# yxyxcyx/Real-Time-Recommendation-System-with-Feature-Store

Hardware: AMD Instinct MI355X
Metric: user-item pairs scored/sec (train) + top-K queries/sec, emb_dim=128 (higher is better)
Workload: dtype f32; 1 GPU; C2: MovieLens-1M two-tower train step, emb 128, batch 1024, 16 negatives, hidden [256,128], dropout 0.2, tau 0.05, Adam+clip; global_batch=1024, emb_dim=128, num_negatives=16, parallelism=dp1

## Files before the change

### include/rtrec_hip.h

```cpp
#ifndef RTREC_HIP_H
#define RTREC_HIP_H

#include <stddef.h>
#include <stdint.h>

#ifdef __cplusplus
extern "C" {
#endif

typedef enum {
    RT_OK = 0,
    RT_ERR_INVALID = -1,
    RT_ERR_UNSUPPORTED = -2,
    RT_ERR_WORKSPACE = -3,
    RT_ERR_HIP = -4
} rt_status;

typedef enum { RT_F32 = 0, RT_F16 = 1, RT_BF16 = 2 } rt_dtype;

typedef enum {
    RT_ACT_RELU = 0,
    RT_ACT_GELU = 1,
    RT_ACT_LEAKY_RELU = 2,
    RT_ACT_TANH = 3,
    RT_ACT_SIGMOID = 4,
    RT_ACT_NONE = 5
} rt_act;

int rt_abi_version(void);
const char* rt_status_string(int status);
const char* rt_last_error(void);

int rt_gather_rows(const void* table, int64_t row_begin, int64_t n_rows, int64_t row_bytes,
                   const int64_t* ids, int64_t n_ids, void* out, int32_t* oob_count, void* stream);

int rt_scatter_add_rows_f32(float* grad_table, int64_t n_rows, int dim, const int64_t* ids,
                            int64_t n_ids, const float* grad_out, int64_t padding_idx, void* stream);

int rt_scatter_rows(const void* src, int64_t n, int64_t row_bytes, const int64_t* positions,
                    void* dst, int64_t dst_rows, int32_t* oob_count, void* stream);
size_t rt_rows_compact_workspace_bytes(int64_t n_rows);
int rt_rows_compact(const void* src, int64_t n_rows, int64_t row_bytes,
                    const uint32_t* keep_bits, int64_t keep_words,
                    void* dst, int64_t dst_rows, int64_t* n_kept,
                    void* workspace, size_t workspace_bytes, void* stream);

int rt_l2_renorm_f32(float* x, int64_t n, int d, void* stream);

size_t rt_flatip_topk_workspace_bytes(int64_t nq, int64_t nx, int d, int dtype, int k);
int rt_flatip_topk(const void* queries, int64_t nq, const void* items, int64_t nx, int d, int dtype,
                   int k, const uint32_t* exclude_bits, int64_t exclude_words, int64_t id_offset,
                   float* out_scores, int64_t* out_ids, void* workspace, size_t workspace_bytes,
                   void* stream);

#define RT_ONLINE_MAX_NQ 8
#define RT_ONLINE_MAX_K 128
size_t rt_flatip_topk_online_workspace_bytes(int64_t nq, int64_t nx, int d, int dtype, int k);
int rt_flatip_topk_online_plan(int64_t nq, int64_t nx, int d, int dtype, int k, int64_t* out);
int rt_flatip_topk_online(const void* queries, int64_t nq, const void* items, int64_t nx, int d, int dtype,
                          int k, const uint32_t* exclude_bits, int64_t exclude_words, int64_t id_offset,
                          float* out_scores, int64_t* out_ids, void* workspace, size_t workspace_bytes,
                          void* stream);

typedef struct {
    const int64_t* offsets;
    const int32_t* items;
    int64_t        n_rows;
    const int64_t* rows;
} RtExclusionLists;

#define RT_ONLINE_MAX_EXCL_SOURCES 2
int rt_flatip_topk_online_lists(const void* queries, int64_t nq, const void* items, int64_t nx, int d, int dtype,
                                int k, const RtExclusionLists* lists, int n_lists, int64_t id_offset,
                                float* out_scores, int64_t* out_ids, void* workspace, size_t workspace_bytes,
                                void* stream);

#define RT_IVF_MAX_K 128
#define RT_IVF_MAX_NPROBE 128
int rt_ivf_topk_tuning(int min_chunk_tiles);
int rt_ivf_topk_plan(int64_t nq, int nprobe, int64_t max_list_rows, int64_t* out);
size_t rt_ivf_topk_workspace_bytes(int64_t nq, int nprobe, int64_t max_list_rows, int k);
int rt_ivf_topk(const void* queries, int64_t nq, const void* rows, int64_t nx, int d, int dtype,
                const int64_t* list_offsets, int64_t nlist, const int32_t* row_pos, const int64_t* probes,
                int nprobe, int64_t max_list_rows, int k, const uint32_t* exclude_bits, int64_t exclude_words,
                float* out_scores, int64_t* out_ids, void* workspace, size_t workspace_bytes, void* stream);
int rt_segment_mean_f32(const void* rows, int64_t n, int d, int dtype, const int64_t* offsets, int64_t n_seg,
                        const float* prev, int normalize, float* out, void* stream);

size_t rt_flatip_topk_shard_workspace_bytes(int64_t nq, int64_t nx, int d, int dtype, int k);
int rt_flatip_topk_shard_plan(int64_t nq, int64_t nx, int d, int dtype, int k, int stride, int64_t* stage_counts);
int rt_flatip_topk_shard_sample(const void* queries, int64_t nq, const void* items, int64_t nx, int d, int dtype,
                                int k, int stride, float* top32, int64_t* stage_counts, void* workspace,
                                size_t workspace_bytes, void* stream);
int rt_topk_sample_rank(int k, int64_t sampled_stages, int64_t stages, int* rank);
int rt_topk_sample_threshold(const float* lists, int n_lists, int64_t nq, int rank, float* thr, void* stream);
int rt_flatip_topk_shard_search(const void* queries, int64_t nq, const void* items, int64_t nx, int d, int dtype,
                                int k, const float* thr, int64_t id_offset, float* out_scores, int64_t* out_ids,
                                void* workspace, size_t workspace_bytes, void* stream);

int rt_flatip_topk_tuning(int v4_mode, int v4_stride, int v4_rank);

int rt_l2_augment_f32(const float* x, int64_t n, int d, float* out, int ld_out, int role, void* stream);
int rt_l2_finish_f32(const float* q_aug, int ld_q, const float* x_aug, int ld_x, int d, int64_t nq, int k_sel,
                     const int64_t* sel_ids, const float* sel_scores, int k, float* scores, int64_t* ids,
                     int32_t* unverified, int64_t id_offset, void* stream);

int rt_topk_merge(const float* scores, const int64_t* ids, int64_t nq, int n_lists, int k_in,
                  int k_out, float* out_scores, int64_t* out_ids, void* stream);

int rt_sample_negatives(const int64_t* pos_offsets, const int32_t* pos_items, int64_t n_users,
                        const int64_t* users, int64_t n, int64_t num_items, int num_neg, uint64_t seed,
                        const uint64_t* seed_offset, int64_t* out, void* stream);

int rt_feeder_batch(const int64_t* order, const int64_t* inter_u, const int64_t* inter_m, const int64_t* state,
                    int64_t batch, int64_t* users, int64_t* pos, void* stream);
int rt_feeder_commit(const double* loss, double* losses, int64_t n_losses, int64_t* state, void* stream);

#ifndef RT_STAT_SLOTS
#define RT_STAT_SLOTS 8
#endif
#if RT_STAT_SLOTS > 15
#error "RT_STAT_SLOTS > 15: the host arenas (rtrec_amd/models/fused.py STAT_SLOTS) hold 16 slot rows, one of them for ticket counters"
#endif

typedef struct {
    const float* src;
    int64_t src_rows;
    int ld_src;
    const int64_t* ids;
    int64_t m;
    int k;
    int n;
    const float* w;
    const float* bias;
    int prev_mode;
    int prev_act;
    const double* prev_stats;
    const float* bn_gamma;
    const float* bn_beta;
    float* running_mean;
    float* running_var;
    float* save_mean;
    float* save_invstd;
    float bn_eps;
    float bn_momentum;
    float drop_p;
    uint64_t drop_seed;
    const uint64_t* seed_offset;
    float* z_out;
    int act;
    double* stats_out;
    float* l2_out;
    float* norms_out;
    int64_t* num_batches_tracked;
    int64_t seg_split;
    double* zero_buf;
    int64_t zero_words;
    float* wt_out;
    float* a_out;
    float* fin_save_mean;
    float* fin_save_invstd;
    float* fin_running_mean;
    float* fin_running_var;
    int64_t* fin_num_batches_tracked;
    float fin_eps;
    float fin_momentum;
    int prev_final;
    const uint16_t* w_planes;
    uint16_t* wt_planes_out;
    const float* next_w;
    uint16_t* next_w_planes;
    int next_n;
    int next_k;
} rt_linear_fwd_args;

int rt_linear_fwd_f32(const rt_linear_fwd_args* args, void* stream);

typedef struct {
    int64_t m; int k; int n;
    const float* w;
    float* dw;
    float* dbias;
    float* dz_ws;
    int grad_mode;
    const float* dout;
    const float* l2_out;
    const float* norms;
    const float* g;
    const float* z;
    int act;
    const double* g_stats;
    const float* save_mean;
    const float* save_invstd;
    const float* bn_gamma;
    float* dgamma;
    float* dbeta;
    const float* src; int64_t src_rows; int ld_src; const int64_t* ids;
    int prev_mode; int prev_act;
    const float* prev_mean; const float* prev_invstd;
    const float* prev_gamma; const float* prev_beta;
    float prev_drop_p; uint64_t prev_drop_seed; const uint64_t* seed_offset;
    float* g_prev;
    double* g_prev_stats;
    float* dsrc;
    int64_t seg_split;
    double* dbias_slots;
    const float* wt;
    int fuse_dz;
    const float* a_in;
    float* dw_part;
    const float* fold_src;
    float* fold_dst;
    int64_t fold_words;
    int fold_splits;
    int fold_in;
    const uint16_t* wt_planes;
} rt_linear_bwd_args;

int rt_linear_bwd_f32(const rt_linear_bwd_args* args, void* stream);
int rt_linear_bwd_dz_fused(const rt_linear_bwd_args* args, int n_args);
int rt_linear_bwd_dw_splits(const rt_linear_bwd_args* args, int n_args, int64_t* splits);
int rt_linear_bwd_dz_f32(const rt_linear_bwd_args* args, void* stream);
int rt_linear_bwd_dw_f32(const rt_linear_bwd_args* args, void* stream);
int rt_linear_fwd_f32_multi(const rt_linear_fwd_args* args, int n_args, void* stream);
int rt_linear_bwd_dz_f32_multi(const rt_linear_bwd_args* args, int n_args, void* stream);
int rt_linear_bwd_dw_f32_multi(const rt_linear_bwd_args* args, int n_args, void* stream);
int rt_linear_bwd_dw_f32_joint(const rt_linear_bwd_args* args, int n_args, void* stream);
int rt_linear_bwd_dw_joint_splits(const rt_linear_bwd_args* args, int n_args, int64_t* splits);

size_t rt_twotower_loss_workspace_bytes(int64_t b, int d);
int rt_twotower_loss_fwd_bwd(const void* u, const void* p, const void* q, int dtype, int64_t b,
                             int d, int n_neg, float inv_tau, const float* user_bias,
                             const float* item_bias, float w_explicit, float w_in_batch,
                             double* loss_out, float* du, float* dp, float* dq, float* d_user_bias,
                             float* d_item_bias, void* workspace, size_t workspace_bytes, void* stream);

int rt_twotower_loss_fwd(const void* u, const void* p, const void* q, int dtype, int64_t b, int d,
                         int n_neg, float inv_tau, const float* user_bias, const float* item_bias,
                         float w_explicit, float w_in_batch, double* loss_out, void* workspace,
                         size_t workspace_bytes, void* stream);

size_t rt_inbatch_loss_workspace_bytes(int64_t b, int64_t n_items, int d);
int rt_inbatch_loss_fwd_bwd(const void* u, const void* p, int dtype, int64_t b, int64_t n_items, int d,
                            int64_t label_offset, float inv_tau, double* loss_out, float* du, float* dp,
                            void* workspace, size_t workspace_bytes, void* stream);

int rt_similarity_f32(const float* u, const float* v, int64_t b, int d, float inv_tau,
                      const float* user_bias, const float* item_bias, float* out, void* stream);

#define RT_GRAD_FOLD_MAX 8
typedef struct {
    const float* part;
    int64_t dst_off;
    int64_t words;
    int splits;
    int tensor;
} rt_grad_fold;
int rt_grad_sqnorm(const float* grads, const int64_t* offsets, int n_tensors, double* sumsq_out,
                   int32_t* step_counter, int64_t* seed_counter, void* stream);
int rt_grad_sqnorm_fold(float* grads, const int64_t* offsets, int n_tensors, double* sumsq_out,
                        int32_t* step_counter, int64_t* seed_counter, const rt_grad_fold* folds,
                        int n_folds, void* stream);
int rt_clip_adam_step(float* params, float* grads, float* exp_avg, float* exp_avg_sq,
                      int64_t n, const double* sumsq, int n_tensors, float max_norm, float lr,
                      const float* lr_dev, float beta1, float beta2, float eps, float weight_decay,
                      int step, const int32_t* step_dev, double* zero_buf, int64_t zero_words,
                      void* stream);

#define RT_TOWER_MAX_LAYERS 8
#define RT_TOWER_MAX_ROWS   8
#define RT_TOWER_MAX_WIDTH  512
typedef struct {
    const float* w;
    const float* bias;
    int k, n;
    int act;
    const float* bn_gamma;
    const float* bn_beta;
    const float* bn_mean;
    const float* bn_var;
    float bn_eps;
} rt_tower_layer;
typedef struct {
    const float* src; int64_t src_rows; int ld_src;
    const int64_t* ids;
    int m;
    int n_layers;
    rt_tower_layer layers[RT_TOWER_MAX_LAYERS];
    int normalize;
    float* out;
    float* norms_out;
} rt_tower_infer_args;
int rt_tower_infer_f32(const rt_tower_infer_args* args, void* stream);

#define RT_METRICS_MAX_K 16

int rt_exclusion_bitmap(const int64_t* offsets, const int32_t* items, int64_t n_csr_rows, const int64_t* rows,
                        int64_t n_rows, int64_t n_items, uint32_t* bits, int64_t words, void* stream);
int rt_rank_metrics(const int64_t* preds, int64_t n_rows, int list_len, const int64_t* gt_offsets,
                    const int32_t* gt_items, const int64_t* gt_rows, int64_t n_gt_rows,
                    const int64_t* ex_offsets, const int32_t* ex_items, const int64_t* ex_rows,
                    int64_t n_ex_rows, const int32_t* k_values, int n_k, int64_t num_items,
                    double* per_row, int32_t* valid, uint32_t* coverage_bits, void* stream);
int rt_rank_metrics_reduce(const double* per_row, const int32_t* valid, int64_t n_rows, int n_cols,
                           const uint32_t* coverage_bits, int64_t num_items, double* out, void* stream);

int rt_list_metrics(const int64_t* preds, int64_t n_rows, int list_len, const void* emb, int emb_dtype,
                    int64_t n_emb, int d, int64_t ld_emb, const double* info, int64_t n_info, double default_info,
                    const int32_t* k_values, int n_k, double* div, int32_t* div_valid, double* nov_sum,
                    int32_t* nov_cnt, int32_t* oob_count, void* stream);
int rt_list_metrics_reduce(const double* div, const int32_t* div_valid, const double* nov_sum,
                           const int32_t* nov_cnt, int64_t n_rows, int n_k, double* out, void* stream);

#ifdef __cplusplus
}
#endif

#endif
```

### real-time-recommendation-system-with-feature-store_amd/csrc/loss.hip

```cpp
#include <float.h>

#include "rt_common.h"
#include "split3.h"

namespace rt {
size_t ib16_workspace_bytes(int64_t b, int64_t nx, int d);
int ib16_run(const void* u, const void* p, int dtype, int64_t b, int64_t nx, int d, int64_t off, float inv_tau,
             double* loss_out, float* du, float* dp, void* ws, size_t ws_bytes, hipStream_t st);
namespace loss {

typedef float f32x16 __attribute__((ext_vector_type(16)));
constexpr int RB = 32;
constexpr int kMaxD = 256;
constexpr int kMaxNeg = 64;
constexpr int NG = 16;


__device__ __forceinline__ int tile_row(int r, int h) { return (r & 3) + 8 * (r >> 2) + 4 * h; }

struct Args {
    const void* u; const void* p; const void* q;
    int64_t b; int d; int n_neg; float inv_tau;
    const float* ub; const float* ib;
    float we, wb;
    double* loss;
    float* du; float* dp; float* dq; float* dub; float* dib;
    float2* part;
    float* diag;
    float* expl;
    float* dposv;
    int64_t nx;
    int64_t off;
    int n_split;
    int ib_blocks;
    bool grad;
};

constexpr int SPAN = 256;
constexpr int LDP = 4;

template <typename T>
__device__ __forceinline__ float4 load4(const T* __restrict__ p) {
    if constexpr (sizeof(T) == 4) {
        return *reinterpret_cast<const float4*>(p);
    } else {
        const uint2 r = *reinterpret_cast<const uint2*>(p);
        const T* e = reinterpret_cast<const T*>(&r);
        return make_float4(to_f32(e[0]), to_f32(e[1]), to_f32(e[2]), to_f32(e[3]));
    }
}

template <int DP, typename T>
__device__ __forceinline__ void load_rows(const T* __restrict__ M, int64_t r0, int64_t n, int D,
                                          float4 (&v)[DP / 8]) {
    const int lane = threadIdx.x & 63;
#pragma unroll
    for (int u = 0; u < DP / 8; ++u) {
        const int e = lane + 64 * u;
        const int row = e / (DP / 4), c = (e % (DP / 4)) * 4;
        const int64_t gr = r0 + row;
        v[u] = make_float4(0.f, 0.f, 0.f, 0.f);
        if (gr < n && c < D) v[u] = load4<T>(M + gr * D + c);
    }
}
template <int DP>
__device__ __forceinline__ void store_rows(float* __restrict__ S, const float4 (&v)[DP / 8]) {
    const int lane = threadIdx.x & 63;
#pragma unroll
    for (int u = 0; u < DP / 8; ++u) {
        const int e = lane + 64 * u;
        const int row = e / (DP / 4), c = (e % (DP / 4)) * 4;
        *reinterpret_cast<float4*>(S + row * (DP + LDP) + c) = v[u];
    }
}
using fsplit::Pieces;
using fsplit::split8;
using fsplit::mfma3;
template <int DP, typename T>
__device__ __forceinline__ void load_fixed3(const T* __restrict__ F, int64_t f0, int64_t n, int D,
                                            Pieces (&pf)[DP / 16]) {
    const int lane = threadIdx.x & 63, c = lane & 31, h = lane >> 5;
    const int64_t r = f0 + c;
#pragma unroll
    for (int kb = 0; kb < DP / 16; ++kb) {
        const int k = 16 * kb + 8 * h;
        float4 u = make_float4(0.f, 0.f, 0.f, 0.f), v = u;
        if (r < n && k < D) {
            u = load4<T>(F + r * D + k);
            v = load4<T>(F + r * D + k + 4);
        }
        const float x[8] = {u.x, u.y, u.z, u.w, v.x, v.y, v.z, v.w};
        pf[kb] = split8(x);
    }
}
template <int DP>
__device__ __forceinline__ f32x16 s_tile3(const float* __restrict__ Ss, const Pieces (&pf)[DP / 16]) {
    const int lane = threadIdx.x & 63, c = lane & 31, h = lane >> 5;
    const float* ap = Ss + c * (DP + LDP) + 8 * h;
    f32x16 acc = {};
#pragma unroll
    for (int kb = 0; kb < DP / 16; ++kb) {
        const float4 u = *reinterpret_cast<const float4*>(ap + 16 * kb);
        const float4 v = *reinterpret_cast<const float4*>(ap + 16 * kb + 4);
        const float x[8] = {u.x, u.y, u.z, u.w, v.x, v.y, v.z, v.w};
        acc = mfma3(split8(x), pf[kb], acc);
    }
    return acc;
}
template <int DP>
constexpr size_t inb_lds_bytes(int waves) { return static_cast<size_t>(waves) * 32 * (DP + LDP) * sizeof(float); }
template <int DP>
constexpr int bwd_waves() {
#ifdef RT_LOSS_BWD_WAVES
    static_assert(RT_LOSS_BWD_WAVES == 4 || RT_LOSS_BWD_WAVES == 8, "the two forms that are built and tested");
    return DP <= 128 ? RT_LOSS_BWD_WAVES : 4;
#else
    return DP <= 128 ? 8 : 4;
#endif
}

template <int DP, typename T>
__global__ __launch_bounds__(256) void loss_fwd_kernel(Args a) {
    const T* __restrict__ U = static_cast<const T*>(a.u);
    const T* __restrict__ P = static_cast<const T*>(a.p);
    const T* __restrict__ Qn = static_cast<const T*>(a.q);
    extern __shared__ __attribute__((aligned(16))) float sm_f[];
    __shared__ float negs[4][kMaxNeg];
    __shared__ float red_m[4][RB], red_l[4][RB];
    const int tid = threadIdx.x, lane = tid & 63, w = tid >> 6, c = lane & 31, h = lane >> 5;
    const int it = blockIdx.x, js = blockIdx.y;
    const int64_t i0 = static_cast<int64_t>(it) * RB;
    const int D = a.d;
    const float bias = (a.ub ? a.ub[0] : 0.f) + (a.ib ? a.ib[0] : 0.f);
    const float inv_b = 1.f / static_cast<float>(a.b);

    if (js < a.ib_blocks) {
        float* Ss = sm_f + w * 32 * (DP + LDP);
        Pieces pf[DP / 16];
        load_fixed3<DP, T>(U, i0, a.b, D, pf);
        const int64_t t0 = static_cast<int64_t>(js) * SPAN + 32 * w, t1 = t0 + 128;
        float4 buf[DP / 8];
        load_rows<DP, T>(P, t0, a.nx, D, buf);
        float om = -INFINITY, ol = 0.f;
#pragma unroll 1
        for (int q = 0; q < 2; ++q) {
            const int64_t tt = q == 0 ? t0 : t1;
            if (tt >= a.nx) break;
            store_rows<DP>(Ss, buf);
            wave_lds_sync();
            if (q == 0 && t1 < a.nx) load_rows<DP, T>(P, t1, a.nx, D, buf);
            const f32x16 acc = s_tile3<DP>(Ss, pf);
#pragma unroll
            for (int r = 0; r < 16; ++r) {
                if (tt + tile_row(r, h) < a.nx) {
                    const float sv = acc[r] * a.inv_tau;
                    if (sv > om) { ol = ol * expf(om - sv) + 1.f; om = sv; }
                    else ol += expf(sv - om);
                }
            }
            wave_lds_sync();
        }
        const float m2 = __shfl_xor(om, 32, 64), l2 = __shfl_xor(ol, 32, 64);
        const float mm = fmaxf(om, m2);
        ol = (mm == -INFINITY) ? 0.f : ol * expf(om - mm) + l2 * expf(m2 - mm);
        if (h == 0) { red_m[w][c] = mm; red_l[w][c] = ol; }
        __syncthreads();
        if (w == 0 && h == 0 && i0 + c < a.b) {
            float m3 = -INFINITY;
            for (int x = 0; x < 4; ++x) m3 = fmaxf(m3, red_m[x][c]);
            float ll = 0.f;
            if (m3 != -INFINITY)
                for (int x = 0; x < 4; ++x) ll += red_l[x][c] * expf(red_m[x][c] - m3);
            a.part[static_cast<int64_t>(js) * a.b + i0 + c] = make_float2(m3, ll);
        }
        return;
    }

    const int64_t i = i0 + 4 * (js - a.ib_blocks) + w;
    if (i >= a.b) return;
    const T* ur = U + i * D;
    const T* pr = P + (a.off + i) * D;
    constexpr int V = kMaxD / 64;
    float uv[V], pv[V];
    float part = 0.f;
#pragma unroll
    for (int t = 0; t < V; ++t) {
        const int dd = lane + 64 * t;
        uv[t] = dd < D ? to_f32(ur[dd]) : 0.f;
        pv[t] = dd < D ? to_f32(pr[dd]) : 0.f;
        part += uv[t] * pv[t];
    }
    float qv[NG][V];
    auto load_q = [&](int g0) {
#pragma unroll
        for (int jj = 0; jj < NG; ++jj) {
            const int j = g0 + jj;
            const T* qr = Qn + (i * a.n_neg + (j < a.n_neg ? j : 0)) * D;
#pragma unroll
            for (int t = 0; t < V; ++t) {
                const int dd = lane + 64 * t;
                qv[jj][t] = (j < a.n_neg && dd < D) ? to_f32(qr[dd]) : 0.f;
            }
        }
    };
    if (a.n_neg > 0) load_q(0);
    const float dup = wave_sum(part) * a.inv_tau;
    if (lane == 0) a.diag[i] = dup;
    if (a.n_neg <= 0) {
        if (a.grad) {
#pragma unroll
            for (int t = 0; t < V; ++t) {
                const int dd = lane + 64 * t;
                if (dd < D) { a.du[i * D + dd] = 0.f; a.dp[i * D + dd] = 0.f; }
            }
        }
        return;
    }
    const float pos = dup + bias;
    float mx = pos;
    for (int g0 = 0; g0 < a.n_neg; g0 += NG) {
        if (g0 > 0) load_q(g0);
        float part_j[NG];
#pragma unroll
        for (int jj = 0; jj < NG; ++jj) {
            part_j[jj] = 0.f;
#pragma unroll
            for (int t = 0; t < V; ++t) part_j[jj] += uv[t] * qv[jj][t];
        }
#pragma unroll
        for (int o = 32; o > 0; o >>= 1)
#pragma unroll
            for (int jj = 0; jj < NG; ++jj) part_j[jj] += __shfl_xor(part_j[jj], o, 64);
#pragma unroll
        for (int jj = 0; jj < NG; ++jj) {
            if (g0 + jj < a.n_neg) {
                const float nv = part_j[jj] * a.inv_tau;
                if (lane == 0) negs[w][g0 + jj] = nv;
                mx = fmaxf(mx, nv);
            }
        }
    }
    wave_lds_sync();
    float se = expf(pos - mx);
    for (int j = 0; j < a.n_neg; ++j) se += expf(negs[w][j] - mx);
    const float lse = mx + logf(se);
    const float dpos = a.we * inv_b * (expf(pos - lse) - 1.f);
    if (lane == 0) {
        a.expl[i] = lse - pos;
        a.dposv[i] = dpos;
    }
    if (!a.grad) return;
    float duv[V];
#pragma unroll
    for (int t = 0; t < V; ++t) duv[t] = dpos * pv[t];
    for (int g0 = 0; g0 < a.n_neg; g0 += NG) {
        if (a.n_neg > NG) load_q(g0);
#pragma unroll
        for (int jj = 0; jj < NG; ++jj) {
            const int j = g0 + jj;
            if (j >= a.n_neg) break;
            const float dn = a.we * inv_b * expf(negs[w][j] - lse);
            float* dqr = a.dq + (i * a.n_neg + j) * D;
#pragma unroll
            for (int t = 0; t < V; ++t) {
                const int dd = lane + 64 * t;
                if (dd < D) {
                    duv[t] += dn * qv[jj][t];
                    dqr[dd] = dn * uv[t] * a.inv_tau;
                }
            }
        }
    }
#pragma unroll
    for (int t = 0; t < V; ++t) {
        const int dd = lane + 64 * t;
        if (dd < D) {
            a.du[i * D + dd] = duv[t] * a.inv_tau;
            a.dp[i * D + dd] = dpos * uv[t] * a.inv_tau;
        }
    }
}

__device__ __forceinline__ float combine_lse(const float2* part, int n_split, int64_t b, int64_t i) {
    float mm = -INFINITY;
    for (int s = 0; s < n_split; ++s) mm = fmaxf(mm, part[static_cast<int64_t>(s) * b + i].x);
    float ll = 0.f;
    for (int s = 0; s < n_split; ++s) {
        const float2 v = part[static_cast<int64_t>(s) * b + i];
        if (v.x != -INFINITY) ll += v.y * expf(v.x - mm);
    }
    return mm + logf(ll);
}

template <int DP, typename T, int NW>
__global__ __launch_bounds__(64 * NW) void loss_bwd_kernel(Args a, float wb_eff, bool add_loss) {
    constexpr int DT = DP / 32;
    constexpr int NT = SPAN / (32 * NW);
    static_assert(NT * 32 * NW == SPAN && NT >= 1, "the waves' tiles cover the span");
    extern __shared__ __attribute__((aligned(16))) float sm_b[];
    __shared__ float lse_s[SPAN];
    const int tid = threadIdx.x, lane = tid & 63, w = tid >> 6, c = lane & 31, h = lane >> 5;
    const int D = a.d;
    const bool row_pass = blockIdx.z == 0;
    const int64_t f0 = static_cast<int64_t>(blockIdx.x) * RB;
    const int64_t s0 = static_cast<int64_t>(blockIdx.y) * SPAN;
    const int64_t n_fixed = row_pass ? a.b : a.nx, n_str = row_pass ? a.nx : a.b;
    if (f0 >= n_fixed || s0 >= n_str) {
        if (!(row_pass && blockIdx.y == 0 && f0 < a.b)) return;
    }
    const T* Fm = static_cast<const T*>(row_pass ? a.u : a.p);
    const T* Sm = static_cast<const T*>(row_pass ? a.p : a.u);
    const float scale = wb_eff / static_cast<float>(a.b);
    float lse_fixed = 0.f;
    const bool ib = wb_eff != 0.f;
    if (row_pass) {
        const int64_t i = f0 + c;
        if (ib && i < a.b) lse_fixed = combine_lse(a.part, a.n_split, a.b, i);
        if (add_loss && blockIdx.y == 0 && w == 0) {
            double li = 0.0, le = 0.0;
            float dpb = 0.f;
            if (h == 0 && i < a.b) {
                if (ib) li = static_cast<double>(lse_fixed - a.diag[i]) / static_cast<double>(a.b);
                if (a.n_neg > 0) {
                    le = static_cast<double>(a.expl[i]) / static_cast<double>(a.b);
                    dpb = a.dposv[i];
                }
            }
            li = wave_sum(li);
            le = wave_sum(le);
            dpb = wave_sum(dpb);
            if (lane == 0) {
                if (ib) atomicAdd(&a.loss[2], li);
                if (a.n_neg > 0) atomicAdd(&a.loss[1], le);
                atomicAdd(&a.loss[0], static_cast<double>(wb_eff) * li + static_cast<double>(a.we) * le);
                if (a.grad && a.n_neg > 0) {
                    if (a.dub) atomicAdd(a.dub, dpb);
                    if (a.dib) atomicAdd(a.dib, dpb);
                }
            }
        }
    } else {
        for (int x = tid; x < SPAN; x += 64 * NW) {
            const int64_t i = s0 + x;
            lse_s[x] = i < a.b ? combine_lse(a.part, a.n_split, a.b, i) : 0.f;
        }
    }
    __syncthreads();
    if (!a.grad || !ib || f0 >= n_fixed || s0 >= n_str) return;

    float* Ss = sm_b + w * 32 * (DP + LDP);
    Pieces pf[DP / 16];
    load_fixed3<DP, T>(Fm, f0, n_fixed, D, pf);
    const int64_t t0 = s0 + 32 * w;
    float4 buf[DP / 8];
    load_rows<DP, T>(Sm, t0, n_str, D, buf);
    f32x16 acc[DT];
#pragma unroll
    for (int x = 0; x < DT; ++x) acc[x] = f32x16{};
#pragma unroll 1
    for (int q = 0; q < NT; ++q) {
        const int64_t tt = t0 + 32 * NW * q;
        if (tt >= n_str) break;
        store_rows<DP>(Ss, buf);
        wave_lds_sync();
        if (q + 1 < NT && tt + 32 * NW < n_str) load_rows<DP, T>(Sm, tt + 32 * NW, n_str, D, buf);
        const f32x16 st = s_tile3<DP>(Ss, pf);
        float ds[16];
        const int64_t fcol = f0 + c;
#pragma unroll
        for (int r = 0; r < 16; ++r) {
            const int rr = tile_row(r, h);
            const int64_t srow = tt + rr;
            float v = 0.f;
            if (srow < n_str && fcol < n_fixed) {
                const float lse = row_pass ? lse_fixed : lse_s[32 * (w + NW * q) + rr];
                const bool label = row_pass ? (srow == a.off + fcol) : (fcol == a.off + srow);
                v = scale * (expf(st[r] * a.inv_tau - lse) - (label ? 1.f : 0.f));
            }
            ds[r] = v;
        }
        Pieces pds[2];
#pragma unroll
        for (int b = 0; b < 2; ++b) {
            const float x[8] = {ds[8 * b], ds[8 * b + 1], ds[8 * b + 2], ds[8 * b + 3],
                                ds[8 * b + 4], ds[8 * b + 5], ds[8 * b + 6], ds[8 * b + 7]};
            pds[b] = split8(x);
        }
#pragma unroll
        for (int dt = 0; dt < DT; ++dt) {
#pragma unroll
            for (int b = 0; b < 2; ++b) {
                float y[8];
#pragma unroll
                for (int j = 0; j < 8; ++j) y[j] = Ss[tile_row(8 * b + j, h) * (DP + LDP) + dt * 32 + c];
                acc[dt] = mfma3(pds[b], split8(y), acc[dt]);
            }
        }
        wave_lds_sync();
    }
    __syncthreads();
    float* red = sm_b;
#pragma unroll
    for (int dt = 0; dt < DT; ++dt)
#pragma unroll
        for (int r = 0; r < 16; ++r) red[(w * DT * 16 + dt * 16 + r) * 64 + lane] = acc[dt][r];
    __syncthreads();
    float* out = row_pass ? a.du : a.dp;
    for (int p = tid; p < DT * 16 * 64; p += 64 * NW) {
        const int v = p >> 6, l = p & 63;
        float t = red[v * 64 + l];
#pragma unroll
        for (int x = 1; x < NW; ++x) t += red[(x * DT * 16 + v) * 64 + l];
        const int dt = v >> 4, r = v & 15;
        const int64_t gi = f0 + tile_row(r, l >> 5);
        const int dd = dt * 32 + (l & 31);
        if (gi < n_fixed && dd < D) atomicAdd(&out[gi * D + dd], t * a.inv_tau);
    }
}

__global__ __launch_bounds__(256) void similarity_kernel(const float* u, const float* v, int64_t b, int d,
                                                         float inv_tau, const float* ub, const float* ib,
                                                         float* out) {
    const int lane = threadIdx.x & 63;
    const int64_t i = static_cast<int64_t>(blockIdx.x) * 4 + (threadIdx.x >> 6);
    if (i >= b) return;
    float s = 0.f;
    for (int dd = lane; dd < d; dd += 64) s += u[i * d + dd] * v[i * d + dd];
    s = wave_sum(s);
    if (lane == 0) {
        float r = s * inv_tau;
        if (ub) r = r + ub[0] + ib[0];
        out[i] = r;
    }
}

}
}

using namespace rt;

namespace {
template <auto Kernel>
void allow_lds(size_t bytes) {
    static size_t set = 0;
    if (bytes > set) {
        (void)hipFuncSetAttribute(reinterpret_cast<const void*>(Kernel), hipFuncAttributeMaxDynamicSharedMemorySize,
                                  static_cast<int>(bytes));
        set = bytes;
    }
}

template <int DP, typename T>
int launch_loss(const loss::Args& a, dim3 grid1, dim3 grid2, float wb_eff, hipStream_t st) {
    const size_t lds1 = loss::inb_lds_bytes<DP>(4);
    allow_lds<loss::loss_fwd_kernel<DP, T>>(lds1);
    hipLaunchKernelGGL((loss::loss_fwd_kernel<DP, T>), grid1, dim3(256), lds1, st, a);
    const int rc = check_launch("loss_fwd_kernel");
    if (rc) return rc;
    constexpr int NW = loss::bwd_waves<DP>();
    const size_t lds2 = loss::inb_lds_bytes<DP>(NW);
    allow_lds<loss::loss_bwd_kernel<DP, T, NW>>(lds2);
    hipLaunchKernelGGL((loss::loss_bwd_kernel<DP, T, NW>), grid2, dim3(64 * NW), lds2, st, a, wb_eff, true);
    return check_launch("loss_bwd_kernel");
}

template <typename T>
int launch_loss_d(const loss::Args& a, int dp32, dim3 grid1, dim3 grid2, float wb_eff, hipStream_t st) {
    switch (dp32) {
        case 32: return launch_loss<32, T>(a, grid1, grid2, wb_eff, st);
        case 64: return launch_loss<64, T>(a, grid1, grid2, wb_eff, st);
        case 96:
        case 128: return launch_loss<128, T>(a, grid1, grid2, wb_eff, st);
        default: return launch_loss<256, T>(a, grid1, grid2, wb_eff, st);
    }
}

size_t loss_ws_bytes(int64_t b, int64_t nx) {
    const int64_t n_split = (nx + loss::SPAN - 1) / loss::SPAN;
    return static_cast<size_t>(n_split) * b * sizeof(float2) + 3 * static_cast<size_t>(b) * sizeof(float);
}

int run_loss(const void* u, const void* p, const void* q, int dtype, int64_t b, int64_t nx, int64_t off, int d,
             int n_neg, float inv_tau, const float* ub, const float* ib, float we, float wb, double* loss_out,
             float* du, float* dp, float* dq, float* dub, float* dib, void* ws, size_t ws_bytes, void* stream,
             bool grad) {
    if (dtype != RT_F32 && dtype != RT_F16 && dtype != RT_BF16) return RT_ERR_INVALID;
    if (b <= 0 || d <= 0 || n_neg < 0 || !u || !p || !loss_out) return RT_ERR_INVALID;
    if (nx < b || off < 0 || off + b > nx) return RT_ERR_INVALID;
    if (d % 8 != 0 || d > loss::kMaxD || n_neg > loss::kMaxNeg) return RT_ERR_UNSUPPORTED;
    if (n_neg > 0 && !q) return RT_ERR_INVALID;
    if (grad && (!du || !dp || (n_neg > 0 && !dq))) return RT_ERR_INVALID;
    const int n_split = static_cast<int>((nx + loss::SPAN - 1) / loss::SPAN);
    if (!ws || ws_bytes < loss_ws_bytes(b, nx)) return RT_ERR_WORKSPACE;
    if ((reinterpret_cast<uintptr_t>(u) | reinterpret_cast<uintptr_t>(p)) & 15) return RT_ERR_INVALID;
    float2* part = reinterpret_cast<float2*>(ws);
    float* diag = reinterpret_cast<float*>(part + static_cast<size_t>(n_split) * b);
    const float wb_eff = n_neg > 0 ? wb : 1.f;
    const float we_eff = n_neg > 0 ? we : 0.f;
    const bool want_ib = wb_eff != 0.f;
    loss::Args a{u, p, q, b, d, n_neg, inv_tau, ub, ib, we_eff, wb_eff, loss_out, du, dp, dq, dub, dib, part, diag,
                 diag + b, diag + 2 * b, nx, off, n_split, want_ib ? n_split : 0, grad};
    hipStream_t st = as_stream(stream);
    if (grad && nx != b) {
        if (hipMemsetAsync(dp, 0, static_cast<size_t>(nx) * d * sizeof(float), st) != hipSuccess)
            return check_launch("hipMemsetAsync(dp)");
    }
    const int64_t big = nx > b ? nx : b;
    const int dp32 = (d + 31) / 32 * 32;
    const unsigned y2 = static_cast<unsigned>((big + loss::SPAN - 1) / loss::SPAN);
    const dim3 grid1(static_cast<unsigned>((b + loss::RB - 1) / loss::RB), a.ib_blocks + 8);
    const dim3 grid2(static_cast<unsigned>((big + loss::RB - 1) / loss::RB), want_ib ? y2 : 1,
                     (grad && want_ib) ? 2 : 1);
    switch (dtype) {
        case RT_F32: return launch_loss_d<float>(a, dp32, grid1, grid2, wb_eff, st);
        case RT_F16: return launch_loss_d<__half>(a, dp32, grid1, grid2, wb_eff, st);
        default: return launch_loss_d<__hip_bfloat16>(a, dp32, grid1, grid2, wb_eff, st);
    }
}
}

extern "C" size_t rt_twotower_loss_workspace_bytes(int64_t b, int d) {
    (void)d;
    if (b <= 0) return 256;
    return loss_ws_bytes(b, b) + 256;
}

extern "C" size_t rt_inbatch_loss_workspace_bytes(int64_t b, int64_t n_items, int d) {
    if (b <= 0 || n_items < b || d <= 0) return 256;
    const size_t f32 = loss_ws_bytes(b, n_items), h16 = ib16_workspace_bytes(b, n_items, d);
    return (f32 > h16 ? f32 : h16) + 256;
}

extern "C" int rt_inbatch_loss_fwd_bwd(const void* u, const void* p, int dtype, int64_t b, int64_t n_items, int d,
                                       int64_t label_offset, float inv_tau, double* loss_out, float* du, float* dp,
                                       void* workspace, size_t workspace_bytes, void* stream) {
    if (dtype == RT_F16 || dtype == RT_BF16) {
        if (b <= 0 || d <= 0 || !u || !p || !loss_out) return RT_ERR_INVALID;
        if (n_items < b || label_offset < 0 || label_offset + b > n_items) return RT_ERR_INVALID;
        if (d % 8 != 0 || d > loss::kMaxD) return RT_ERR_UNSUPPORTED;
        if ((du == nullptr) != (dp == nullptr)) return RT_ERR_INVALID;
        if ((reinterpret_cast<uintptr_t>(u) | reinterpret_cast<uintptr_t>(p)) & 15) return RT_ERR_INVALID;
        return ib16_run(u, p, dtype, b, n_items, d, label_offset, inv_tau, loss_out, du, dp, workspace,
                        workspace_bytes, as_stream(stream));
    }
    return run_loss(u, p, nullptr, dtype, b, n_items, label_offset, d, 0, inv_tau, nullptr, nullptr, 0.f, 1.f,
                    loss_out, du, dp, nullptr, nullptr, nullptr, workspace, workspace_bytes, stream, du != nullptr);
}


extern "C" int rt_twotower_loss_fwd_bwd(const void* u, const void* p, const void* q, int dtype, int64_t b, int d,
                                        int n_neg, float inv_tau, const float* user_bias, const float* item_bias,
                                        float w_explicit, float w_in_batch, double* loss_out, float* du, float* dp,
                                        float* dq, float* d_user_bias, float* d_item_bias, void* workspace,
                                        size_t workspace_bytes, void* stream) {
    return run_loss(u, p, q, dtype, b, b, 0, d, n_neg, inv_tau, user_bias, item_bias, w_explicit, w_in_batch,
                    loss_out, du, dp, dq, d_user_bias, d_item_bias, workspace, workspace_bytes, stream, true);
}

extern "C" int rt_twotower_loss_fwd(const void* u, const void* p, const void* q, int dtype, int64_t b, int d,
                                    int n_neg, float inv_tau, const float* user_bias, const float* item_bias,
                                    float w_explicit, float w_in_batch, double* loss_out, void* workspace,
                                    size_t workspace_bytes, void* stream) {
    return run_loss(u, p, q, dtype, b, b, 0, d, n_neg, inv_tau, user_bias, item_bias, w_explicit, w_in_batch,
                    loss_out, nullptr, nullptr, nullptr, nullptr, nullptr, workspace, workspace_bytes, stream, false);
}

extern "C" int rt_similarity_f32(const float* u, const float* v, int64_t b, int d, float inv_tau,
                                 const float* user_bias, const float* item_bias, float* out, void* stream) {
    if (b < 0 || d <= 0 || !u || !v || !out) return RT_ERR_INVALID;
    if ((user_bias == nullptr) != (item_bias == nullptr)) return RT_ERR_INVALID;
    if (b == 0) return RT_OK;
    hipLaunchKernelGGL(loss::similarity_kernel, dim3(static_cast<unsigned>((b + 3) / 4)), dim3(256), 0,
                       as_stream(stream), u, v, b, d, inv_tau, user_bias, item_bias, out);
    return check_launch("similarity_kernel");
}
```

### real-time-recommendation-system-with-feature-store_amd/csrc/mlp.hip

```cpp
#include "rt_common.h"
#include "split3.h"

namespace rt {
namespace mlp {

typedef float f32x16 __attribute__((ext_vector_type(16)));



constexpr float kNormEps = 1e-12f;

struct FwdLaunch {
    rt_linear_fwd_args a0, a1;
    unsigned split;
};
struct BwdLaunch {
    rt_linear_bwd_args a0, a1;
    unsigned split;
    int64_t rps0, rps1;
    unsigned tn0, tk0, tn1, tk1;
    bool vec0, vec1;
    int ngroups;
    unsigned ksplit = 1;
};

constexpr int kFoldG = 8;
__device__ __forceinline__ void fold_side(const BwdLaunch& L, int which) {
    const int64_t nt = static_cast<int64_t>(gridDim.x) * blockDim.x;
    const int64_t gt = static_cast<int64_t>(blockIdx.x) * blockDim.x + threadIdx.x;
    for (int g = 0; g < L.ngroups; ++g) {
        const rt_linear_bwd_args& f = g ? L.a1 : L.a0;
        if (!f.fold_src || f.fold_in != which || f.fold_splits <= 0) continue;
        const int64_t n4 = f.fold_words / 4;
        const int ng = (f.fold_splits + kFoldG - 1) / kFoldG;
        for (int64_t it = gt; it < n4 * ng; it += nt) {
            const int64_t e = it % n4;
            const int s0 = static_cast<int>(it / n4) * kFoldG;
            float4 v[kFoldG];
#pragma unroll
            for (int j = 0; j < kFoldG; ++j)
                v[j] = s0 + j < f.fold_splits
                           ? reinterpret_cast<const float4*>(f.fold_src + static_cast<int64_t>(s0 + j) * f.fold_words)[e]
                           : make_float4(0.f, 0.f, 0.f, 0.f);
            float4 t = v[0];
#pragma unroll
            for (int j = 1; j < kFoldG; ++j) { t.x += v[j].x; t.y += v[j].y; t.z += v[j].z; t.w += v[j].w; }
            float* d = f.fold_dst + 4 * e;
            if (ng == 1) {
                const float4 o = *reinterpret_cast<const float4*>(d);
                *reinterpret_cast<float4*>(d) = make_float4(o.x + t.x, o.y + t.y, o.z + t.z, o.w + t.w);
            } else {
                atomicAdd(d, t.x); atomicAdd(d + 1, t.y); atomicAdd(d + 2, t.z); atomicAdd(d + 3, t.w);
            }
        }
    }
}


#ifdef RT_PHASE_PROBE
__device__ unsigned long long* g_probe_buf = nullptr;
__device__ unsigned int g_probe_ctr[64];
__device__ unsigned int g_probe_cap = 0;
struct PhaseProbe {
    uint64_t rt0 = 0, t0 = 0, m[4] = {0, 0, 0, 0};
    __device__ __forceinline__ void start() {
        if (threadIdx.x == 0) {
            rt0 = __builtin_amdgcn_s_memrealtime();
            t0 = __builtin_amdgcn_s_memtime();
        }
    }
    __device__ __forceinline__ void mark(int i) {
        if (threadIdx.x == 0) m[i] = __builtin_amdgcn_s_memtime() - t0;
    }
    __device__ __forceinline__ void end(unsigned tag) {
        if (threadIdx.x == 0) {
            asm volatile("s_waitcnt vmcnt(0)" ::: "memory");
            m[3] = __builtin_amdgcn_s_memtime() - t0;
            const uint64_t rt1 = __builtin_amdgcn_s_memrealtime();
            const unsigned xcc = __builtin_amdgcn_s_getreg((20) | (0 << 6) | ((4 - 1) << 11));
            const unsigned sh = blockIdx.x & 63u;
            const unsigned slot = atomicAdd(&g_probe_ctr[sh], 1u);
            if (slot < g_probe_cap && g_probe_buf) {
                unsigned long long* o = g_probe_buf + (static_cast<uint64_t>(slot) * 64 + sh) * 8;
                o[0] = (static_cast<uint64_t>(tag) << 32) | blockIdx.x;
                o[1] = rt0; o[2] = m[0]; o[3] = m[1]; o[4] = m[2]; o[5] = m[3]; o[6] = rt1; o[7] = xcc;
            }
        }
    }
};
#define RT_PP_DECL PhaseProbe pp_; pp_.start();
#define RT_PP_MARK(i) pp_.mark(i);
#define RT_PP_END(tag) pp_.end(tag);
#else
#define RT_PP_DECL
#define RT_PP_MARK(i)
#define RT_PP_END(tag)
#endif

#if !defined(RT_NO_WT_STORES)
#define RT_WT_STORES 1
#endif
__device__ __forceinline__ void st_act(float* p, float v) {
#ifdef RT_WT_STORES
    __hip_atomic_store(p, v, __ATOMIC_RELAXED, __HIP_MEMORY_SCOPE_AGENT);
#else
    *p = v;
#endif
}
__device__ __forceinline__ void st_act4(float* p, float4 v) {
#ifdef RT_WT_STORES
    typedef float f4v __attribute__((ext_vector_type(4)));
    const f4v x = {v.x, v.y, v.z, v.w};
    asm volatile("global_store_dwordx4 %0, %1, off sc1" ::"v"(p), "v"(x) : "memory");
#else
    *reinterpret_cast<float4*>(p) = v;
#endif
}

__device__ __forceinline__ f32x16 mfma(float a, float b, f32x16 c) {
    return __builtin_amdgcn_mfma_f32_32x32x2f32(a, b, c, 0, 0, 0);
}

using fsplit::Pieces;
using fsplit::s16x8;
using fsplit::split8;
using fsplit::mfma3;
using fsplit::split3;

struct Pro {
    int mode;
    int act;
    float drop_p, drop_scale;
    uint64_t seed;
    const float* scale;
    const float* shift;
};

__device__ __forceinline__ float pro_apply(const Pro& p, int64_t r, int c, float v) {
    if (p.mode == 0) return v;
    v = act_eval(p.act, v);
    if (p.mode != 3) v = __builtin_fmaf(v, p.scale[c], p.shift[c]);
    if (p.drop_p > 0.f) v = dropout_keep(p.seed, r, c, p.drop_p) ? v * p.drop_scale : 0.f;
    return v;
}

__device__ __forceinline__ void slot_sums(const double* __restrict__ base, int w, int c, double& s1, double& s2) {
    double v1[RT_STAT_SLOTS], v2[RT_STAT_SLOTS];
#pragma unroll
    for (int sl = 0; sl < RT_STAT_SLOTS; ++sl) {
        v1[sl] = base[static_cast<int64_t>(sl) * 2 * w + c];
        v2[sl] = base[static_cast<int64_t>(sl) * 2 * w + w + c];
    }
    s1 = 0.0;
    s2 = 0.0;
#pragma unroll
    for (int sl = 0; sl < RT_STAT_SLOTS; ++sl) {
        s1 += v1[sl];
        s2 += v2[sl];
    }
}

__device__ __forceinline__ void bn_affine(float gamma, float beta, float mean, float invstd, float& scale,
                                          float& shift) {
    scale = gamma * invstd;
    shift = __builtin_fmaf(-mean, scale, beta);
}

__device__ __forceinline__ void ticket_release() {
#ifdef RT_TICKET_WBL2
    __builtin_amdgcn_fence(__ATOMIC_RELEASE, "agent");
#endif
    asm volatile("s_waitcnt vmcnt(0)" ::: "memory");
}

__device__ __forceinline__ void bn_finalize_last(const rt_linear_fwd_args& a, unsigned nblk) {
    __shared__ int last_s;
    const int tid = threadIdx.x, n = a.n;
    const bool two = a.seg_split > 0;
    const int nseg = two ? 2 : 1;
    asm volatile("s_waitcnt vmcnt(0)" ::: "memory");
    __syncthreads();
    if (tid == 0) {
        ticket_release();
        unsigned long long* cnt =
            reinterpret_cast<unsigned long long*>(a.stats_out + static_cast<int64_t>(nseg) * RT_STAT_SLOTS * 2 * n);
        last_s = atomicAdd(cnt, 1ull) == static_cast<unsigned long long>(nblk) - 1ull ? 1 : 0;
    }
    __syncthreads();
    if (!last_s) return;
    for (int c = tid; c < n; c += blockDim.x) {
        for (int sg = 0; sg < nseg; ++sg) {
            const int64_t ms = two ? (sg == 0 ? a.seg_split : a.m - a.seg_split) : a.m;
            double* ps = a.stats_out + static_cast<int64_t>(sg) * RT_STAT_SLOTS * 2 * n;
            double v1[RT_STAT_SLOTS], v2[RT_STAT_SLOTS];
#pragma unroll
            for (int sl = 0; sl < RT_STAT_SLOTS; ++sl) {
                v1[sl] = atomicAdd(&ps[static_cast<int64_t>(sl) * 2 * n + c], 0.0);
                v2[sl] = atomicAdd(&ps[static_cast<int64_t>(sl) * 2 * n + n + c], 0.0);
            }
            double s1 = 0.0, s2 = 0.0;
#pragma unroll
            for (int sl = 0; sl < RT_STAT_SLOTS; ++sl) {
                s1 += v1[sl];
                s2 += v2[sl];
            }
            const double md = s1 / static_cast<double>(ms);
            double vd = s2 / static_cast<double>(ms) - md * md;
            vd = vd > 0.0 ? vd : 0.0;
            const float mean = static_cast<float>(md);
            const float invstd = static_cast<float>(1.0 / sqrt(vd + static_cast<double>(a.fin_eps)));
            const float var_f = static_cast<float>(ms > 1 ? vd * static_cast<double>(ms) / static_cast<double>(ms - 1) : vd);
            a.fin_save_mean[sg * n + c] = mean;
            if (a.fin_save_invstd) a.fin_save_invstd[sg * n + c] = invstd;
            if (a.fin_running_mean) {
                const float mo = a.fin_momentum;
                a.fin_running_mean[c] = (1.f - mo) * a.fin_running_mean[c] + mo * mean;
                a.fin_running_var[c] = (1.f - mo) * a.fin_running_var[c] + mo * var_f;
            }
        }
    }
    if (tid == 0 && a.fin_num_batches_tracked) *a.fin_num_batches_tracked += nseg;
}

constexpr int FM = 32;

__host__ __device__ __forceinline__ int pad8(int k) { return (k + 31) / 32 * 32; }
__host__ __device__ __forceinline__ bool dz_norm_fast(int n) {
    const int l4 = n / 4;
    return (n % 4) == 0 && l4 <= 64 && (l4 & (l4 - 1)) == 0 && pad8(n) == n;
}
__host__ __device__ __forceinline__ bool dz_bn_fast(int n, int act, int grad_mode) {
    return (n % 4) == 0 && (256 % (pad8(n) / 4)) == 0 && act_is_piecewise_linear(act) && grad_mode != 3;
}
__host__ __device__ __forceinline__ bool dz_da_fast(const rt_linear_bwd_args& a) {
    return !a.dsrc && a.g_prev && act_is_piecewise_linear(a.prev_act);
}

template <int TPW, bool KVEC, bool WPL>
__global__ __launch_bounds__(256) __attribute__((amdgpu_waves_per_eu(TPW == 1 ? 3 : 2))) void linear_fwd_kernel(FwdLaunch L) {
    static_assert(!WPL || (TPW == 1 && KVEC), "split-weight planes: one-tile waves, k % 4 == 0");
    const bool g1 = blockIdx.x >= L.split;
    const rt_linear_fwd_args& a = g1 ? L.a1 : L.a0;
    const unsigned bid = blockIdx.x - (g1 ? L.split : 0u);
    constexpr int NT = 4 * TPW;
    extern __shared__ __attribute__((aligned(16))) float sm[];
    const int k = a.k, n = a.n;
    const int kp = pad8(k), aplane = FM * kp, aw = 3 * aplane / 2;
    const int nch = kp / 8, am = ((nch & -nch) < 16 ? (nch & -nch) : 16) - 1;
    float* scale = sm;
    float* shift = scale + kp;
    float* As = shift + kp;
    uint16_t* const Ap = reinterpret_cast<uint16_t*>(As);
    float* rowpart = As + aw;
    int64_t* srow = reinterpret_cast<int64_t*>(rowpart + NT * FM);

    const int tid = threadIdx.x, lane = tid & 63, w = tid >> 6, h = lane >> 5, c32 = lane & 31;
    const int64_t row0 = static_cast<int64_t>(bid) * FM;
    const int64_t m = a.m;
    auto put_a = [&](int r, int c, float4 o) {
        if (a.a_out && c < k && row0 + r < m) st_act4(a.a_out + (row0 + r) * k + c, o);
        uint32_t h0, m0, l0, h1, m1, l1;
        split3(o.x, o.y, h0, m0, l0);
        split3(o.z, o.w, h1, m1, l1);
        uint16_t* q = Ap + r * kp + ((((c >> 3) ^ (r & am)) << 3) | (c & 7));
        *reinterpret_cast<uint2*>(q) = make_uint2(h0, h1);
        *reinterpret_cast<uint2*>(q + aplane) = make_uint2(m0, m1);
        *reinterpret_cast<uint2*>(q + 2 * aplane) = make_uint2(l0, l1);
    };
    RT_PP_DECL
    if (blockIdx.x == 0 && a.zero_buf)
        for (int64_t e = tid; e < a.zero_words; e += 256) a.zero_buf[e] = 0.0;

    const int vpr = kp / 4;
    const bool vec = (a.ld_src % 4) == 0 && (reinterpret_cast<uintptr_t>(a.src) & 15) == 0;
    const bool fast = vec && (a.k % 4) == 0 && (256 % vpr) == 0 &&
                      (a.prev_mode == 0 || act_is_piecewise_linear(a.prev_act));
    const bool early = fast && !a.ids && 8 * (256 / vpr) >= FM;
    if (a.wt_out) {
        const int tk = (k + 31) / 32, tiles = tk * ((n + 31) / 32);
        const int nblk = static_cast<int>(g1 ? gridDim.x - L.split : L.split);
        for (int wt = static_cast<int>(bid); wt < tiles; wt += nblk) {
            const int n0 = (wt / tk) * 32, k0 = (wt % tk) * 32;
            const int r = tid >> 3, c = (tid & 7) * 4;
            if (n0 + r < n) {
#pragma unroll
                for (int j = 0; j < 4; ++j)
                    if (k0 + c + j < k) a.wt_out[static_cast<int64_t>(k0 + c + j) * n + n0 + r] = a.w[static_cast<int64_t>(n0 + r) * k + k0 + c + j];
            }
        }
    }
    if (a.wt_planes_out || a.next_w_planes) {
        const int nblk = static_cast<int>(g1 ? gridDim.x - L.split : L.split);
        if (a.wt_planes_out) {
            const int64_t plane = static_cast<int64_t>(n) * k;
            const int nq = (n + 3) / 4;
            for (int64_t e = static_cast<int64_t>(bid) * 256 + tid; e < static_cast<int64_t>(k) * nq;
                 e += static_cast<int64_t>(nblk) * 256) {
                const int kk = static_cast<int>(e / nq), n0 = static_cast<int>(e % nq) * 4;
                float x[4];
#pragma unroll
                for (int j = 0; j < 4; ++j) x[j] = n0 + j < n ? a.w[static_cast<int64_t>(n0 + j) * k + kk] : 0.f;
                uint32_t h0, m0, l0, h1, m1, l1;
                split3(x[0], x[1], h0, m0, l0);
                split3(x[2], x[3], h1, m1, l1);
                uint16_t* q = a.wt_planes_out + static_cast<int64_t>(kk) * n + n0;
                if (n0 + 4 <= n && (n % 4) == 0) {
                    *reinterpret_cast<uint2*>(q) = make_uint2(h0, h1);
                    *reinterpret_cast<uint2*>(q + plane) = make_uint2(m0, m1);
                    *reinterpret_cast<uint2*>(q + 2 * plane) = make_uint2(l0, l1);
                } else {
                    const uint32_t hv[2] = {h0, h1}, mv[2] = {m0, m1}, lv[2] = {l0, l1};
                    for (int j = 0; j < 4 && n0 + j < n; ++j) {
                        const int sh = 16 * (j & 1);
                        q[j] = static_cast<uint16_t>(hv[j >> 1] >> sh);
                        q[j + plane] = static_cast<uint16_t>(mv[j >> 1] >> sh);
                        q[j + 2 * plane] = static_cast<uint16_t>(lv[j >> 1] >> sh);
                    }
                }
            }
        }
        if (a.next_w_planes) {
            const int64_t tot8 = static_cast<int64_t>(a.next_n) * a.next_k / 8;
            const float4* src4 = reinterpret_cast<const float4*>(a.next_w);
            s16x8* dst = reinterpret_cast<s16x8*>(a.next_w_planes);
            for (int64_t e = static_cast<int64_t>(bid) * 256 + tid; e < tot8; e += static_cast<int64_t>(nblk) * 256) {
                const float4 u = src4[2 * e], v = src4[2 * e + 1];
                const float x[8] = {u.x, u.y, u.z, u.w, v.x, v.y, v.z, v.w};
                const Pieces pc = split8(x);
                dst[e] = pc.hi;
                dst[e + tot8] = pc.mid;
                dst[e + 2 * tot8] = pc.lo;
            }
        }
    }
    const float* wrow[TPW];
    bool tile_on[TPW], row_ok[TPW];
#pragma unroll
    for (int i = 0; i < TPW; ++i) {
        tile_on[i] = (w + 4 * i) * 32 < n;
        const int nn = (w + 4 * i) * 32 + c32;
        row_ok[i] = nn < n;
        wrow[i] = a.w + static_cast<int64_t>(row_ok[i] ? nn : 0) * k;
    }
    float4 wv[TPW][4], wn[TPW][4];
    auto load_w = [&](int s, float4 (&dst)[TPW][4]) {
#pragma unroll
        for (int i = 0; i < TPW; ++i)
#pragma unroll
            for (int j = 0; j < 4; ++j) {
                const int kk = s + 16 * (j >> 1) + 8 * h + 4 * (j & 1);
                float4 v = make_float4(0.f, 0.f, 0.f, 0.f);
                if (tile_on[i] && row_ok[i]) {
                    const float* wr = wrow[i] + kk;
                    if constexpr (KVEC) {
                        if (kk < k) v = *reinterpret_cast<const float4*>(wr);
                    } else {
                        if (kk < k) v.x = wr[0];
                        if (kk + 1 < k) v.y = wr[1];
                        if (kk + 2 < k) v.z = wr[2];
                        if (kk + 3 < k) v.w = wr[3];
                    }
                }
                dst[i][j] = v;
            }
    };
    uint4 pv[2][3], pn[2][3];
    const int64_t wplane = static_cast<int64_t>(n) * k;
    auto load_p = [&](int s, uint4 (&dst)[2][3]) {
#pragma unroll
        for (int b = 0; b < 2; ++b) {
            const int kk = s + 16 * b + 8 * h;
            const bool ok = tile_on[0] && row_ok[0] && kk < k;
            const uint16_t* q = a.w_planes + (static_cast<int64_t>(row_ok[0] ? w * 32 + c32 : 0) * k + (ok ? kk : 0));
#pragma unroll
            for (int p = 0; p < 3; ++p)
                dst[b][p] = ok ? *reinterpret_cast<const uint4*>(q + p * wplane) : make_uint4(0u, 0u, 0u, 0u);
        }
    };
    if constexpr (WPL) load_p(0, pn);
    else if constexpr (TPW == 1) load_w(0, wn);
    float4 pre[8];
    if (early) {
        const int c = (tid % vpr) * 4, rstep = 256 / vpr, r0 = tid / vpr;
#pragma unroll
        for (int u = 0; u < 8; ++u) {
            const int r = r0 + u * rstep;
            const int64_t gr = row0 + r;
            pre[u] = make_float4(0.f, 0.f, 0.f, 0.f);
            if (r < FM && c < k && gr < m && gr < a.src_rows)
                pre[u] = *reinterpret_cast<const float4*>(a.src + gr * a.ld_src + c);
        }
    }

    const bool two = a.seg_split > 0;
    const int my_seg = (two && row0 >= a.seg_split) ? 1 : 0;
    if (a.prev_mode == 1 && a.prev_final) {
        for (int c = tid; c < k; c += 256)
            bn_affine(a.bn_gamma[c], a.bn_beta[c], a.save_mean[my_seg * k + c], a.save_invstd[my_seg * k + c], scale[c],
                      shift[c]);
    } else if (a.prev_mode == 1 || a.prev_mode == 2) {
        const int nseg = two ? 2 : 1;
        for (int c = tid; c < k; c += 256) {
            for (int sg = 0; sg < nseg; ++sg) {
                if (bid != 0 && sg != my_seg) continue;
                const int64_t ms = two ? (sg == 0 ? a.seg_split : m - a.seg_split) : m;
                float mean, invstd, var_f = 0.f;
                if (a.prev_mode == 1) {
                    const double* ps = a.prev_stats + static_cast<int64_t>(sg) * RT_STAT_SLOTS * 2 * k;
                    double s1, s2;
                    slot_sums(ps, k, c, s1, s2);
                    const double md = s1 / static_cast<double>(ms);
                    double vd = s2 / static_cast<double>(ms) - md * md;
                    vd = vd > 0.0 ? vd : 0.0;
                    mean = static_cast<float>(md);
                    invstd = static_cast<float>(1.0 / sqrt(vd + static_cast<double>(a.bn_eps)));
                    var_f = static_cast<float>(ms > 1 ? vd * static_cast<double>(ms) / static_cast<double>(ms - 1) : vd);
                } else {
                    mean = a.running_mean[c];
                    invstd = static_cast<float>(1.0 / sqrt(static_cast<double>(a.running_var[c]) + a.bn_eps));
                }
                if (sg == my_seg) bn_affine(a.bn_gamma[c], a.bn_beta[c], mean, invstd, scale[c], shift[c]);
                if (bid == 0) {
                    if (c == 0 && a.prev_mode == 1 && a.num_batches_tracked) *a.num_batches_tracked += 1;
                    if (a.save_mean) a.save_mean[sg * k + c] = mean;
                    if (a.save_invstd) a.save_invstd[sg * k + c] = invstd;
                    if (a.prev_mode == 1 && a.running_mean) {
                        const float mo = a.bn_momentum;
                        a.running_mean[c] = (1.f - mo) * a.running_mean[c] + mo * mean;
                        a.running_var[c] = (1.f - mo) * a.running_var[c] + mo * var_f;
                    }
                }
            }
        }
    }
    RT_PP_MARK(0)
    if (tid < FM) {
        const int64_t gr = row0 + tid;
        int64_t sr = -1;
        if (gr < m) {
            sr = a.ids ? a.ids[gr] : gr;
            if (sr < 0 || sr >= a.src_rows) sr = -1;
        }
        srow[tid] = sr;
    }
    __syncthreads();
    const uint64_t seed = a.drop_seed + (a.seed_offset ? *a.seed_offset : 0ull);
    const Pro pro{a.prev_mode, a.prev_act, a.drop_p, a.drop_p > 0.f ? 1.f / (1.f - a.drop_p) : 1.f, seed,
                  scale, shift};
    {
        const int total = FM * vpr;
        if (fast) {
            const int c = (tid % vpr) * 4, rstep = 256 / vpr;
            const bool bn = pro.mode == 1 || pro.mode == 2;
            const float4 sc4 = bn ? *reinterpret_cast<const float4*>(scale + c) : make_float4(1.f, 1.f, 1.f, 1.f);
            const float4 sh4 = bn ? *reinterpret_cast<const float4*>(shift + c) : make_float4(0.f, 0.f, 0.f, 0.f);
            const float sl = act_slope(pro.act);
            const bool drop = pro.drop_p > 0.f;
            for (int r0 = tid / vpr; r0 < FM; r0 += 8 * rstep) {
                float4 v[8];
#pragma unroll
                for (int u = 0; u < 8; ++u) {
                    const int r = r0 + u * rstep;
                    v[u] = make_float4(0.f, 0.f, 0.f, 0.f);
                    if (early) {
                        v[u] = pre[u];
                    } else if (r < FM && c < k) {
                        const int64_t sr = srow[r];
                        if (sr >= 0) v[u] = *reinterpret_cast<const float4*>(a.src + sr * a.ld_src + c);
                    }
                }
#pragma unroll
                for (int u = 0; u < 8; ++u) {
                    const int r = r0 + u * rstep;
                    if (r >= FM) break;
                    const int64_t gr = row0 + r;
                    const bool ok = srow[r] >= 0 && c < k;
                    auto tf = [&](float x, int cc, float scv, float shv) {
                        if (pro.mode == 0) return x;
                        x = act_pwl(sl, x);
                        if (bn) x = __builtin_fmaf(x, scv, shv);
                        if (drop) x = dropout_keep(pro.seed, gr, cc, pro.drop_p) ? x * pro.drop_scale : 0.f;
                        return x;
                    };
                    float4 o;
                    o.x = ok ? tf(v[u].x, c, sc4.x, sh4.x) : 0.f;
                    o.y = ok ? tf(v[u].y, c + 1, sc4.y, sh4.y) : 0.f;
                    o.z = ok ? tf(v[u].z, c + 2, sc4.z, sh4.z) : 0.f;
                    o.w = ok ? tf(v[u].w, c + 3, sc4.w, sh4.w) : 0.f;
                    put_a(r, c, o);
                }
            }
        } else
        for (int base = tid; base < total; base += 256 * 4) {
            float4 v[4];
#pragma unroll
            for (int u = 0; u < 4; ++u) {
                const int e = base + u * 256;
                v[u] = make_float4(0.f, 0.f, 0.f, 0.f);
                if (e < total) {
                    const int r = e / vpr, c = (e - r * vpr) * 4;
                    const int64_t sr = srow[r];
                    if (sr >= 0 && c < k) {
                        const float* sp = a.src + sr * a.ld_src + c;
                        if (vec && c + 4 <= k) v[u] = *reinterpret_cast<const float4*>(sp);
                        else {
                            v[u].x = sp[0];
                            if (c + 1 < k) v[u].y = sp[1];
                            if (c + 2 < k) v[u].z = sp[2];
                            if (c + 3 < k) v[u].w = sp[3];
                        }
                    }
                }
            }
#pragma unroll
            for (int u = 0; u < 4; ++u) {
                const int e = base + u * 256;
                if (e < total) {
                    const int r = e / vpr, c = (e - r * vpr) * 4;
                    const bool ok = srow[r] >= 0;
                    const int64_t gr = row0 + r;
                    float4 o;
                    o.x = (ok && c < k) ? pro_apply(pro, gr, c, v[u].x) : 0.f;
                    o.y = (ok && c + 1 < k) ? pro_apply(pro, gr, c + 1, v[u].y) : 0.f;
                    o.z = (ok && c + 2 < k) ? pro_apply(pro, gr, c + 2, v[u].z) : 0.f;
                    o.w = (ok && c + 3 < k) ? pro_apply(pro, gr, c + 3, v[u].w) : 0.f;
                    put_a(r, c, o);
                }
            }
        }
    }
    __syncthreads();
    RT_PP_MARK(1)

    f32x16 acc[TPW];
#pragma unroll
    for (int i = 0; i < TPW; ++i) acc[i] = f32x16{};
    const uint16_t* ap = Ap + c32 * kp;
    const int asw = c32 & am;
    if constexpr (TPW != 1) load_w(0, wn);
    if constexpr (WPL) {
        for (int s = 0; s < kp; s += 32) {
#pragma unroll
            for (int b = 0; b < 2; ++b)
#pragma unroll
                for (int p = 0; p < 3; ++p) pv[b][p] = pn[b][p];
            if (s + 32 < kp) load_p(s + 32, pn);
#pragma unroll
            for (int b = 0; b < 2; ++b) {
                const int ao = (((s + 16 * b) >> 3) + h) ^ asw;
                Pieces pa;
                pa.hi = *reinterpret_cast<const s16x8*>(ap + 8 * ao);
                pa.mid = *reinterpret_cast<const s16x8*>(ap + aplane + 8 * ao);
                pa.lo = *reinterpret_cast<const s16x8*>(ap + 2 * aplane + 8 * ao);
                if (tile_on[0]) {
                    const Pieces pb{__builtin_bit_cast(s16x8, pv[b][0]), __builtin_bit_cast(s16x8, pv[b][1]),
                                    __builtin_bit_cast(s16x8, pv[b][2])};
                    acc[0] = mfma3(pa, pb, acc[0]);
                }
            }
        }
    } else
    for (int s = 0; s < kp; s += 32) {
#pragma unroll
        for (int i = 0; i < TPW; ++i)
#pragma unroll
            for (int j = 0; j < 4; ++j) wv[i][j] = wn[i][j];
        if (s + 32 < kp) load_w(s + 32, wn);
#pragma unroll
        for (int b = 0; b < 2; ++b) {
            const int ao = (((s + 16 * b) >> 3) + h) ^ asw;
            Pieces pa;
            pa.hi = *reinterpret_cast<const s16x8*>(ap + 8 * ao);
            pa.mid = *reinterpret_cast<const s16x8*>(ap + aplane + 8 * ao);
            pa.lo = *reinterpret_cast<const s16x8*>(ap + 2 * aplane + 8 * ao);
#pragma unroll
            for (int i = 0; i < TPW; ++i) {
                if (!tile_on[i]) continue;
                const float4 u = wv[i][2 * b], v = wv[i][2 * b + 1];
                const float x[8] = {u.x, u.y, u.z, u.w, v.x, v.y, v.z, v.w};
                acc[i] = mfma3(pa, split8(x), acc[i]);
            }
        }
    }

    RT_PP_MARK(2)
    const bool l2 = a.l2_out != nullptr;
    if (l2 && !a.z_out && !a.stats_out && n * (FM + 1) <= aw) {
        __syncthreads();
        float* zsq = As;
#pragma unroll
        for (int i = 0; i < TPW; ++i) {
            const int col = (w + 4 * i) * 32 + c32;
            if ((w + 4 * i) * 32 >= n) continue;
            const bool col_ok = col < n;
            const float b = (col_ok && a.bias) ? a.bias[col] : 0.f;
#pragma unroll
            for (int r = 0; r < 16; ++r) {
                const int lr = (r & 3) + 8 * (r >> 2) + 4 * h;
                const float z = acc[i][r] + b;
                acc[i][r] = z;
                if (col_ok) zsq[col * (FM + 1) + lr] = (row0 + lr < m) ? z * z : 0.f;
            }
        }
        __syncthreads();
        {
            const int row = tid >> 3, part = tid & 7;
            float ss = 0.f;
            for (int c = part; c < n; c += 8) ss += zsq[c * (FM + 1) + row];
            ss += __shfl_xor(ss, 1, 64);
            ss += __shfl_xor(ss, 2, 64);
            ss += __shfl_xor(ss, 4, 64);
            if (part == 0) {
                const float nrm = sqrtf(ss);
                rowpart[row] = 1.f / fmaxf(nrm, kNormEps);
                if (row0 + row < m && a.norms_out) a.norms_out[row0 + row] = nrm;
            }
        }
        __syncthreads();
#pragma unroll
        for (int i = 0; i < TPW; ++i) {
            const int col = (w + 4 * i) * 32 + c32;
            if ((w + 4 * i) * 32 >= n) continue;
#pragma unroll
            for (int r = 0; r < 16; ++r) {
                const int lr = (r & 3) + 8 * (r >> 2) + 4 * h;
                const int64_t gr = row0 + lr;
                if (gr < m && col < n) st_act(a.l2_out + gr * n + col, acc[i][r] * rowpart[lr]);
            }
        }
        RT_PP_END(1)
        return;
    }
    double* const stats = a.stats_out ? a.stats_out + (static_cast<int64_t>(my_seg) * RT_STAT_SLOTS +
                                                       bid % RT_STAT_SLOTS) * 2 * n : nullptr;
#pragma unroll
    for (int i = 0; i < TPW; ++i) {
        const int ct = w + 4 * i;
        const int col = ct * 32 + c32;
        const bool col_ok = col < n;
        const float b = (col_ok && a.bias) ? a.bias[col] : 0.f;
        float s1 = 0.f, s2 = 0.f;
        if (row0 + FM <= m && a.z_out && !l2 && act_is_piecewise_linear(a.act)) {
            if (ct * 32 >= n) continue;
            float* zp = a.z_out + (row0 + 4 * h) * n + col;
            const float sl = act_slope(a.act);
#pragma unroll
            for (int r = 0; r < 16; ++r) {
                const float z = acc[i][r] + b;
                if (col_ok) st_act(zp + ((r & 3) + 8 * (r >> 2)) * n, z);
                const float av = act_pwl(sl, z);
                s1 += av;
                s2 += av * av;
            }
            if (!col_ok) s1 = s2 = 0.f;
        } else
#pragma unroll
        for (int r = 0; r < 16; ++r) {
            const int lr = (r & 3) + 8 * (r >> 2) + 4 * h;
            const int64_t gr = row0 + lr;
            const float z = acc[i][r] + b;
            acc[i][r] = z;
            const bool ok = col_ok && gr < m;
            if (ok && a.z_out) st_act(a.z_out + gr * n + col, z);
            if (ok && stats) {
                const float av = act_eval(a.act, z);
                s1 += av;
                s2 += av * av;
            }
            if (l2) {
                float q = ok ? z * z : 0.f;
#pragma unroll
                for (int o = 1; o < 32; o <<= 1) q += __shfl_xor(q, o, 64);
                if (c32 == 0) rowpart[ct * FM + lr] = q;
            }
        }
        if (stats) {
            s1 += __shfl_xor(s1, 32, 64);
            s2 += __shfl_xor(s2, 32, 64);
            if (h == 0 && col_ok) {
                atomicAdd(&stats[col], static_cast<double>(s1));
                atomicAdd(&stats[n + col], static_cast<double>(s2));
            }
        }
    }
    if (stats && a.fin_save_mean) bn_finalize_last(a, g1 ? gridDim.x - L.split : L.split);
    if (l2) {
        __syncthreads();
        const int nt_used = (n + 31) / 32;
#pragma unroll
        for (int i = 0; i < TPW; ++i) {
            const int col = (w + 4 * i) * 32 + c32;
#pragma unroll
            for (int r = 0; r < 16; ++r) {
                const int lr = (r & 3) + 8 * (r >> 2) + 4 * h;
                const int64_t gr = row0 + lr;
                if (gr < m && col < n) {
                    float ss = 0.f;
                    for (int t = 0; t < nt_used; ++t) ss += rowpart[t * FM + lr];
                    const float nrm = sqrtf(ss);
                    a.l2_out[gr * n + col] = acc[i][r] / fmaxf(nrm, kNormEps);
                    if (col == 0 && a.norms_out) a.norms_out[gr] = nrm;
                }
            }
        }
    }
    RT_PP_END(1)
}

template <int TPWK, bool WPL, bool KS, int FE>
__global__ __launch_bounds__(256) __attribute__((amdgpu_waves_per_eu(3))) void linear_bwd_dz_kernel(BwdLaunch L) {
#ifdef RT_FOLD_FIRST
    fold_side(L, 0);
#endif
    const unsigned kpart = KS ? blockIdx.x % L.ksplit : 0u, bx = KS ? blockIdx.x / L.ksplit : blockIdx.x;
    const bool prim = kpart == 0;
    const int tb = static_cast<int>(kpart) * 4 * TPWK;
    const bool g1 = bx >= L.split;
    const rt_linear_bwd_args& a = g1 ? L.a1 : L.a0;
    const unsigned bid = bx - (g1 ? L.split : 0u);
    extern __shared__ __attribute__((aligned(16))) float sm[];
    const int n = a.n, k = a.k;
    const int64_t m = a.m;
    const int np = pad8(n), ldz = np + 4;
    float* Dz = sm;
    const int tid = threadIdx.x, lane = tid & 63, w = tid >> 6, h = lane >> 5, c32 = lane & 31;
    const int64_t row0 = static_cast<int64_t>(bid) * FM;
    const bool two = a.seg_split > 0;
    const int my_seg = (two && row0 >= a.seg_split) ? 1 : 0;
    const int64_t seg_m = two ? (my_seg == 0 ? a.seg_split : m - a.seg_split) : m;
    RT_PP_DECL

    float wv[TPWK][8], wn[TPWK][8];
    const float* __restrict__ Wt = a.w;
#ifdef RT_NO_WT_ROWS
    const float* __restrict__ WtT = nullptr;
#else
    const float* __restrict__ WtT = (a.wt && (n % 8) == 0) ? a.wt : nullptr;
#endif
    auto load_w = [&](int s, float (&dst)[TPWK][8]) {
#pragma unroll
        for (int i = 0; i < TPWK; ++i) {
            const int kk = (tb + w + 4 * i) * 32 + c32;
            const bool on = (tb + w + 4 * i) * 32 < k && kk < k;
            if (FE != 0 || WtT) {
                const int nn = s + 8 * h;
                float4 v0 = make_float4(0.f, 0.f, 0.f, 0.f), v1 = v0;
                if (on && nn < n) {
                    const float* p = WtT + static_cast<int64_t>(kk) * n + nn;
                    v0 = *reinterpret_cast<const float4*>(p);
                    v1 = *reinterpret_cast<const float4*>(p + 4);
                }
                dst[i][0] = v0.x; dst[i][1] = v0.y; dst[i][2] = v0.z; dst[i][3] = v0.w;
                dst[i][4] = v1.x; dst[i][5] = v1.y; dst[i][6] = v1.z; dst[i][7] = v1.w;
            } else {
#pragma unroll
                for (int j = 0; j < 8; ++j) {
                    const int nn = s + 8 * h + j;
                    dst[i][j] = (on && nn < n) ? Wt[static_cast<int64_t>(nn) * k + kk] : 0.f;
                }
            }
        }
    };
    uint4 pv[TPWK][3], pn[TPWK][3];
    const uint16_t* __restrict__ WtP = a.wt_planes;
    const int64_t tplane = static_cast<int64_t>(k) * n;
    auto load_p = [&](int s, uint4 (&dst)[TPWK][3]) {
#pragma unroll
        for (int i = 0; i < TPWK; ++i) {
            const int kk = (tb + w + 4 * i) * 32 + c32;
            const int nn = s + 8 * h;
            const bool ok = (tb + w + 4 * i) * 32 < k && kk < k && nn < n;
            const uint16_t* q = WtP + (ok ? static_cast<int64_t>(kk) * n + nn : 0);
#pragma unroll
            for (int p = 0; p < 3; ++p)
                dst[i][p] = ok ? *reinterpret_cast<const uint4*>(q + p * tplane) : make_uint4(0u, 0u, 0u, 0u);
        }
    };
    if constexpr (TPWK == 1) {
        if (a.g_prev || a.dsrc) {
            if constexpr (WPL) load_p(0, pn);
            else load_w(0, wn);
        }
    }

    const int l4 = n / 4;
    if (FE == 1 || (FE == 0 && a.grad_mode == 0 && dz_norm_fast(n))) {
        const int rpp = 64 / l4, sub = lane / l4, li = lane % l4, c = 4 * li;
        float4 lv[8], dv[8];
        float nr[8];
#pragma unroll
        for (int p = 0; p < 8; ++p) {
            const int r = w * 8 + p * rpp + sub;
            const int64_t gr = row0 + r;
            lv[p] = make_float4(0.f, 0.f, 0.f, 0.f);
            dv[p] = lv[p];
            nr[p] = 1.f;
            if (p * rpp < 8 && gr < m) {
                lv[p] = *reinterpret_cast<const float4*>(a.l2_out + gr * n + c);
                dv[p] = *reinterpret_cast<const float4*>(a.dout + gr * n + c);
                nr[p] = a.norms[gr];
            }
        }
#pragma unroll
        for (int p = 0; p < 8; ++p) {
            if (p * rpp >= 8) break;
            const int r = w * 8 + p * rpp + sub;
            const int64_t gr = row0 + r;
            float dot = lv[p].x * dv[p].x + lv[p].y * dv[p].y + lv[p].z * dv[p].z + lv[p].w * dv[p].w;
            for (int o = 1; o < l4; o <<= 1) dot += __shfl_xor(dot, o, 64);
            const bool big = nr[p] > kNormEps;
            const float inv = 1.f / (big ? nr[p] : kNormEps);
            float4 d = make_float4(0.f, 0.f, 0.f, 0.f);
            if (gr < m) {
                d.x = big ? (dv[p].x - lv[p].x * dot) * inv : dv[p].x * inv;
                d.y = big ? (dv[p].y - lv[p].y * dot) * inv : dv[p].y * inv;
                d.z = big ? (dv[p].z - lv[p].z * dot) * inv : dv[p].z * inv;
                d.w = big ? (dv[p].w - lv[p].w * dot) * inv : dv[p].w * inv;
                if (prim) st_act4(a.dz_ws + gr * n + c, d);
            }
            *reinterpret_cast<float4*>(Dz + r * ldz + c) = d;
        }
    } else if (FE == 0 && a.grad_mode == 0) {
        for (int rr = w * 8; rr < w * 8 + 8; ++rr) {
            const int64_t gr = row0 + rr;
            if (gr < m) {
                float dot = 0.f;
                for (int c = lane; c < n; c += 64) dot += a.l2_out[gr * n + c] * a.dout[gr * n + c];
                dot = wave_sum(dot);
                const float nrm = a.norms[gr];
                const bool big = nrm > kNormEps;
                const float inv = 1.f / (big ? nrm : kNormEps);
                for (int c = lane; c < np; c += 64) {
                    float dz = 0.f;
                    if (c < n) {
                        const float dv = a.dout[gr * n + c];
                        dz = big ? (dv - a.l2_out[gr * n + c] * dot) * inv : dv * inv;
                        if (prim) a.dz_ws[gr * n + c] = dz;
                    }
                    Dz[rr * ldz + c] = dz;
                }
            } else {
                for (int c = lane; c < np; c += 64) Dz[rr * ldz + c] = 0.f;
            }
        }
    } else if constexpr (FE != 1) {
        float* cA = Dz + FM * ldz;
        float* cB = cA + np;
        float* cC = cB + np;
        float* cM = cC + np;
        float* cI = cM + np;
        const float inv_m = 1.f / static_cast<float>(seg_m);
        const double* gst = a.g_stats ? a.g_stats + static_cast<int64_t>(my_seg) * RT_STAT_SLOTS * 2 * n : nullptr;
        const int vpr = np / 4;
        const bool vec = (n % 4) == 0;
        const bool fast = FE != 0 || dz_bn_fast(n, a.act, a.grad_mode);
        const bool early = fast && 8 * (256 / vpr) >= FM;
        float4 pg[8];
        if (early) {
            const int c = (tid % vpr) * 4, rstep = 256 / vpr, r0 = tid / vpr;
#pragma unroll
            for (int u = 0; u < 8; ++u) {
                const int r = r0 + u * rstep;
                const int64_t gr = row0 + r;
                pg[u] = make_float4(0.f, 0.f, 0.f, 0.f);
                if (r < FM && gr < m && c < n) pg[u] = *reinterpret_cast<const float4*>(a.g + gr * n + c);
            }
        }
        for (int c = tid; c < np; c += 256) {
            float A = 1.f, Bc = 0.f, C = 0.f, M = 0.f, I = 1.f;
            if (c < n && (a.grad_mode == 1 || a.grad_mode == 2)) {
                I = a.save_invstd[my_seg * n + c];
                M = a.save_mean[my_seg * n + c];
                A = a.bn_gamma[c] * I;
                if (a.grad_mode == 1) {
                    double gs1, gs2;
                    slot_sums(gst, n, c, gs1, gs2);
                    Bc = static_cast<float>(gs1) * inv_m;
                    C = static_cast<float>(gs2) * inv_m;
                }
            }
            cA[c] = A; cB[c] = Bc; cC[c] = C; cM[c] = M; cI[c] = I;
        }
        __syncthreads();
        const int total = FM * vpr;
        if (fast) {
            const int c = (tid % vpr) * 4, rstep = 256 / vpr;
            const float4 fA = *reinterpret_cast<const float4*>(cA + c), fB = *reinterpret_cast<const float4*>(cB + c);
            const float4 fC = *reinterpret_cast<const float4*>(cC + c), fM = *reinterpret_cast<const float4*>(cM + c);
            const float4 fI = *reinterpret_cast<const float4*>(cI + c);
            const float sl = act_slope(a.act);
            for (int r0 = tid / vpr; r0 < FM; r0 += 8 * rstep) {
                float4 gv[8], zv[8];
#pragma unroll
                for (int u = 0; u < 8; ++u) {
                    const int r = r0 + u * rstep;
                    const int64_t gr = row0 + r;
                    gv[u] = make_float4(0.f, 0.f, 0.f, 0.f);
                    zv[u] = gv[u];
                    if (early) {
                        gv[u] = pg[u];
                        if (r < FM && gr < m && c < n) zv[u] = *reinterpret_cast<const float4*>(a.z + gr * n + c);
                    } else if (r < FM && gr < m && c < n) {
                        gv[u] = *reinterpret_cast<const float4*>(a.g + gr * n + c);
                        zv[u] = *reinterpret_cast<const float4*>(a.z + gr * n + c);
                    }
                }
#pragma unroll
                for (int u = 0; u < 8; ++u) {
                    const int r = r0 + u * rstep;
                    if (r >= FM) break;
                    const int64_t gr = row0 + r;
                    auto one = [&](float g, float z, float A, float B, float C, float M, float I) {
                        const float xh = (act_pwl(sl, z) - M) * I;
                        return A * (g - B - xh * C) * (z > 0.f ? 1.f : sl);
                    };
                    float4 d;
                    d.x = one(gv[u].x, zv[u].x, fA.x, fB.x, fC.x, fM.x, fI.x);
                    d.y = one(gv[u].y, zv[u].y, fA.y, fB.y, fC.y, fM.y, fI.y);
                    d.z = one(gv[u].z, zv[u].z, fA.z, fB.z, fC.z, fM.z, fI.z);
                    d.w = one(gv[u].w, zv[u].w, fA.w, fB.w, fC.w, fM.w, fI.w);
                    if (gr >= m || c >= n) d = make_float4(0.f, 0.f, 0.f, 0.f);
                    *reinterpret_cast<float4*>(Dz + r * ldz + c) = d;
                    if (prim && gr < m && c < n) st_act4(a.dz_ws + gr * n + c, d);
                }
            }
        } else if constexpr (FE == 0) {
        for (int base = tid; base < total; base += 256 * 4) {
            float4 gv[4], zv[4];
#pragma unroll
            for (int u = 0; u < 4; ++u) {
                const int e = base + u * 256;
                gv[u] = make_float4(0.f, 0.f, 0.f, 0.f);
                zv[u] = gv[u];
                if (e < total) {
                    const int r = e / vpr, c = (e - r * vpr) * 4;
                    const int64_t gr = row0 + r;
                    if (gr < m && c < n) {
                        const int64_t off = gr * n + c;
                        if (vec) {
                            gv[u] = *reinterpret_cast<const float4*>(a.g + off);
                            zv[u] = *reinterpret_cast<const float4*>(a.z + off);
                        } else {
                            gv[u].x = a.g[off]; zv[u].x = a.z[off];
                            if (c + 1 < n) { gv[u].y = a.g[off + 1]; zv[u].y = a.z[off + 1]; }
                            if (c + 2 < n) { gv[u].z = a.g[off + 2]; zv[u].z = a.z[off + 2]; }
                            if (c + 3 < n) { gv[u].w = a.g[off + 3]; zv[u].w = a.z[off + 3]; }
                        }
                    }
                }
            }
#pragma unroll
            for (int u = 0; u < 4; ++u) {
                const int e = base + u * 256;
                if (e >= total) continue;
                const int r = e / vpr, c = (e - r * vpr) * 4;
                const int64_t gr = row0 + r;
                float dzv[4];
                const float gs[4] = {gv[u].x, gv[u].y, gv[u].z, gv[u].w};
                const float zs[4] = {zv[u].x, zv[u].y, zv[u].z, zv[u].w};
#pragma unroll
                for (int j = 0; j < 4; ++j) {
                    const int cc = c + j;
                    float dz = 0.f;
                    if (gr < m && cc < n) {
                        const float xh = (act_eval(a.act, zs[j]) - cM[cc]) * cI[cc];
                        const float dr = (a.grad_mode == 3) ? gs[j] : cA[cc] * (gs[j] - cB[cc] - xh * cC[cc]);
                        dz = dr * act_grad_eval(a.act, zs[j]);
                    }
                    dzv[j] = dz;
                }
                *reinterpret_cast<float4*>(Dz + r * ldz + c) = make_float4(dzv[0], dzv[1], dzv[2], dzv[3]);
                if (prim && gr < m && c < n) {
                    const int64_t off = gr * n + c;
                    if (vec) *reinterpret_cast<float4*>(a.dz_ws + off) = make_float4(dzv[0], dzv[1], dzv[2], dzv[3]);
                    else
                        for (int j = 0; j < 4 && c + j < n; ++j) a.dz_ws[off + j] = dzv[j];
                }
            }
        }
        }
    }
    RT_PP_MARK(0)
    if (prim && a.dbias && a.dbias_slots) {
        __syncthreads();
        double* sl = a.dbias_slots + static_cast<int64_t>(bid % RT_STAT_SLOTS) * n;
        for (int c = tid; c < n; c += 256) {
            float cs = 0.f;
#pragma unroll 8
            for (int r = 0; r < FM; ++r) cs += Dz[r * ldz + c];
            atomicAdd(&sl[c], static_cast<double>(cs));
        }
    }
    if (prim && bid == 0 && (a.grad_mode == 1 || a.grad_mode == 2) && a.dgamma) {
        for (int c = tid; c < n; c += 256) {
            for (int sg = 0; sg < (two ? 2 : 1); ++sg) {
                const double* gs = a.g_stats + static_cast<int64_t>(sg) * RT_STAT_SLOTS * 2 * n;
                double gs1, gs2;
                slot_sums(gs, n, c, gs1, gs2);
                atomicAdd(&a.dgamma[c], static_cast<float>(gs2));
                atomicAdd(&a.dbeta[c], static_cast<float>(gs1));
            }
        }
    }
    if (!a.g_prev && !a.dsrc) {
#ifndef RT_FOLD_FIRST
        fold_side(L, 0);
#endif
        RT_PP_END(2)
        return;
    }
    __syncthreads();
    RT_PP_MARK(1)

    const int ldb = np + 8;
    uint16_t* const planes = reinterpret_cast<uint16_t*>(Dz + FM * ldz + 5 * np);
    const int plane = FM * ldb;
    for (int e = tid; e < FM * (np / 4); e += 256) {
        const int r = e / (np / 4), c = (e - r * (np / 4)) * 4;
        const float4 v = *reinterpret_cast<const float4*>(Dz + r * ldz + c);
        uint32_t h0, m0, l0, h1, m1, l1;
        split3(v.x, v.y, h0, m0, l0);
        split3(v.z, v.w, h1, m1, l1);
        uint16_t* q = planes + r * ldb + c;
        *reinterpret_cast<uint2*>(q) = make_uint2(h0, h1);
        *reinterpret_cast<uint2*>(q + plane) = make_uint2(m0, m1);
        *reinterpret_cast<uint2*>(q + 2 * plane) = make_uint2(l0, l1);
    }
    __syncthreads();
    f32x16 acc[TPWK];
#pragma unroll
    for (int i = 0; i < TPWK; ++i) acc[i] = f32x16{};
    const uint16_t* ap = planes + c32 * ldb + 8 * h;
    const bool want_stats = a.g_prev && a.g_prev_stats && (a.prev_mode == 1 || a.prev_mode == 2);
    const bool fast = FE != 0 || (row0 + FM <= m && dz_da_fast(a));
    float zpre[TPWK][16], pmean[TPWK], pinv[TPWK];
#pragma unroll
    for (int i = 0; i < TPWK; ++i) {
        const int kk = (tb + w + 4 * i) * 32 + c32;
        const bool ld = fast && want_stats && kk < k;
        pmean[i] = ld ? a.prev_mean[my_seg * k + kk] : 0.f;
        pinv[i] = ld ? a.prev_invstd[my_seg * k + kk] : 0.f;
        const float* zp = a.src + (row0 + 4 * h) * a.ld_src + kk;
        if (ld) {
#pragma unroll
            for (int r = 0; r < 16; ++r) zpre[i][r] = zp[((r & 3) + 8 * (r >> 2)) * a.ld_src];
        } else {
#pragma unroll
            for (int r = 0; r < 16; ++r) zpre[i][r] = 0.f;
        }
    }
    if constexpr (WPL) {
        if constexpr (TPWK != 1) load_p(0, pn);
        for (int s = 0; s < np; s += 16) {
#pragma unroll
            for (int i = 0; i < TPWK; ++i)
#pragma unroll
                for (int p = 0; p < 3; ++p) pv[i][p] = pn[i][p];
            if (s + 16 < np) load_p(s + 16, pn);
            Pieces pa;
            pa.hi = *reinterpret_cast<const s16x8*>(ap + s);
            pa.mid = *reinterpret_cast<const s16x8*>(ap + plane + s);
            pa.lo = *reinterpret_cast<const s16x8*>(ap + 2 * plane + s);
#pragma unroll
            for (int i = 0; i < TPWK; ++i) {
                if ((tb + w + 4 * i) * 32 >= k) continue;
                const Pieces pb{__builtin_bit_cast(s16x8, pv[i][0]), __builtin_bit_cast(s16x8, pv[i][1]),
                                __builtin_bit_cast(s16x8, pv[i][2])};
                acc[i] = mfma3(pa, pb, acc[i]);
            }
        }
    } else {
    if constexpr (TPWK != 1) load_w(0, wn);
    for (int s = 0; s < np; s += 16) {
#pragma unroll
        for (int i = 0; i < TPWK; ++i)
#pragma unroll
            for (int j = 0; j < 8; ++j) wv[i][j] = wn[i][j];
        if (s + 16 < np) load_w(s + 16, wn);
        Pieces pa;
        pa.hi = *reinterpret_cast<const s16x8*>(ap + s);
        pa.mid = *reinterpret_cast<const s16x8*>(ap + plane + s);
        pa.lo = *reinterpret_cast<const s16x8*>(ap + 2 * plane + s);
#pragma unroll
        for (int i = 0; i < TPWK; ++i) {
            if ((tb + w + 4 * i) * 32 >= k) continue;
            acc[i] = mfma3(pa, split8(wv[i]), acc[i]);
        }
    }
    }
    RT_PP_MARK(2)
    const float pscale = a.prev_drop_p > 0.f ? 1.f / (1.f - a.prev_drop_p) : 1.f;
    const uint64_t pseed = a.prev_drop_seed + (a.seed_offset ? *a.seed_offset : 0ull);
    double* const gps = want_stats ? a.g_prev_stats + (static_cast<int64_t>(my_seg) * RT_STAT_SLOTS +
                                                        bid % RT_STAT_SLOTS) * 2 * k : nullptr;
    const float psl = act_slope(a.prev_act);
#pragma unroll
    for (int i = 0; i < TPWK; ++i) {
        const int kk = (tb + w + 4 * i) * 32 + c32;
        const bool col_ok = kk < k;
        float s1 = 0.f, s2 = 0.f;
        if ((tb + w + 4 * i) * 32 >= k) continue;
        if (fast) {
            const int64_t rb = row0 + 4 * h;
            float* gp = a.g_prev + rb * k + kk;
            const float* zv = zpre[i];
            const float pm = pmean[i], pi = pinv[i];
            const bool drop = a.prev_drop_p > 0.f;
#pragma unroll
            for (int r = 0; r < 16; ++r) {
                const int lr = (r & 3) + 8 * (r >> 2);
                float gv = acc[i][r];
                if (drop) gv = dropout_keep(pseed, rb + lr, kk, a.prev_drop_p) ? gv * pscale : 0.f;
                if (col_ok) st_act(gp + lr * k, gv);
                const float xh = (act_pwl(psl, zv[r]) - pm) * pi;
                s1 += gv;
                s2 += gv * xh;
            }
            if (!want_stats || !col_ok) s1 = s2 = 0.f;
        } else if constexpr (FE == 0) {
#pragma unroll
        for (int r = 0; r < 16; ++r) {
            const int64_t gr = row0 + (r & 3) + 8 * (r >> 2) + 4 * h;
            if (gr < m && col_ok) {
                const float da = acc[i][r];
                if (a.dsrc) a.dsrc[gr * k + kk] = da;
                if (a.g_prev) {
                    float gv = da;
                    if (a.prev_drop_p > 0.f)
                        gv = dropout_keep(pseed, gr, kk, a.prev_drop_p) ? da * pscale : 0.f;
                    a.g_prev[gr * k + kk] = gv;
                    if (want_stats) {
                        const float xh = (act_eval(a.prev_act, a.src[gr * a.ld_src + kk]) -
                                          a.prev_mean[my_seg * k + kk]) * a.prev_invstd[my_seg * k + kk];
                        s1 += gv;
                        s2 += gv * xh;
                    }
                }
            }
        }
        }
        if (want_stats) {
            s1 += __shfl_xor(s1, 32, 64);
            s2 += __shfl_xor(s2, 32, 64);
            if (h == 0 && col_ok) {
                atomicAdd(&gps[kk], static_cast<double>(s1));
                atomicAdd(&gps[k + kk], static_cast<double>(s2));
            }
        }
    }
#ifndef RT_FOLD_FIRST
    fold_side(L, 0);
#endif
    RT_PP_END(2)
}

constexpr int DW_R = 32;
constexpr int DW_G = 2;
constexpr int DW_NT = 256 * DW_G;
constexpr int DW_MAXR = 2048;

__host__ __device__ constexpr int dw_ld(int x) { return x + ((x / 32) % 2 == 0 ? 32 : 0); }

template <int PRO>
__device__ __forceinline__ float pro_col(const Pro& p, float slope, int64_t r, int c, float sc, float sh, float v) {
    if constexpr (PRO == 0) {
        return v;
    } else {
        if constexpr (PRO == 3) v = act_eval(p.act, v);
        else v = act_pwl(slope, v);
        v = __builtin_fmaf(v, sc, sh);
        if constexpr (PRO == 2) v = dropout_keep(p.seed, r, c, p.drop_p) ? v * p.drop_scale : 0.f;
        if constexpr (PRO == 3) {
            if (p.drop_p > 0.f) v = dropout_keep(p.seed, r, c, p.drop_p) ? v * p.drop_scale : 0.f;
        }
        return v;
    }
}

__host__ __device__ constexpr int dw_lds_floats(int BN, int BK, int PRO, bool DZF) {
    return 2 * DW_R * dw_ld(BN) + 2 * DW_R * dw_ld(BK) + (PRO != 0 ? 4 * BK : 0) + (DZF ? 10 * BN : 0) + 4;
}

template <int BN, int BK, int PRO, bool VEC, bool DZF>
__device__ __forceinline__ void dw_tile(const rt_linear_bwd_args& a_set, const int64_t rows_per_split,
                                        const unsigned tn, const unsigned tk, const unsigned bid, float* smem) {
    constexpr int NTN = BN / 32, WK = 4 / NTN, T = (BK / 32) / WK;
    static_assert(NTN * 32 == BN && 4 % NTN == 0 && T >= 1 && T * WK * 32 == BK, "dW tile");
    constexpr int LDN = dw_ld(BN), LDK = dw_ld(BK);
    constexpr int VN = BN / 4, VK = BK / 4;
    constexpr int LN = (DW_R * VN + DW_NT - 1) / DW_NT, LK = (DW_R * VK + DW_NT - 1) / DW_NT;
    static_assert(DW_NT % VN == 0 && DW_NT % VK == 0, "fixed staging columns per thread");
    static_assert(2 * DW_R * LDN >= 4 * T * 16 * 64, "row-group reduction fits in the dz buffers");
    static_assert(2 * DW_R * LDK >= (DW_NT / 64) * VN * 4, "dbias partials fit in the A buffers");
    float* const Ld = smem;
    float* const La = Ld + 2 * DW_R * LDN;
    float* const aff_s = La + 2 * DW_R * LDK;
    float* const dzc_s = aff_s + (PRO != 0 ? 4 * BK : 0);
    int* const last_s = reinterpret_cast<int*>(dzc_s + (DZF ? 10 * BN : 0));
    int* const srow = last_s + 4;
    static_assert(dw_lds_floats(BN, BK, PRO, DZF) * sizeof(float) % 16 == 0, "16-B carve offsets");

    const rt_linear_bwd_args a = a_set;
    const unsigned bx = bid % tn, by = (bid / tn) % tk, bz = bid / (tn * tk);
    const int n = a.n, k = a.k;
    const int64_t m = a.m;
    const int tid = threadIdx.x, lane = tid & 63, wg = tid >> 6, w = wg & 3, grp = wg >> 2, h = lane >> 5,
              c = lane & 31;
    const int n0 = static_cast<int>(bx) * BN, k0 = static_cast<int>(by) * BK;
    const int64_t r_begin = static_cast<int64_t>(bz) * rows_per_split;
    const int64_t r_end = (r_begin + rows_per_split) < m ? (r_begin + rows_per_split) : m;
    if (r_begin >= m) return;
    RT_PP_DECL
    const bool gather = PRO == 0 && a.ids != nullptr && !a.a_in;
    const float* const asrc = a.a_in ? a.a_in : a.src;
    const int64_t ald = a.a_in ? static_cast<int64_t>(k) : static_cast<int64_t>(a.ld_src);
    const bool two = a.seg_split > 0;

    const int cn = (tid % VN) * 4, ck = (tid % VK) * 4;
    const int gn = n0 + cn, gk = k0 + ck;
    float4 sc0 = make_float4(1.f, 1.f, 1.f, 1.f), sc1 = sc0;
    float4 sh0 = make_float4(0.f, 0.f, 0.f, 0.f), sh1 = sh0;
    if (PRO != 0 && (a.prev_mode == 1 || a.prev_mode == 2) && !a.a_in) {
        if (tid < 2 * BK) {
            const int sg = tid / BK, cl = tid % BK, cc = k0 + cl;
            const int so = two ? sg * k : 0;
            float scv = 1.f, shv = 0.f;
            if (cc < k) bn_affine(a.prev_gamma[cc], a.prev_beta[cc], a.prev_mean[so + cc], a.prev_invstd[so + cc], scv, shv);
            aff_s[(sg * 2 + 0) * BK + cl] = scv;
            aff_s[(sg * 2 + 1) * BK + cl] = shv;
        }
        __syncthreads();
        sc0 = *reinterpret_cast<const float4*>(&aff_s[0 * BK + ck]);
        sh0 = *reinterpret_cast<const float4*>(&aff_s[1 * BK + ck]);
        sc1 = *reinterpret_cast<const float4*>(&aff_s[2 * BK + ck]);
        sh1 = *reinterpret_cast<const float4*>(&aff_s[3 * BK + ck]);
    }
    const uint64_t pseed = a.prev_drop_seed + (a.seed_offset ? *a.seed_offset : 0ull);
    const Pro pro{a.prev_mode, a.prev_act, a.prev_drop_p, a.prev_drop_p > 0.f ? 1.f / (1.f - a.prev_drop_p) : 1.f,
                  pseed, nullptr, nullptr};
    const float slope = act_slope(a.prev_act);
    if constexpr (DZF) {
        if (tid < 2 * BN) {
            const int sg = tid / BN, cl = tid % BN, c = n0 + cl;
            const int my = two ? sg : 0;
            const int64_t seg_m = two ? (my == 0 ? a.seg_split : m - a.seg_split) : m;
            float A = 1.f, Bc = 0.f, C = 0.f, M = 0.f, I = 1.f;
            if (c < n && (a.grad_mode == 1 || a.grad_mode == 2)) {
                I = a.save_invstd[my * n + c];
                M = a.save_mean[my * n + c];
                A = a.bn_gamma[c] * I;
                if (a.grad_mode == 1) {
                    double gs1, gs2;
                    slot_sums(a.g_stats + static_cast<int64_t>(my) * RT_STAT_SLOTS * 2 * n, n, c, gs1, gs2);
                    const float inv_m = 1.f / static_cast<float>(seg_m);
                    Bc = static_cast<float>(gs1) * inv_m;
                    C = static_cast<float>(gs2) * inv_m;
                }
            }
            float* const dc = dzc_s + sg * 5 * BN + cl;
            dc[0] = A; dc[BN] = Bc; dc[2 * BN] = C;
            dc[3 * BN] = M; dc[4 * BN] = I;
        }
        if (bid == 0 && (a.grad_mode == 1 || a.grad_mode == 2) && a.dgamma) {
            for (int c = tid; c < n; c += DW_NT) {
                for (int sg = 0; sg < (two ? 2 : 1); ++sg) {
                    double gs1, gs2;
                    slot_sums(a.g_stats + static_cast<int64_t>(sg) * RT_STAT_SLOTS * 2 * n, n, c, gs1, gs2);
                    atomicAdd(&a.dgamma[c], static_cast<float>(gs2));
                    atomicAdd(&a.dbeta[c], static_cast<float>(gs1));
                }
            }
        }
        __syncthreads();
    }
    if (!DZF && a.dbias && a.dbias_slots && bid == 0) {
        for (int cc = tid; cc < n; cc += DW_NT) {
            double v = 0.0;
#pragma unroll
            for (int sl = 0; sl < RT_STAT_SLOTS; ++sl) v += a.dbias_slots[static_cast<int64_t>(sl) * n + cc];
            atomicAdd(&a.dbias[cc], static_cast<float>(v));
        }
    }
    const bool do_bias = a.dbias != nullptr && (DZF || a.dbias_slots == nullptr) && by == 0;
    const bool slot_bias = DZF && do_bias && a.dbias_slots != nullptr;

    if (gather) {
        for (int64_t t = tid; t < r_end - r_begin; t += DW_NT) {
            const int64_t id = a.ids[r_begin + t];
            srow[t] = (id < 0 || id >= a.src_rows) ? -1 : static_cast<int>(id);
        }
        __syncthreads();
    }

    float4 rd[LN], rz[DZF ? LN : 1], ra[LK];
    float4 bsum = make_float4(0.f, 0.f, 0.f, 0.f);
    const float dsl = act_slope(a.act);
    auto load = [&](int64_t base) {
#pragma unroll
        for (int j = 0; j < LN; ++j) {
            const int e = tid + DW_NT * j, row = e / VN;
            const int64_t r = base + row;
            float4 v = make_float4(0.f, 0.f, 0.f, 0.f);
            if constexpr (DZF) {
                float4 zv = v;
                if (e < DW_R * VN && r < r_end && gn < n) {
                    v = *reinterpret_cast<const float4*>(a.g + r * n + gn);
                    zv = *reinterpret_cast<const float4*>(a.z + r * n + gn);
                }
                rd[j] = v;
                rz[j] = zv;
                continue;
            }
            if (e < DW_R * VN && r < r_end) {
                const float* dz = a.dz_ws + r * n + gn;
                if constexpr (VEC) {
                    if (gn < n) v = *reinterpret_cast<const float4*>(dz);
                } else {
                    if (gn < n) v.x = dz[0];
                    if (gn + 1 < n) v.y = dz[1];
                    if (gn + 2 < n) v.z = dz[2];
                    if (gn + 3 < n) v.w = dz[3];
                }
            }
            rd[j] = v;
        }
#pragma unroll
        for (int j = 0; j < LK; ++j) {
            const int e = tid + DW_NT * j, row = e / VK;
            const int64_t r = base + row;
            float4 v = make_float4(0.f, 0.f, 0.f, 0.f);
            if (e < DW_R * VK && r < r_end) {
                const int64_t sr = gather ? srow[r - r_begin] : r;
                if (sr >= 0) {
                    const float* ap = asrc + sr * ald + gk;
                    if constexpr (VEC) {
                        if (gk < k) v = *reinterpret_cast<const float4*>(ap);
                    } else {
                        if (gk < k) v.x = ap[0];
                        if (gk + 1 < k) v.y = ap[1];
                        if (gk + 2 < k) v.z = ap[2];
                        if (gk + 3 < k) v.w = ap[3];
                    }
                }
            }
            ra[j] = v;
        }
    };
    auto store = [&](int buf, int64_t base) {
#pragma unroll
        for (int j = 0; j < LN; ++j) {
            const int e = tid + DW_NT * j, row = e / VN;
            if (e < DW_R * VN) {
                if constexpr (DZF) {
                    const int64_t r = base + row;
                    const int sg = (two && r >= a.seg_split) ? 1 : 0;
                    const bool ok = r < r_end;
                    float4 d;
                    auto one = [&](float g, float z, int i) {
                        const int cl = cn + i;
                        const float* const dc = dzc_s + sg * 5 * BN + cl;
                        const float A = dc[0], Bc = dc[BN], C = dc[2 * BN];
                        const float M = dc[3 * BN], I = dc[4 * BN];
                        const float xh = (act_pwl(dsl, z) - M) * I;
                        return (ok && gn + i < n) ? A * (g - Bc - xh * C) * (z > 0.f ? 1.f : dsl) : 0.f;
                    };
                    d.x = one(rd[j].x, rz[j].x, 0);
                    d.y = one(rd[j].y, rz[j].y, 1);
                    d.z = one(rd[j].z, rz[j].z, 2);
                    d.w = one(rd[j].w, rz[j].w, 3);
                    rd[j] = d;
                }
                *reinterpret_cast<float4*>(&Ld[buf * DW_R * LDN + row * LDN + cn]) = rd[j];
                bsum.x += rd[j].x; bsum.y += rd[j].y; bsum.z += rd[j].z; bsum.w += rd[j].w;
            }
        }
#pragma unroll
        for (int j = 0; j < LK; ++j) {
            const int e = tid + DW_NT * j, row = e / VK;
            if (e < DW_R * VK) {
                const int64_t r = base + row;
                const bool ok = r < r_end && (!gather || srow[r - r_begin] >= 0);
                const bool hi_seg = two && r >= a.seg_split;
                const float4 scs = hi_seg ? sc1 : sc0, shs = hi_seg ? sh1 : sh0;
                float4 v;
                v.x = (ok && gk < k) ? pro_col<PRO>(pro, slope, r, gk, scs.x, shs.x, ra[j].x) : 0.f;
                v.y = (ok && gk + 1 < k) ? pro_col<PRO>(pro, slope, r, gk + 1, scs.y, shs.y, ra[j].y) : 0.f;
                v.z = (ok && gk + 2 < k) ? pro_col<PRO>(pro, slope, r, gk + 2, scs.z, shs.z, ra[j].z) : 0.f;
                v.w = (ok && gk + 3 < k) ? pro_col<PRO>(pro, slope, r, gk + 3, scs.w, shs.w, ra[j].w) : 0.f;
                *reinterpret_cast<float4*>(&La[buf * DW_R * LDK + row * LDK + ck]) = v;
            }
        }
    };

    f32x16 acc[T];
#pragma unroll
    for (int t = 0; t < T; ++t) acc[t] = f32x16{};
    const int ncol = (w % NTN) * 32 + c;
    const int kcol0 = (w / NTN) * T * 32 + c;
    int buf = 0;
    RT_PP_MARK(0)
    load(r_begin);
    store(0, r_begin);
    __syncthreads();
    RT_PP_MARK(1)
    for (int64_t base = r_begin; base < r_end; base += DW_R) {
        const bool more = base + DW_R < r_end;
        if (more) load(base + DW_R);
        const float* dl = &Ld[buf * DW_R * LDN + (2 * grp + h) * LDN + ncol];
        const float* al = &La[buf * DW_R * LDK + (2 * grp + h) * LDK + kcol0];
#pragma unroll
        for (int i = 0; i < DW_R / (2 * DW_G); ++i) {
            const float av = dl[2 * DW_G * i * LDN];
#pragma unroll
            for (int t = 0; t < T; ++t) acc[t] = mfma(av, al[2 * DW_G * i * LDK + 32 * t], acc[t]);
        }
        if (more) store(buf ^ 1, base + DW_R);
        __syncthreads();
        buf ^= 1;
    }

    RT_PP_MARK(2)
    float* red = Ld;
    float* bred = La;
    if (do_bias) {
#pragma unroll
        for (int o = VN; o < 64; o <<= 1) {
            bsum.x += __shfl_xor(bsum.x, o, 64);
            bsum.y += __shfl_xor(bsum.y, o, 64);
            bsum.z += __shfl_xor(bsum.z, o, 64);
            bsum.w += __shfl_xor(bsum.w, o, 64);
        }
        if (lane < VN) *reinterpret_cast<float4*>(&bred[(wg * VN + lane) * 4]) = bsum;
    }
#pragma unroll
    for (int t = 0; t < T; ++t)
#pragma unroll
        for (int r = 0; r < 16; ++r)
            if ((r >> 3) != grp) red[((w * T + t) * 16 + r) * 64 + lane] = acc[t][r];
    __syncthreads();
    if (do_bias && tid < VN) {
        float4 sb = make_float4(0.f, 0.f, 0.f, 0.f);
#pragma unroll
        for (int o = 0; o < DW_NT / 64; ++o) {
            const float4 v = *reinterpret_cast<const float4*>(&bred[(o * VN + tid) * 4]);
            sb.x += v.x; sb.y += v.y; sb.z += v.z; sb.w += v.w;
        }
        const int cb = n0 + tid * 4;
        if (slot_bias) {
            double* sl = a.dbias_slots + static_cast<int64_t>(bz % RT_STAT_SLOTS) * n;
            if (cb < n) atomicAdd(&sl[cb], static_cast<double>(sb.x));
            if (cb + 1 < n) atomicAdd(&sl[cb + 1], static_cast<double>(sb.y));
            if (cb + 2 < n) atomicAdd(&sl[cb + 2], static_cast<double>(sb.z));
            if (cb + 3 < n) atomicAdd(&sl[cb + 3], static_cast<double>(sb.w));
        } else {
            if (cb < n) atomicAdd(&a.dbias[cb], sb.x);
            if (cb + 1 < n) atomicAdd(&a.dbias[cb + 1], sb.y);
            if (cb + 2 < n) atomicAdd(&a.dbias[cb + 2], sb.z);
            if (cb + 3 < n) atomicAdd(&a.dbias[cb + 3], sb.w);
        }
    }
    auto add_row = [&](int t, int r, int kk) {
        const int nn = n0 + (w % NTN) * 32 + (r & 3) + 8 * (r >> 2) + 4 * h;
        const float v = acc[t][r] + red[((w * T + t) * 16 + r) * 64 + lane];
        if (nn < n) {
            if (a.dw_part) {
#ifdef RT_DW_PART_PLAIN
                a.dw_part[(static_cast<int64_t>(bz) * n + nn) * k + kk] = v;
#else
                st_act(a.dw_part + (static_cast<int64_t>(bz) * n + nn) * k + kk, v);
#endif
            }
            else atomicAdd(&a.dw[static_cast<int64_t>(nn) * k + kk], v);
        }
    };
#pragma unroll
    for (int t = 0; t < T; ++t) {
        const int kk = k0 + kcol0 + 32 * t;
        if (kk >= k) continue;
#pragma unroll
        for (int r = 0; r < 16; ++r)
            if ((r >> 3) == grp) add_row(t, r, kk);
    }
    if (slot_bias) {
        asm volatile("s_waitcnt vmcnt(0)" ::: "memory");
        __syncthreads();
        if (tid == 0) {
            ticket_release();
            unsigned long long* cnt = reinterpret_cast<unsigned long long*>(a.dbias_slots + static_cast<int64_t>(RT_STAT_SLOTS) * n);
            const unsigned long long nsplit = static_cast<unsigned long long>((m + rows_per_split - 1) / rows_per_split);
            *last_s = atomicAdd(&cnt[bx], 1ull) == nsplit - 1 ? 1 : 0;
        }
        __syncthreads();
        if (*last_s) {
            for (int cl = tid; cl < BN; cl += DW_NT) {
                const int c = n0 + cl;
                if (c >= n) continue;
                double v = 0.0;
#pragma unroll
                for (int sl = 0; sl < RT_STAT_SLOTS; ++sl) v += atomicAdd(&a.dbias_slots[static_cast<int64_t>(sl) * n + c], 0.0);
                atomicAdd(&a.dbias[c], static_cast<float>(v));
            }
        }
    }
    RT_PP_END(3)
}

extern __shared__ __attribute__((aligned(16))) float dw_smem[];

template <int BN, int BK, int PRO, bool VEC, bool DZF>
__global__ __launch_bounds__(DW_NT) void linear_bwd_dw_kernel(BwdLaunch L) {
#ifdef RT_FOLD_FIRST
    fold_side(L, 1);
#endif
    const bool g1 = blockIdx.x >= L.split;
    dw_tile<BN, BK, PRO, VEC, DZF>(g1 ? L.a1 : L.a0, g1 ? L.rps1 : L.rps0, g1 ? L.tn1 : L.tn0, g1 ? L.tk1 : L.tk0,
                                   blockIdx.x - (g1 ? L.split : 0u), dw_smem);
#ifndef RT_FOLD_FIRST
    fold_side(L, 1);
#endif
}

constexpr int DWJ_MAX = 6;
struct DwJointLaunch {
    rt_linear_bwd_args a[DWJ_MAX];
    int64_t rps[DWJ_MAX];
    unsigned tn[DWJ_MAX], tk[DWJ_MAX], end[DWJ_MAX];
    unsigned char body[DWJ_MAX];
    int nsets;
};
template <bool VS>
__global__ __launch_bounds__(DW_NT) void linear_bwd_dw_joint_kernel(DwJointLaunch L) {
    int s = 0;
    while (s + 1 < L.nsets && blockIdx.x >= L.end[s]) ++s;
    const unsigned bid = blockIdx.x - (s ? L.end[s - 1] : 0u);
    if (L.body[s] == 0) dw_tile<128, 32, 0, VS, true>(L.a[s], L.rps[s], L.tn[s], L.tk[s], bid, dw_smem);
    else dw_tile<64, 64, 0, true, false>(L.a[s], L.rps[s], L.tn[s], L.tk[s], bid, dw_smem);
}

}
}

using namespace rt;

template <auto Kernel>
static void allow_lds(size_t bytes) {
    static size_t set = 0;
    if (bytes > set) {
        (void)hipFuncSetAttribute(reinterpret_cast<const void*>(Kernel), hipFuncAttributeMaxDynamicSharedMemorySize,
                            static_cast<int>(bytes));
        set = bytes;
    }
}

static int validate_fwd(const rt_linear_fwd_args* args) {
    if (!args) return RT_ERR_INVALID;
    const rt_linear_fwd_args& a = *args;
    if (a.m < 0 || a.k <= 0 || a.n <= 0 || !a.src || !a.w || a.ld_src < a.k) return RT_ERR_INVALID;
    if (a.n > 512 || a.k > 8192) return RT_ERR_UNSUPPORTED;
    if (a.prev_mode < 0 || a.prev_mode > 3) return RT_ERR_INVALID;
    if (a.seg_split < 0 || (a.seg_split > 0 && (a.seg_split >= a.m || a.seg_split % mlp::FM != 0)))
        return RT_ERR_INVALID;
    if (a.prev_mode == 1 && (!a.prev_stats || !a.bn_gamma || !a.bn_beta)) return RT_ERR_INVALID;
    if (a.prev_mode == 2 && (!a.running_mean || !a.running_var || !a.bn_gamma || !a.bn_beta)) return RT_ERR_INVALID;
    if (a.a_out && ((a.k % 4) != 0 || (reinterpret_cast<uintptr_t>(a.a_out) & 15) != 0)) return RT_ERR_INVALID;
    if (a.fin_save_mean && (!a.stats_out || !a.fin_save_invstd || (!a.fin_running_mean != !a.fin_running_var)))
        return RT_ERR_INVALID;
    if (a.prev_final && (a.prev_mode != 1 || !a.save_mean || !a.save_invstd)) return RT_ERR_INVALID;
    if (a.w_planes && ((a.k % 8) != 0 || a.n > 128 || (reinterpret_cast<uintptr_t>(a.w_planes) & 15) ||
                       (reinterpret_cast<uintptr_t>(a.w) & 15)))
        return RT_ERR_INVALID;
    if (a.next_w_planes && (!a.next_w || a.next_n <= 0 || a.next_k <= 0 || (a.next_k % 8) != 0 ||
                            (reinterpret_cast<uintptr_t>(a.next_w) & 15) ||
                            (reinterpret_cast<uintptr_t>(a.next_w_planes) & 15)))
        return RT_ERR_INVALID;
    const int kp = mlp::pad8(a.k);
    const int tpw = a.n <= 128 ? 1 : a.n <= 256 ? 2 : 4;
    const size_t lds = (2 * kp + 3 * mlp::FM * kp / 2 + 4 * tpw * mlp::FM) * sizeof(float) + mlp::FM * sizeof(int64_t) + 16;
    if (lds > 160 * 1024) return RT_ERR_UNSUPPORTED;
    return RT_OK;
}

extern "C" int rt_linear_fwd_f32_multi(const rt_linear_fwd_args* args, int n_args, void* stream) {
    if (!args || n_args < 1 || n_args > 2) return RT_ERR_INVALID;
#ifdef RT_NO_AIN
    rt_linear_fwd_args noa[2];
    for (int g = 0; g < n_args; ++g) { noa[g] = args[g]; noa[g].a_out = nullptr; }
    args = noa;
#endif
    int tpw = 1, kp_max = 0;
    bool kvec = true, wpl = true;
    unsigned blocks[2] = {0u, 0u};
    for (int g = 0; g < n_args; ++g) {
        const int v = validate_fwd(&args[g]);
        if (v) return v;
        const rt_linear_fwd_args& a = args[g];
        wpl = wpl && a.w_planes != nullptr;
        const int t = a.n <= 128 ? 1 : a.n <= 256 ? 2 : 4;
        tpw = t > tpw ? t : tpw;
        kvec = kvec && (a.k % 4) == 0 && (reinterpret_cast<uintptr_t>(a.w) & 15) == 0;
        const int kp = mlp::pad8(a.k);
        kp_max = kp > kp_max ? kp : kp_max;
        blocks[g] = static_cast<unsigned>((a.m + mlp::FM - 1) / mlp::FM);
    }
    const size_t lds = (2 * kp_max + 3 * mlp::FM * kp_max / 2 + 4 * tpw * mlp::FM) * sizeof(float) +
                       mlp::FM * sizeof(int64_t) + 16;
    if (lds > 160 * 1024) return RT_ERR_UNSUPPORTED;
    mlp::FwdLaunch L{};
    L.a0 = args[0];
    L.a1 = n_args > 1 ? args[1] : args[0];
    L.split = blocks[0];
    const unsigned total = blocks[0] + (n_args > 1 ? blocks[1] : 0u);
    if (total == 0) return RT_OK;
    hipStream_t st = as_stream(stream);
    const dim3 grid(total);
#define RT_FWD(T, V, P)                                                                           \
    do {                                                                                          \
        allow_lds<mlp::linear_fwd_kernel<T, V, P>>(lds);                                          \
        hipLaunchKernelGGL((mlp::linear_fwd_kernel<T, V, P>), grid, dim3(256), lds, st, L);       \
    } while (0)
    if (kvec && tpw == 1 && wpl) {
        RT_FWD(1, true, true);
    } else if (kvec) {
        if (tpw == 1) RT_FWD(1, true, false); else if (tpw == 2) RT_FWD(2, true, false); else RT_FWD(4, true, false);
    } else {
        if (tpw == 1) RT_FWD(1, false, false); else if (tpw == 2) RT_FWD(2, false, false); else RT_FWD(4, false, false);
    }
#undef RT_FWD
    return check_launch("linear_fwd_kernel");
}

extern "C" int rt_linear_fwd_f32(const rt_linear_fwd_args* args, void* stream) {
    return rt_linear_fwd_f32_multi(args, 1, stream);
}

static bool dz_fusable(const rt_linear_bwd_args& a) {
#ifdef RT_NO_DZ_FUSE
    return false;
#endif
    return a.fuse_dz && !a.g_prev && !a.dsrc && a.grad_mode >= 1 && a.grad_mode <= 3 &&
           act_is_piecewise_linear(a.act) && (a.n % 4) == 0 && a.g && a.z &&
           (reinterpret_cast<uintptr_t>(a.g) & 15) == 0 && (reinterpret_cast<uintptr_t>(a.z) & 15) == 0;
}
static bool all_dz_fusable(const rt_linear_bwd_args* args, int n_args) {
    for (int g = 0; g < n_args; ++g)
        if (!dz_fusable(args[g])) return false;
    return true;
}

static int dz_fast_class(const rt_linear_bwd_args& a) {
#if defined(RT_DZ_NO_FE) || defined(RT_NO_WT_ROWS)
    return 0;
#endif
    if (!a.wt || (a.n % 8) != 0) return 0;
    if ((a.m % mlp::FM) != 0 || !mlp::dz_da_fast(a)) return 0;
    if (a.grad_mode == 0) return mlp::dz_norm_fast(a.n) ? 1 : 0;
    return ((a.grad_mode == 1 || a.grad_mode == 2) && mlp::dz_bn_fast(a.n, a.act, a.grad_mode)) ? 2 : 0;
}

static int validate_bwd(const rt_linear_bwd_args* args) {
    if (!args) return RT_ERR_INVALID;
    const rt_linear_bwd_args& a = *args;
    if (a.m < 0 || a.k <= 0 || a.n <= 0 || !a.w || !a.dw || !a.dz_ws || !a.src || a.ld_src < a.k)
        return RT_ERR_INVALID;
    const bool need_da = a.g_prev || a.dsrc;
    if (a.n > 2048 || (need_da && a.k > 512)) return RT_ERR_UNSUPPORTED;
    if (a.grad_mode == 0 && (!a.dout || !a.l2_out || !a.norms)) return RT_ERR_INVALID;
    if (a.grad_mode >= 1 && a.grad_mode <= 3 && (!a.g || !a.z)) return RT_ERR_INVALID;
    if ((a.grad_mode == 1 || a.grad_mode == 2) && (!a.g_stats || !a.save_mean || !a.save_invstd || !a.bn_gamma))
        return RT_ERR_INVALID;
    if (a.grad_mode < 0 || a.grad_mode > 3) return RT_ERR_INVALID;
    if (a.seg_split < 0 || (a.seg_split > 0 && (a.seg_split >= a.m || a.seg_split % mlp::FM != 0)))
        return RT_ERR_INVALID;
    if ((a.prev_mode == 1 || a.prev_mode == 2) &&
        (!a.prev_mean || !a.prev_invstd || !a.prev_gamma || !a.prev_beta))
        return RT_ERR_INVALID;
    if (a.fold_src && (!a.fold_dst || a.fold_words % 4 != 0 || a.fold_splits <= 0 || a.fold_in < 0 || a.fold_in > 1 ||
                       (reinterpret_cast<uintptr_t>(a.fold_src) & 15) || (reinterpret_cast<uintptr_t>(a.fold_dst) & 15)))
        return RT_ERR_INVALID;
    if (a.wt_planes && ((a.n % 8) != 0 || (reinterpret_cast<uintptr_t>(a.wt_planes) & 15))) return RT_ERR_INVALID;
    return RT_OK;
}

extern "C" int rt_linear_bwd_dz_f32_multi(const rt_linear_bwd_args* args, int n_args, void* stream) {
    if (!args || n_args < 1 || n_args > 2) return RT_ERR_INVALID;
    int tpwk = 1;
    size_t lds = 0;
    unsigned blocks[2] = {0u, 0u};
    bool wpl = true;
    int fe = -1;
    for (int g = 0; g < n_args; ++g) {
        const int v = validate_bwd(&args[g]);
        if (v) return v;
        const rt_linear_bwd_args& a = args[g];
        const bool need_da = a.g_prev || a.dsrc;
        const int fc = dz_fast_class(a);
        fe = (fe < 0 || fe == fc) ? fc : 0;
        wpl = wpl && (!need_da || a.wt_planes != nullptr);
        const int t = !need_da ? 1 : a.k <= 128 ? 1 : a.k <= 256 ? 2 : 4;
        tpwk = t > tpwk ? t : tpwk;
        const int np = mlp::pad8(a.n);
        const size_t l = (static_cast<size_t>(mlp::FM) * (np + 4) + 5 * static_cast<size_t>(np)) * sizeof(float) +
                         3 * static_cast<size_t>(mlp::FM) * (np + 8) * sizeof(uint16_t) + 16;
        lds = l > lds ? l : lds;
        blocks[g] = static_cast<unsigned>((a.m + mlp::FM - 1) / mlp::FM);
    }
    if (all_dz_fusable(args, n_args)) {
        for (int g = 0; g < n_args; ++g)
            if (args[g].fold_src && args[g].fold_in == 0) return RT_ERR_INVALID;
        return RT_OK;
    }
    mlp::BwdLaunch L{};
    L.a0 = args[0];
    L.a1 = n_args > 1 ? args[1] : args[0];
    L.ngroups = n_args;
    L.split = blocks[0];
    const unsigned total = blocks[0] + (n_args > 1 ? blocks[1] : 0u);
    if (total == 0) return RT_OK;
    bool any_da = false;
    for (int g = 0; g < n_args; ++g) any_da = any_da || args[g].g_prev || args[g].dsrc;
    static const int ks_env = [] { const char* e = getenv("RT_DZ_KSPLIT"); return e ? atoi(e) : 0; }();
    unsigned ks = (tpwk == 2 && any_da && total <= 256u) ? 2u : 1u;
    if (ks_env == 1 || (ks_env == 2 && tpwk == 2 && any_da)) ks = static_cast<unsigned>(ks_env);
    L.ksplit = ks;
    if (ks == 2) tpwk = 1;
    const dim3 grid(total * ks);
    hipStream_t st = as_stream(stream);
#define RT_DZ(T, P, K, F)                                                                        \
    do {                                                                                         \
        allow_lds<mlp::linear_bwd_dz_kernel<T, P, K, F>>(lds);                                   \
        hipLaunchKernelGGL((mlp::linear_bwd_dz_kernel<T, P, K, F>), grid, dim3(256), lds, st, L); \
    } while (0)
    if (ks > 1) {
        if (wpl) RT_DZ(1, true, true, 0); else RT_DZ(1, false, true, 0);
    } else {
        switch (tpwk) {
            case 1:
                if (wpl) RT_DZ(1, true, false, 0);
                else if (fe == 1) RT_DZ(1, false, false, 1);
                else RT_DZ(1, false, false, 0);
                break;
            case 2:
                if (wpl) RT_DZ(2, true, false, 0);
                else if (fe == 1) RT_DZ(2, false, false, 1);
                else if (fe == 2) RT_DZ(2, false, false, 2);
                else RT_DZ(2, false, false, 0);
                break;
            default: RT_DZ(4, false, false, 0); break;
        }
    }
#undef RT_DZ
    return check_launch("linear_bwd_dz_kernel");
}

extern "C" int rt_linear_bwd_dz_fused(const rt_linear_bwd_args* args, int n_args) {
    return (args && n_args >= 1 && n_args <= 2 && all_dz_fusable(args, n_args)) ? 1 : 0;
}

extern "C" int rt_linear_bwd_dz_f32(const rt_linear_bwd_args* args, void* stream) {
    return rt_linear_bwd_dz_f32_multi(args, 1, stream);
}

#ifndef RT_DW_BLOCKS
#define RT_DW_BLOCKS 384
#endif
#ifndef RT_DW_BLOCKS_SMALLK
#define RT_DW_BLOCKS_SMALLK 256
#endif
#ifndef RT_DW_CAP_SMALLK
#define RT_DW_CAP_SMALLK 128
#endif
static void dw_plan(const rt_linear_bwd_args* args, int n_args, bool small_k, unsigned* tn, unsigned* tk,
                    int64_t* splits, int64_t& rps, int64_t target_blocks = 0, int64_t split_cap = 0) {
    const int bn = small_k ? 128 : 64, bk = small_k ? 32 : 64;
    const int64_t cap = split_cap > 0 ? split_cap : small_k ? RT_DW_CAP_SMALLK : 64;
    int64_t work = 0, rmin = mlp::DW_R;
    for (int g = 0; g < n_args; ++g) {
        const rt_linear_bwd_args& a = args[g];
        tn[g] = static_cast<unsigned>((a.n + bn - 1) / bn);
        tk[g] = static_cast<unsigned>((a.k + bk - 1) / bk);
        work += a.m * tn[g] * tk[g];
        const int64_t r = (a.m + cap - 1) / cap;
        rmin = r > rmin ? r : rmin;
    }
    const int64_t target = target_blocks > 0 ? target_blocks : small_k ? RT_DW_BLOCKS_SMALLK : RT_DW_BLOCKS;
    rps = (work + target - 1) / target;
    rps = rps > rmin ? rps : rmin;
    rps = (rps + mlp::DW_R - 1) / mlp::DW_R * mlp::DW_R;
    for (int g = 0; g < n_args; ++g)
        if (args[g].ids && rps > mlp::DW_MAXR) rps = mlp::DW_MAXR;
    for (int g = 0; g < n_args; ++g) splits[g] = args[g].m > 0 ? (args[g].m + rps - 1) / rps : 0;
}

static int dw_prologue(const rt_linear_bwd_args& a) {
    if (a.prev_mode == 0 || a.a_in) return 0;
    return !act_is_piecewise_linear(a.prev_act) ? 3 : (a.prev_drop_p > 0.f ? 2 : 1);
}
static bool dw_mixed(const rt_linear_bwd_args* args, int n_args) {
    return n_args == 2 && (dw_prologue(args[0]) == 0) != (dw_prologue(args[1]) == 0);
}

static bool dw_vec(const rt_linear_bwd_args& a) {
    const float* asrc = a.a_in ? a.a_in : a.src;
    const int ald = a.a_in ? a.k : a.ld_src;
    return (a.n % 4) == 0 && (a.k % 4) == 0 && (ald % 4) == 0 && (reinterpret_cast<uintptr_t>(asrc) & 15) == 0 &&
           (reinterpret_cast<uintptr_t>(a.dz_ws) & 15) == 0;
}

static int dw_launch(const rt_linear_bwd_args* args, int n_args, bool dzf, hipStream_t st) {
    mlp::BwdLaunch L{};
    unsigned blocks[2] = {0u, 0u};
    int pro = -1;
    bool small_k = true;
    for (int g = 0; g < n_args; ++g) small_k = small_k && args[g].k <= 32;
    unsigned tns[2] = {1u, 1u}, tks[2] = {1u, 1u};
    int64_t nsplit[2] = {0, 0}, rps = mlp::DW_R;
    dw_plan(args, n_args, small_k, tns, tks, nsplit, rps);
    for (int g = 0; g < n_args; ++g) {
        const rt_linear_bwd_args& a = args[g];
        const int64_t nb = static_cast<int64_t>(tns[g]) * tks[g] * nsplit[g];
        if (nb > (1ll << 30)) return RT_ERR_UNSUPPORTED;
        blocks[g] = static_cast<unsigned>(nb);
        (g ? L.tn1 : L.tn0) = tns[g] ? tns[g] : 1u;
        (g ? L.tk1 : L.tk0) = tks[g] ? tks[g] : 1u;
        (g ? L.rps1 : L.rps0) = rps;
        const int p = dw_prologue(a);
        pro = p > pro ? p : pro;
        (g ? L.vec1 : L.vec0) = dw_vec(a);
    }
    L.a0 = args[0];
    L.a1 = n_args > 1 ? args[1] : args[0];
    L.ngroups = n_args;
    if (n_args == 1) { L.tn1 = L.tn0; L.tk1 = L.tk0; L.rps1 = L.rps0; L.vec1 = L.vec0; }
    L.split = blocks[0];
    const unsigned total = blocks[0] + (n_args > 1 ? blocks[1] : 0u);
    if (total == 0) return RT_OK;
    const dim3 grid(total);
    const bool vec = L.vec0 && L.vec1;
    size_t id_bytes = 0;
    for (int g = 0; g < n_args; ++g)
        if (args[g].ids && !args[g].a_in) id_bytes = static_cast<size_t>(rps) * sizeof(int);
#define RT_DW(BN, BK, P)                                                                                                 \
    do {                                                                                                                 \
        const size_t lds = mlp::dw_lds_floats(BN, BK, P, dzf) * sizeof(float) + id_bytes;                                \
        if (dzf) {                                                                                                       \
            if (vec) hipLaunchKernelGGL((mlp::linear_bwd_dw_kernel<BN, BK, P, true, true>), grid, dim3(mlp::DW_NT), lds, st, L);  \
            else hipLaunchKernelGGL((mlp::linear_bwd_dw_kernel<BN, BK, P, false, true>), grid, dim3(mlp::DW_NT), lds, st, L);     \
        } else {                                                                                                         \
            if (vec) hipLaunchKernelGGL((mlp::linear_bwd_dw_kernel<BN, BK, P, true, false>), grid, dim3(mlp::DW_NT), lds, st, L); \
            else hipLaunchKernelGGL((mlp::linear_bwd_dw_kernel<BN, BK, P, false, false>), grid, dim3(mlp::DW_NT), lds, st, L);    \
        }                                                                                                                \
    } while (0)
    if (small_k) {
        switch (pro) { case 0: RT_DW(128, 32, 0); break; case 1: RT_DW(128, 32, 1); break;
                       case 2: RT_DW(128, 32, 2); break; default: RT_DW(128, 32, 3); }
    } else {
        switch (pro) { case 0: RT_DW(64, 64, 0); break; case 1: RT_DW(64, 64, 1); break;
                       case 2: RT_DW(64, 64, 2); break; default: RT_DW(64, 64, 3); }
    }
#undef RT_DW
    return check_launch("linear_bwd_dw_kernel");
}

extern "C" int rt_linear_bwd_dw_f32_multi(const rt_linear_bwd_args* args, int n_args, void* stream) {
    if (!args || n_args < 1 || n_args > 2) return RT_ERR_INVALID;
#ifdef RT_NO_AIN
    rt_linear_bwd_args noa[2];
    for (int g = 0; g < n_args; ++g) { noa[g] = args[g]; noa[g].a_in = nullptr; }
    args = noa;
#endif
    for (int g = 0; g < n_args; ++g) {
        const int v = validate_bwd(&args[g]);
        if (v) return v;
        if (args[g].ids && args[g].prev_mode != 0) return RT_ERR_UNSUPPORTED;
    }
    hipStream_t st = as_stream(stream);
    const bool dzf = all_dz_fusable(args, n_args);
    if (dw_mixed(args, n_args)) {
        const int r0 = dw_launch(&args[0], 1, dzf, st);
        return r0 ? r0 : dw_launch(&args[1], 1, dzf, st);
    }
    return dw_launch(args, n_args, dzf, st);
}

extern "C" int rt_linear_bwd_dw_splits(const rt_linear_bwd_args* args, int n_args, int64_t* splits) {
    if (!args || !splits || n_args < 1 || n_args > 2) return RT_ERR_INVALID;
#ifdef RT_NO_DW_PART
    return RT_ERR_UNSUPPORTED;
#endif
    bool small_k = true;
    for (int g = 0; g < n_args; ++g) {
        const int v = validate_bwd(&args[g]);
        if (v) return v;
        small_k = small_k && args[g].k <= 32;
    }
    unsigned tns[2] = {1u, 1u}, tks[2] = {1u, 1u};
    int64_t nsplit[2] = {0, 0}, rps = mlp::DW_R;
    if (dw_mixed(args, n_args)) {
        for (int g = 0; g < 2; ++g) {
            dw_plan(&args[g], 1, args[g].k <= 32, tns, tks, nsplit, rps);
            splits[g] = nsplit[0];
        }
        return RT_OK;
    }
    dw_plan(args, n_args, small_k, tns, tks, nsplit, rps);
    for (int g = 0; g < n_args; ++g) splits[g] = nsplit[g];
    return RT_OK;
}

extern "C" int rt_linear_bwd_dw_f32(const rt_linear_bwd_args* args, void* stream) {
    return rt_linear_bwd_dw_f32_multi(args, 1, stream);
}

static int dwj_body(const rt_linear_bwd_args& a) {
    if (dw_prologue(a) != 0) return -1;
    if (a.k <= 32) return dz_fusable(a) ? 0 : -1;
    return (!dz_fusable(a) && dw_vec(a) && !(a.ids && !a.a_in)) ? 1 : -1;
}

#ifndef RT_DWJ_SLOTS
#define RT_DWJ_SLOTS 512
#endif
#ifndef RT_DWJ_BLOCKS_SMALLK
#define RT_DWJ_BLOCKS_SMALLK 128
#endif
#ifndef RT_DWJ_CAP_SMALLK
#define RT_DWJ_CAP_SMALLK 64
#endif
#ifndef RT_DWJ_MIN_BLOCKS
#define RT_DWJ_MIN_BLOCKS 128
#endif
struct DwJointPlan {
    int body[mlp::DWJ_MAX];
    unsigned tn[mlp::DWJ_MAX], tk[mlp::DWJ_MAX];
    int64_t splits[mlp::DWJ_MAX], rps[mlp::DWJ_MAX];
};
static void dwj_plan(const rt_linear_bwd_args* args, int n_args, DwJointPlan& P) {
    rt_linear_bwd_args small[mlp::DWJ_MAX];
    int small_of[mlp::DWJ_MAX], ns = 0;
    for (int g = 0; g < n_args; ++g) {
        P.body[g] = dwj_body(args[g]);
        P.tn[g] = P.tk[g] = 1u;
        P.splits[g] = 0;
        P.rps[g] = mlp::DW_R;
        if (P.body[g] == 0) { small_of[ns] = g; small[ns++] = args[g]; }
    }
    int64_t blocks_small = 0;
    if (ns) {
        unsigned tn[mlp::DWJ_MAX], tk[mlp::DWJ_MAX];
        int64_t sp[mlp::DWJ_MAX], rps = mlp::DW_R;
        dw_plan(small, ns, true, tn, tk, sp, rps, RT_DWJ_BLOCKS_SMALLK, RT_DWJ_CAP_SMALLK);
        for (int i = 0; i < ns; ++i) {
            const int g = small_of[i];
            P.tn[g] = tn[i]; P.tk[g] = tk[i]; P.splits[g] = sp[i]; P.rps[g] = rps;
            blocks_small += static_cast<int64_t>(tn[i]) * tk[i] * sp[i];
        }
    }
    int64_t work = 0, rmax = mlp::DW_R;
    for (int g = 0; g < n_args; ++g) {
        if (P.body[g] != 1) continue;
        P.tn[g] = static_cast<unsigned>((args[g].n + 63) / 64);
        P.tk[g] = static_cast<unsigned>((args[g].k + 63) / 64);
        work += args[g].m * P.tn[g] * P.tk[g];
        rmax = args[g].m > rmax ? args[g].m : rmax;
    }
    if (work > 0) {
        int64_t target = RT_DWJ_SLOTS - blocks_small;
        target = target > RT_DWJ_MIN_BLOCKS ? target : RT_DWJ_MIN_BLOCKS;
        int64_t rps = (work + target - 1) / target;
        rps = (rps + mlp::DW_R - 1) / mlp::DW_R * mlp::DW_R;
        rmax = (rmax + mlp::DW_R - 1) / mlp::DW_R * mlp::DW_R;
        for (;; rps += mlp::DW_R) {
            int64_t blocks = 0;
            for (int g = 0; g < n_args; ++g)
                if (P.body[g] == 1) blocks += ((args[g].m + rps - 1) / rps) * P.tn[g] * P.tk[g];
            if (blocks <= target || rps >= rmax) break;
        }
        for (int g = 0; g < n_args; ++g)
            if (P.body[g] == 1) { P.rps[g] = rps; P.splits[g] = args[g].m > 0 ? (args[g].m + rps - 1) / rps : 0; }
    }
    for (int g = 0; g < n_args; ++g) {
        if (P.body[g] >= 0) continue;
        int64_t sp = 0;
        dw_plan(&args[g], 1, args[g].k <= 32, &P.tn[g], &P.tk[g], &sp, P.rps[g]);
        P.splits[g] = sp;
    }
}

static int dwj_validate(const rt_linear_bwd_args* args, int n_args) {
    if (!args || n_args < 1 || n_args > mlp::DWJ_MAX) return RT_ERR_INVALID;
    for (int g = 0; g < n_args; ++g) {
        const int v = validate_bwd(&args[g]);
        if (v) return v;
        if (args[g].ids && args[g].prev_mode != 0) return RT_ERR_UNSUPPORTED;
        if (args[g].fold_src && args[g].fold_in == 1) return RT_ERR_INVALID;
    }
    return RT_OK;
}

#ifdef RT_NO_AIN
#define RT_DWJ_NO_AIN(args, n_args)                                                        \
    rt_linear_bwd_args noa[mlp::DWJ_MAX];                                                  \
    for (int g = 0; g < n_args; ++g) { noa[g] = args[g]; noa[g].a_in = nullptr; }          \
    args = noa;
#else
#define RT_DWJ_NO_AIN(args, n_args)
#endif

extern "C" int rt_linear_bwd_dw_joint_splits(const rt_linear_bwd_args* args, int n_args, int64_t* splits) {
    if (!splits) return RT_ERR_INVALID;
    const int v = dwj_validate(args, n_args);
    if (v) return v;
#ifdef RT_NO_DW_PART
    return RT_ERR_UNSUPPORTED;
#endif
    RT_DWJ_NO_AIN(args, n_args)
    DwJointPlan P;
    dwj_plan(args, n_args, P);
    for (int g = 0; g < n_args; ++g) splits[g] = P.splits[g];
    return RT_OK;
}

extern "C" int rt_linear_bwd_dw_f32_joint(const rt_linear_bwd_args* args, int n_args, void* stream) {
    const int v = dwj_validate(args, n_args);
    if (v) return v;
    RT_DWJ_NO_AIN(args, n_args)
    DwJointPlan P;
    dwj_plan(args, n_args, P);
    hipStream_t st = as_stream(stream);
    mlp::DwJointLaunch L{};
    bool vs = true;
    size_t lds = 0;
    int64_t total = 0;
    for (int body = 0; body < 2; ++body) {
        for (int g = 0; g < n_args; ++g) {
            if (P.body[g] != body) continue;
            const int64_t nb = static_cast<int64_t>(P.tn[g]) * P.tk[g] * P.splits[g];
            if (nb == 0) continue;
            total += nb;
            if (total > (1ll << 30)) return RT_ERR_UNSUPPORTED;
            const int s = L.nsets++;
            L.a[s] = args[g];
            L.rps[s] = P.rps[g];
            L.tn[s] = P.tn[g];
            L.tk[s] = P.tk[g];
            L.end[s] = static_cast<unsigned>(total);
            L.body[s] = static_cast<unsigned char>(body);
            size_t need = mlp::dw_lds_floats(body ? 64 : 128, body ? 64 : 32, 0, body == 0) * sizeof(float);
            if (body == 0) {
                vs = vs && dw_vec(args[g]);
                if (args[g].ids && !args[g].a_in) need += static_cast<size_t>(P.rps[g]) * sizeof(int);
            }
            lds = need > lds ? need : lds;
        }
    }
    if (total > 0) {
        const dim3 grid(static_cast<unsigned>(total));
        if (vs) hipLaunchKernelGGL(mlp::linear_bwd_dw_joint_kernel<true>, grid, dim3(mlp::DW_NT), lds, st, L);
        else hipLaunchKernelGGL(mlp::linear_bwd_dw_joint_kernel<false>, grid, dim3(mlp::DW_NT), lds, st, L);
        const int rc = check_launch("linear_bwd_dw_joint_kernel");
        if (rc) return rc;
    }
    for (int g = 0; g < n_args; ++g) {
        if (P.body[g] >= 0) continue;
        const int rc = dw_launch(&args[g], 1, dz_fusable(args[g]), st);
        if (rc) return rc;
    }
    return RT_OK;
}

#ifdef RT_PHASE_PROBE
extern "C" int rt_probe_setup(void* buf, unsigned cap) {
    unsigned long long* p = static_cast<unsigned long long*>(buf);
    const unsigned zero[64] = {};
    if (hipMemcpyToSymbol(HIP_SYMBOL(mlp::g_probe_buf), &p, sizeof(p)) != hipSuccess) return RT_ERR_HIP;
    if (hipMemcpyToSymbol(HIP_SYMBOL(mlp::g_probe_cap), &cap, sizeof(cap)) != hipSuccess) return RT_ERR_HIP;
    if (hipMemcpyToSymbol(HIP_SYMBOL(mlp::g_probe_ctr), zero, sizeof(zero)) != hipSuccess) return RT_ERR_HIP;
    return RT_OK;
}
extern "C" int rt_probe_count(unsigned* out) {
    return hipMemcpyFromSymbol(out, HIP_SYMBOL(mlp::g_probe_ctr), 64 * sizeof(unsigned)) == hipSuccess ? RT_OK
                                                                                                       : RT_ERR_HIP;
}
#endif

extern "C" int rt_linear_bwd_f32(const rt_linear_bwd_args* args, void* stream) {
    const int rc = rt_linear_bwd_dz_f32(args, stream);
    return rc ? rc : rt_linear_bwd_dw_f32(args, stream);
}
```

### real-time-recommendation-system-with-feature-store_amd/rtrec_amd/models/fused.py

```python
from __future__ import annotations

import ctypes
import itertools
import os
from dataclasses import dataclass, field
from typing import List, Optional

import torch
import torch.nn as nn

from .. import native
from ..native import LinearBwdArgs, LinearFwdArgs, call, ptr
from ..profiling import TIMER

ACT_CODE = {nn.ReLU: 0, nn.GELU: 1, nn.LeakyReLU: 2, nn.Tanh: 3, nn.Sigmoid: 4}
ACT_NONE = 5

_seed_counter = itertools.count(1)


def act_code(mod: Optional[nn.Module]) -> int:
    if mod is None:
        return ACT_NONE
    for cls, code in ACT_CODE.items():
        if isinstance(mod, cls):
            if cls is nn.LeakyReLU and abs(mod.negative_slope - 0.1) > 1e-12:
                raise NotImplementedError("LeakyReLU slope other than 0.1 (two_tower.py:82)")
            return code
    raise NotImplementedError(f"activation {type(mod).__name__}")


@dataclass
class Block:
    linear: nn.Linear
    act: int = ACT_NONE
    bn: Optional[nn.BatchNorm1d] = None
    drop: Optional[nn.Dropout] = None

    def drop_p(self) -> float:
        return float(self.drop.p) if (self.drop is not None and self.drop.training and self.drop.p > 0) else 0.0

    def bn_mode(self) -> int:
        if self.bn is None:
            return 3
        return 1 if self.bn.training else 2


def blocks_from_sequential(seq: nn.Sequential) -> List[Block]:
    mods = list(seq)
    blocks: List[Block] = []
    i = 0
    while i < len(mods):
        lin = mods[i]
        if not isinstance(lin, nn.Linear):
            raise NotImplementedError(f"unexpected module {type(lin).__name__} at {i}")
        b = Block(lin)
        i += 1
        if i < len(mods) and not isinstance(mods[i], (nn.Linear, nn.BatchNorm1d, nn.Dropout)):
            b.act = act_code(mods[i])
            i += 1
        if i < len(mods) and isinstance(mods[i], nn.BatchNorm1d):
            b.bn = mods[i]
            i += 1
        if i < len(mods) and isinstance(mods[i], nn.Dropout):
            b.drop = mods[i]
            i += 1
        blocks.append(b)
    return blocks


class ParamSlab:

    def __init__(self, module: nn.Module):
        self.module = module
        self.params: List[nn.Parameter] = []
        self.data: Optional[torch.Tensor] = None
        self.grad: Optional[torch.Tensor] = None
        self.offsets: List[int] = []
        self.offsets_dev: Optional[torch.Tensor] = None
        self.grad_gen = 0

    def _valid(self) -> bool:
        ps = [p for p in self.module.parameters()]
        if self.data is None or len(ps) != len(self.params) or any(a is not b for a, b in zip(ps, self.params)):
            return False
        base = self.data.data_ptr()
        for p, off in zip(self.params, self.offsets):
            if p.device != self.data.device or p.data_ptr() != base + off * 4:
                return False
        return True

    def ensure(self) -> "ParamSlab":
        if self._valid():
            return self
        ps = list(self.module.parameters())
        if not ps:
            raise ValueError("module has no parameters")
        dev = ps[0].device
        for p in ps:
            if p.dtype != torch.float32 or p.device != dev:
                raise TypeError("parameter slab needs fp32 parameters on one device")
        sizes = [p.numel() for p in ps]
        offs, cur = [], 0
        for s in sizes:
            offs.append(cur)
            cur += (s + 3) // 4 * 4
        data = torch.zeros(cur, dtype=torch.float32, device=dev)
        grad = torch.zeros(cur, dtype=torch.float32, device=dev)
        with torch.no_grad():
            for p, o, s in zip(ps, offs, sizes):
                data[o:o + s].copy_(p.data.reshape(-1))
        for p, o, s in zip(ps, offs, sizes):
            p.data = data[o:o + s].view(p.shape)
            old = p.grad
            p.grad = grad[o:o + s].view(p.shape)
            if old is not None:
                p.grad.copy_(old)
        self.params, self.offsets, self.data, self.grad = ps, offs, data, grad
        self.grad_gen += 1
        self.__dict__["_grad_views"] = {}
        ends = [o + s for o, s in zip(offs, sizes)]
        self.bounds = list(zip(offs, ends))
        self.offsets_dev = None
        return self

    def attach_grads(self):
        self.ensure()
        self.grad_gen += 1
        for p, (o, e) in zip(self.params, self.bounds):
            view = self.grad[o:e]
            if p.grad is None:
                view.zero_()
                p.grad = view.view(p.shape)
            elif p.grad.data_ptr() != view.data_ptr():
                view.copy_(p.grad.reshape(-1))
                p.grad = view.view(p.shape)

    def grad_of(self, p: torch.Tensor) -> torch.Tensor:
        cache = self.__dict__.setdefault("_grad_views", {})
        v = cache.get(id(p))
        if v is not None and v[0] is p and v[1].data_ptr() >= self.grad.data_ptr():
            return v[1]
        for q, (o, e) in zip(self.params, self.bounds):
            if q is p:
                view = self.grad[o:e].view(p.shape)
                cache[id(p)] = (p, view)
                return view
        raise KeyError("parameter not in slab")

    def tensor_offsets(self) -> torch.Tensor:
        if self.offsets_dev is None:
            b = [o for o, _ in self.bounds] + [self.bounds[-1][1]]
            self.offsets_dev = torch.tensor(b, dtype=torch.int64, device=self.data.device)
        return self.offsets_dev


@dataclass
class ChainCtx:
    m: int
    src: torch.Tensor
    ids: Optional[torch.Tensor]
    zs: List[Optional[torch.Tensor]] = field(default_factory=list)
    save_mean: List[Optional[torch.Tensor]] = field(default_factory=list)
    save_invstd: List[Optional[torch.Tensor]] = field(default_factory=list)
    seeds: List[int] = field(default_factory=list)
    drop_ps: List[float] = field(default_factory=list)
    bn_modes: List[int] = field(default_factory=list)
    out: Optional[torch.Tensor] = None
    norms: Optional[torch.Tensor] = None
    normalize: bool = True
    seg_split: int = 0
    wts: List[Optional[torch.Tensor]] = field(default_factory=list)
    w_planes: List[Optional[torch.Tensor]] = field(default_factory=list)
    wt_planes: List[Optional[torch.Tensor]] = field(default_factory=list)
    ains: List[Optional[torch.Tensor]] = field(default_factory=list)


def _stream(t: torch.Tensor):
    return ctypes.c_void_p(torch.cuda.current_stream(t.device).cuda_stream)


STAT_SLOTS = 16
DBIAS_ROWS = STAT_SLOTS + 1
FINALIZE_BN_IN_PRODUCER = os.environ.get("RTREC_BN_FINAL", "0") == "1"
_WPL = os.environ.get("RTREC_W_PLANES", "0")
SPLIT_W_PLANES = _WPL in ("1", "fwd", "dz")
SPLIT_W_PLANES_FWD = _WPL in ("1", "fwd")
SPLIT_W_PLANES_DZ = _WPL in ("1", "dz")


def stats_arena_size(blocks: List[Block], n_seg: int = 1) -> int:
    return max(1, n_seg * STAT_SLOTS * 2 * sum(b.linear.out_features for b in blocks[:-1])
               + DBIAS_ROWS * sum(b.linear.out_features for b in blocks))


def _zero_on_entry(layer, zero_buf: Optional[torch.Tensor]):
    if zero_buf is not None:
        layer.zero_buf = zero_buf.data_ptr()
        layer.zero_words = zero_buf.numel()


def chain_forward(blocks: List[Block], src: torch.Tensor, ids: Optional[torch.Tensor] = None,
                  normalize: bool = True, seed_offset: Optional[torch.Tensor] = None,
                  stats_arena: Optional[torch.Tensor] = None, seg_split: int = 0,
                  zero_buf: Optional[torch.Tensor] = None, seed_base: Optional[int] = None) -> ChainCtx:
    ctx, layers = _forward_plan(blocks, src, ids, normalize, seed_offset, stats_arena, seg_split, seed_base)
    _zero_on_entry(layers[0], zero_buf)
    st = _stream(src)
    for a in layers:
        _launch_fwd([a], st)
    return ctx


def chain_forward_pair(first: tuple, second: tuple, zero_buf: Optional[torch.Tensor] = None) -> tuple:
    c1, l1 = _forward_plan(*first)
    c2, l2 = _forward_plan(*second)
    _zero_on_entry(l1[0], zero_buf)
    st = _stream(first[1])
    if len(l1) == len(l2):
        for a, b in zip(l1, l2):
            _launch_fwd([a, b], st)
    else:
        for a in l1 + l2:
            _launch_fwd([a], st)
    return c1, c2


def _launch_fwd(group: list, st) -> None:
    flops = sum(2.0 * a.m * a.k * a.n for a in group)
    nbytes = sum(4.0 * (a.m * a.k + a.n * a.k + a.m * a.n) for a in group)
    with TIMER.region("linear_fwd", flops=flops, bytes_=nbytes):
        if len(group) == 1:
            call("rt_linear_fwd_f32", ctypes.byref(group[0]), st)
        else:
            arr = (LinearFwdArgs * len(group))(*group)
            call("rt_linear_fwd_f32_multi", arr, len(group), st)


def layer_seed(seed_base: int, layer: int) -> int:
    z = (seed_base * 0x100000001B3 + (layer + 1) * 0x9E3779B97F4A7C15) & 0xFFFFFFFFFFFFFFFF
    z = ((z ^ (z >> 30)) * 0xBF58476D1CE4E5B9) & 0xFFFFFFFFFFFFFFFF
    z = ((z ^ (z >> 27)) * 0x94D049BB133111EB) & 0xFFFFFFFFFFFFFFFF
    return z ^ (z >> 31)


def _forward_plan(blocks: List[Block], src: torch.Tensor, ids: Optional[torch.Tensor] = None,
                  normalize: bool = True, seed_offset: Optional[torch.Tensor] = None,
                  stats_arena: Optional[torch.Tensor] = None, seg_split: int = 0,
                  seed_base: Optional[int] = None):
    native.require_device(src, what="tower forward")
    if src.dtype != torch.float32:
        raise TypeError("tower input must be fp32 (the reference towers are fp32)")
    src = src.contiguous()
    m = int(ids.numel()) if ids is not None else int(src.shape[0])
    if ids is not None:
        ids = ids.contiguous().to(torch.int64)
    dev = src.device
    L = len(blocks) - 1
    k0 = blocks[0].linear.in_features
    if src.dim() != 2 or src.shape[1] != k0:
        raise RuntimeError(f"mat1 and mat2 shapes cannot be multiplied ({m}x{src.shape[-1]} and "
                           f"{k0}x{blocks[0].linear.out_features})")
    n_seg = 2 if seg_split else 1
    if seg_split and (seg_split % 32 != 0 or not 0 < seg_split < m):
        raise ValueError("seg_split must be a multiple of 32 inside (0, m)")
    seg_rows = [seg_split, m - seg_split] if seg_split else [m]
    for b in blocks[:-1]:
        if b.bn is not None and b.bn.training and min(seg_rows) <= 1:
            raise ValueError("Expected more than 1 value per channel when training (BatchNorm1d)")
    ctx = ChainCtx(m=m, src=src, ids=ids, normalize=normalize, seg_split=seg_split)
    widths = [b.linear.out_features for b in blocks[:-1]]
    if stats_arena is None:
        stats_arena = torch.zeros(stats_arena_size(blocks, n_seg), dtype=torch.float64, device=dev)
    stats, off = [], 0
    for wdt in widths:
        stats.append(stats_arena[off:off + n_seg * STAT_SLOTS * 2 * wdt])
        off += n_seg * STAT_SLOTS * 2 * wdt
    layers = []
    cur_src, cur_ids, ld = src, ids, src.shape[1]
    for li, b in enumerate(blocks):
        lin = b.linear
        a = LinearFwdArgs()
        a.src = cur_src.data_ptr()
        a.src_rows = cur_src.shape[0]
        a.ld_src = ld
        a.ids = cur_ids.data_ptr() if cur_ids is not None else None
        a.m = m
        a.k = lin.in_features
        a.n = lin.out_features
        a.w = lin.weight.data_ptr()
        a.bias = lin.bias.data_ptr() if lin.bias is not None else None
        a.seed_offset = seed_offset.data_ptr() if seed_offset is not None else None
        a.seg_split = seg_split
        if li == 0:
            a.prev_mode = 0
        else:
            pb = blocks[li - 1]
            a.prev_mode = pb.bn_mode()
            a.prev_act = pb.act
            a.drop_p = pb.drop_p()
            a.drop_seed = ctx.seeds[li - 1]
            if pb.bn is not None:
                a.prev_stats = stats[li - 1].data_ptr()
                a.bn_gamma = pb.bn.weight.data_ptr()
                a.bn_beta = pb.bn.bias.data_ptr()
                a.running_mean = pb.bn.running_mean.data_ptr()
                a.running_var = pb.bn.running_var.data_ptr()
                sm = torch.empty(n_seg * lin.in_features, dtype=torch.float32, device=dev)
                si = torch.empty(n_seg * lin.in_features, dtype=torch.float32, device=dev)
                ctx.save_mean[li - 1], ctx.save_invstd[li - 1] = sm, si
                a.save_mean = sm.data_ptr()
                a.save_invstd = si.data_ptr()
                a.bn_eps = float(pb.bn.eps)
                a.bn_momentum = float(pb.bn.momentum if pb.bn.momentum is not None else 0.1)
                if pb.bn.training and pb.bn.num_batches_tracked is not None:
                    a.num_batches_tracked = pb.bn.num_batches_tracked.data_ptr()
                prod = layers[li - 1]
                if a.prev_mode == 1 and prod.stats_out and FINALIZE_BN_IN_PRODUCER:
                    prod.fin_save_mean, prod.fin_save_invstd = a.save_mean, a.save_invstd
                    prod.fin_running_mean, prod.fin_running_var = a.running_mean, a.running_var
                    prod.fin_num_batches_tracked = a.num_batches_tracked
                    prod.fin_eps, prod.fin_momentum = a.bn_eps, a.bn_momentum
                    a.prev_final = 1
        a.act = b.act
        wt = wtp = None
        if li > 0 and lin.training:
            if SPLIT_W_PLANES and SPLIT_W_PLANES_DZ and lin.out_features % 8 == 0:
                wtp = torch.empty((3, lin.in_features, lin.out_features), dtype=torch.int16, device=dev)
                a.wt_planes_out = wtp.data_ptr()
            else:
                wt = torch.empty((lin.in_features, lin.out_features), dtype=torch.float32, device=dev)
                a.wt_out = wt.data_ptr()
        ctx.wts.append(wt)
        ctx.wt_planes.append(wtp)
        wp = None
        if SPLIT_W_PLANES and SPLIT_W_PLANES_FWD and li > 0 and lin.in_features % 8 == 0 and lin.out_features <= 128:
            wp = torch.empty((3, lin.out_features, lin.in_features), dtype=torch.int16, device=dev)
            prev = layers[li - 1]
            prev.next_w = lin.weight.data_ptr()
            prev.next_w_planes = wp.data_ptr()
            prev.next_n, prev.next_k = lin.out_features, lin.in_features
            a.w_planes = wp.data_ptr()
        ctx.w_planes.append(wp)
        ain = None
        if li > 0 and lin.training and lin.in_features % 4 == 0:
            ain = torch.empty((m, lin.in_features), dtype=torch.float32, device=dev)
            a.a_out = ain.data_ptr()
        ctx.ains.append(ain)
        if li < L:
            z = torch.empty((m, lin.out_features), dtype=torch.float32, device=dev)
            a.z_out = z.data_ptr()
            if b.bn is not None and b.bn.training:
                a.stats_out = stats[li].data_ptr()
            ctx.zs.append(z)
            ctx.save_mean.append(None)
            ctx.save_invstd.append(None)
            ctx.seeds.append(layer_seed(seed_base, li) if seed_base is not None else
                             next(_seed_counter) * 0x9E3779B97F4A7C15 & 0xFFFFFFFFFFFFFFFF)
            ctx.drop_ps.append(b.drop_p())
            ctx.bn_modes.append(b.bn_mode())
            cur_src, cur_ids, ld = z, None, lin.out_features
        else:
            out = torch.empty((m, lin.out_features), dtype=torch.float32, device=dev)
            if normalize:
                norms = torch.empty(m, dtype=torch.float32, device=dev)
                a.l2_out = out.data_ptr()
                a.norms_out = norms.data_ptr()
                ctx.norms = norms
            else:
                a.z_out = out.data_ptr()
            ctx.out = out
        layers.append(a)
    return ctx, layers


def chain_backward(blocks: List[Block], ctx: ChainCtx, dout: torch.Tensor, slab: ParamSlab,
                   want_dsrc: bool = False, seed_offset: Optional[torch.Tensor] = None,
                   stats_arena: Optional[torch.Tensor] = None, attach: bool = True) -> Optional[torch.Tensor]:
    layers, dsrc, keep = _backward_plan(blocks, ctx, dout, slab, want_dsrc, seed_offset, stats_arena, attach)
    st = _stream(dout)
    groups = [[a] for a in layers]
    if dw_joint_enabled():
        _launch_bwd_joint(groups, st, None)
        return dsrc
    keep += _plan_partials(groups, dout.device)
    for g in groups:
        _launch_bwd(g, st)
    return dsrc


def chain_backward_pair(first: tuple, second: tuple, fold_sink: Optional["FoldSink"] = None) -> None:
    l1, _, keep1 = _backward_plan(*first)
    l2, _, keep2 = _backward_plan(*second)
    st = _stream(first[2])
    if len(l1) == len(l2):
        groups = [[a, b] for a, b in zip(l1, l2)]
        if dw_joint_enabled():
            _launch_bwd_joint(groups, st, fold_sink)
            return
        keep1 += _plan_partials(groups, first[2].device)
    else:
        groups = [[a] for a in l1 + l2]
    for g in groups:
        _launch_bwd(g, st)


def dw_joint_enabled() -> bool:
    lib = native.lib()
    return (os.environ.get("RTREC_DW_LEGACY", "0") != "1" and hasattr(lib, "rt_linear_bwd_dw_f32_joint")
            and hasattr(lib, "rt_linear_bwd_dw_joint_splits") and hasattr(lib, "rt_linear_bwd_dz_fused"))


class FoldSink:

    def __init__(self, slab: ParamSlab):
        self.slab = slab
        self.buf: Optional[torch.Tensor] = None
        self.retired: list = []
        self.folds: list = []

    def begin(self) -> None:
        self.folds = []

    def place(self, sets: list, splits: list) -> None:
        grad = self.slab.grad
        index = {o: i for i, o in enumerate(self.slab.offsets)}
        plan, total = [], 0
        for a, sp in zip(sets, splits):
            words = a.n * a.k
            off = (a.dw - grad.data_ptr()) // 4
            if sp < 1 or words % 4 or off not in index or len(plan) >= native.GRAD_FOLD_MAX:
                continue
            plan.append((a, sp, words, off, total))
            total += sp * words
        if self.buf is None or self.buf.numel() < total:
            if self.buf is not None:
                self.retired.append(self.buf)
            self.buf = torch.empty(max(total, 64), dtype=torch.float32, device=grad.device)
        base = self.buf.data_ptr()
        for a, sp, words, off, start in plan:
            a.dw_part = base + 4 * start
            self.folds.append(native.GradFold(a.dw_part, off, words, sp, index[off]))


def _launch_bwd_joint(groups: list, st, sink: Optional[FoldSink]) -> None:
    lib = native.lib()
    for g in groups:
        arr = (LinearBwdArgs * len(g))(*g)
        if lib.rt_linear_bwd_dz_fused(arr, len(g)):
            continue
        for a in g:
            a.fuse_dz = 0
        _launch_dz(g, st)
    sets = [a for g in groups for a in g]
    chunks = [sets[i:i + native.DW_JOINT_MAX] for i in range(0, len(sets), native.DW_JOINT_MAX)]
    if sink is not None:
        cand = {id(a) for g in groups[:-1] for a in g}
        part_sets, part_splits = [], []
        for ch in chunks:
            splits = (ctypes.c_int64 * len(ch))()
            if lib.rt_linear_bwd_dw_joint_splits((LinearBwdArgs * len(ch))(*ch), len(ch), splits) != 0:
                continue
            for a, sp in zip(ch, splits):
                if id(a) in cand:
                    part_sets.append(a)
                    part_splits.append(int(sp))
        sink.place(part_sets, part_splits)
    with TIMER.region("linear_bwd_dw", flops=sum(2.0 * a.m * a.k * a.n for a in sets),
                      bytes_=sum(4.0 * (a.m * a.n + a.m * a.k + a.n * a.k) for a in sets)):
        for ch in chunks:
            call("rt_linear_bwd_dw_f32_joint", (LinearBwdArgs * len(ch))(*ch), len(ch), st)


def _plan_partials(groups: list, dev) -> list:
    lib = native.lib()
    if not hasattr(lib, "rt_linear_bwd_dw_splits"):
        return []
    keep = []
    for gi in range(len(groups) - 1):
        grp, nxt = groups[gi], groups[gi + 1]
        if len(grp) != len(nxt):
            continue
        arr = (LinearBwdArgs * len(grp))(*grp)
        splits = (ctypes.c_int64 * len(grp))()
        if lib.rt_linear_bwd_dw_splits(arr, len(grp), splits) != 0:
            continue
        narr = (LinearBwdArgs * len(nxt))(*nxt)
        fold_in = 1 if lib.rt_linear_bwd_dz_fused(narr, len(nxt)) else 0
        for a, b, sp in zip(grp, nxt, splits):
            words = a.n * a.k
            if sp < 1 or words % 4 or b.fold_src:
                continue
            part = torch.empty(sp * words, dtype=torch.float32, device=dev)
            keep.append(part)
            a.dw_part = part.data_ptr()
            b.fold_src, b.fold_dst, b.fold_words = part.data_ptr(), a.dw, words
            b.fold_splits, b.fold_in = sp, fold_in
    return keep


def _launch_bwd(group: list, st) -> None:
    arr = (LinearBwdArgs * len(group))(*group)
    lib = native.lib()
    fused = hasattr(lib, "rt_linear_bwd_dz_fused") and lib.rt_linear_bwd_dz_fused(arr, len(group))
    if not fused:
        _launch_dz(group, st)
    _launch_dw(group, st)


def _launch_dz(group: list, st) -> None:
    da = [a.g_prev is not None or a.dsrc is not None for a in group]
    flops = sum((2.0 if d else 0.0) * a.m * a.k * a.n for a, d in zip(group, da))
    nbytes = sum(4.0 * (3 * a.m * a.n + (2 * a.m * a.k if d else 0) + a.n * a.k) for a, d in zip(group, da))
    with TIMER.region("linear_bwd_dz", flops=flops, bytes_=nbytes):
        call("rt_linear_bwd_dz_f32_multi", (LinearBwdArgs * len(group))(*group), len(group), st)


def _launch_dw(group: list, st) -> None:
    with TIMER.region("linear_bwd_dw", flops=sum(2.0 * a.m * a.k * a.n for a in group),
                      bytes_=sum(4.0 * (a.m * a.n + a.m * a.k + a.n * a.k) for a in group)):
        call("rt_linear_bwd_dw_f32_multi", (LinearBwdArgs * len(group))(*group), len(group), st)


def _backward_plan(blocks: List[Block], ctx: ChainCtx, dout: torch.Tensor, slab: ParamSlab,
                   want_dsrc: bool = False, seed_offset: Optional[torch.Tensor] = None,
                   stats_arena: Optional[torch.Tensor] = None, attach: bool = True):
    dev = dout.device
    dout = dout.contiguous()
    m = ctx.m
    L = len(blocks) - 1
    if attach:
        slab.attach_grads()
    dz_bufs = [torch.empty((m, b.linear.out_features), dtype=torch.float32, device=dev) for b in blocks]
    layers = []
    widths = [b.linear.out_features for b in blocks[:-1]]
    n_seg = 2 if ctx.seg_split else 1
    gst_arena = stats_arena if stats_arena is not None else \
        torch.zeros(stats_arena_size(blocks, n_seg), dtype=torch.float64, device=dev)
    gstats, off = [], 0
    for wdt in widths:
        gstats.append(gst_arena[off:off + n_seg * STAT_SLOTS * 2 * wdt])
        off += n_seg * STAT_SLOTS * 2 * wdt
    bslots = []
    for b in blocks:
        bslots.append(gst_arena[off:off + DBIAS_ROWS * b.linear.out_features])
        off += DBIAS_ROWS * b.linear.out_features
    gs: List[Optional[torch.Tensor]] = [None] * L
    dsrc = torch.empty((m, blocks[0].linear.in_features), dtype=torch.float32, device=dev) if want_dsrc else None
    keep = [dout, gst_arena] + dz_bufs
    for li in range(L, -1, -1):
        b = blocks[li]
        lin = b.linear
        a = LinearBwdArgs()
        a.m, a.k, a.n = m, lin.in_features, lin.out_features
        a.w = lin.weight.data_ptr()
        a.dw = slab.grad_of(lin.weight).data_ptr()
        a.dbias = slab.grad_of(lin.bias).data_ptr() if lin.bias is not None else None
        a.dbias_slots = bslots[li].data_ptr() if lin.bias is not None else None
        a.dz_ws = dz_bufs[li].data_ptr()
        a.seed_offset = seed_offset.data_ptr() if seed_offset is not None else None
        a.seg_split = ctx.seg_split
        if li == L:
            if ctx.normalize:
                a.grad_mode = 0
                a.dout = dout.data_ptr()
                a.l2_out = ctx.out.data_ptr()
                a.norms = ctx.norms.data_ptr()
            else:
                a.grad_mode = 3
                a.g = dout.data_ptr()
                a.z = dout.data_ptr()
                a.act = ACT_NONE
        else:
            a.grad_mode = ctx.bn_modes[li]
            a.g = gs[li].data_ptr()
            a.z = ctx.zs[li].data_ptr()
            a.act = b.act
            if b.bn is not None:
                a.g_stats = gstats[li].data_ptr()
                a.save_mean = ctx.save_mean[li].data_ptr()
                a.save_invstd = ctx.save_invstd[li].data_ptr()
                a.bn_gamma = b.bn.weight.data_ptr()
                a.dgamma = slab.grad_of(b.bn.weight).data_ptr()
                a.dbeta = slab.grad_of(b.bn.bias).data_ptr()
        if li == 0 and not want_dsrc:
            a.fuse_dz = 1
        if li == 0:
            a.src = ctx.src.data_ptr()
            a.src_rows = ctx.src.shape[0]
            a.ld_src = ctx.src.shape[1]
            a.ids = ctx.ids.data_ptr() if ctx.ids is not None else None
            a.prev_mode = 0
            if want_dsrc:
                if ctx.ids is not None:
                    raise NotImplementedError("input gradient through a fused gather")
                a.dsrc = dsrc.data_ptr()
        else:
            pb = blocks[li - 1]
            a.src = ctx.zs[li - 1].data_ptr()
            a.src_rows = m
            a.ld_src = pb.linear.out_features
            a.prev_mode = ctx.bn_modes[li - 1]
            a.prev_act = pb.act
            a.prev_drop_p = ctx.drop_ps[li - 1]
            a.prev_drop_seed = ctx.seeds[li - 1]
            if pb.bn is not None:
                a.prev_mean = ctx.save_mean[li - 1].data_ptr()
                a.prev_invstd = ctx.save_invstd[li - 1].data_ptr()
                a.prev_gamma = pb.bn.weight.data_ptr()
                a.prev_beta = pb.bn.bias.data_ptr()
                a.g_prev_stats = gstats[li - 1].data_ptr()
            g = torch.empty((m, pb.linear.out_features), dtype=torch.float32, device=dev)
            gs[li - 1] = g
            keep.append(g)
            a.g_prev = g.data_ptr()
            if li < len(ctx.wts) and ctx.wts[li] is not None:
                a.wt = ctx.wts[li].data_ptr()
            if li < len(ctx.wt_planes) and ctx.wt_planes[li] is not None:
                a.wt_planes = ctx.wt_planes[li].data_ptr()
            if li < len(ctx.ains) and ctx.ains[li] is not None:
                a.a_in = ctx.ains[li].data_ptr()
        layers.append(a)
    return layers, dsrc, keep
```

### real-time-recommendation-system-with-feature-store_amd/rtrec_amd/native.py

```python
from __future__ import annotations

import ctypes
import os
import threading
from typing import Optional

import torch

PKG_DIR = os.path.dirname(os.path.dirname(os.path.abspath(__file__)))
LIB_PATH = os.environ.get("RTREC_HIP_LIB", os.path.join(PKG_DIR, "lib", "librtrec_hip.so"))

RT_F32, RT_F16, RT_BF16 = 0, 1, 2
ACTS = {"relu": 0, "gelu": 1, "leaky_relu": 2, "tanh": 3, "sigmoid": 4, "none": 5}

c_i64 = ctypes.c_int64
c_int = ctypes.c_int
c_f32 = ctypes.c_float
c_u64 = ctypes.c_uint64
c_size = ctypes.c_size_t
vp = ctypes.c_void_p


class NativeUnavailable(RuntimeError):
    """librtrec_hip.so is missing or unusable (no CPU fallback exists)."""


class RTError(RuntimeError):

    def __init__(self, what: str, status: int, message: str):
        super().__init__(f"{what} failed: {message} (status {status})")
        self.status = status


class LinearFwdArgs(ctypes.Structure):
    _fields_ = [
        ("src", vp), ("src_rows", c_i64), ("ld_src", c_int), ("ids", vp), ("m", c_i64), ("k", c_int),
        ("n", c_int), ("w", vp), ("bias", vp),
        ("prev_mode", c_int), ("prev_act", c_int), ("prev_stats", vp), ("bn_gamma", vp), ("bn_beta", vp),
        ("running_mean", vp), ("running_var", vp), ("save_mean", vp), ("save_invstd", vp),
        ("bn_eps", c_f32), ("bn_momentum", c_f32), ("drop_p", c_f32), ("drop_seed", c_u64),
        ("seed_offset", vp), ("z_out", vp), ("act", c_int), ("stats_out", vp), ("l2_out", vp), ("norms_out", vp),
        ("num_batches_tracked", vp), ("seg_split", c_i64), ("zero_buf", vp), ("zero_words", c_i64),
        ("wt_out", vp), ("a_out", vp),
        ("fin_save_mean", vp), ("fin_save_invstd", vp), ("fin_running_mean", vp), ("fin_running_var", vp),
        ("fin_num_batches_tracked", vp), ("fin_eps", c_f32), ("fin_momentum", c_f32), ("prev_final", c_int),
        ("w_planes", vp), ("wt_planes_out", vp), ("next_w", vp), ("next_w_planes", vp), ("next_n", c_int),
        ("next_k", c_int),
    ]


class LinearBwdArgs(ctypes.Structure):
    _fields_ = [
        ("m", c_i64), ("k", c_int), ("n", c_int), ("w", vp), ("dw", vp), ("dbias", vp), ("dz_ws", vp),
        ("grad_mode", c_int), ("dout", vp), ("l2_out", vp), ("norms", vp),
        ("g", vp), ("z", vp), ("act", c_int), ("g_stats", vp), ("save_mean", vp), ("save_invstd", vp),
        ("bn_gamma", vp), ("dgamma", vp), ("dbeta", vp),
        ("src", vp), ("src_rows", c_i64), ("ld_src", c_int), ("ids", vp),
        ("prev_mode", c_int), ("prev_act", c_int), ("prev_mean", vp), ("prev_invstd", vp),
        ("prev_gamma", vp), ("prev_beta", vp), ("prev_drop_p", c_f32), ("prev_drop_seed", c_u64),
        ("seed_offset", vp), ("g_prev", vp), ("g_prev_stats", vp), ("dsrc", vp), ("seg_split", c_i64),
        ("dbias_slots", vp), ("wt", vp), ("fuse_dz", c_int), ("a_in", vp), ("dw_part", vp),
        ("fold_src", vp), ("fold_dst", vp), ("fold_words", c_i64), ("fold_splits", c_int), ("fold_in", c_int),
        ("wt_planes", vp),
    ]


class GradFold(ctypes.Structure):
    _fields_ = [("part", vp), ("dst_off", c_i64), ("words", c_i64), ("splits", c_int), ("tensor", c_int)]


TOWER_MAX_LAYERS, TOWER_MAX_ROWS, TOWER_MAX_WIDTH = 8, 8, 512


class TowerLayer(ctypes.Structure):
    _fields_ = [("w", vp), ("bias", vp), ("k", c_int), ("n", c_int), ("act", c_int), ("bn_gamma", vp),
                ("bn_beta", vp), ("bn_mean", vp), ("bn_var", vp), ("bn_eps", c_f32)]


class TowerInferArgs(ctypes.Structure):
    _fields_ = [("src", vp), ("src_rows", c_i64), ("ld_src", c_int), ("ids", vp), ("m", c_int),
                ("n_layers", c_int), ("layers", TowerLayer * TOWER_MAX_LAYERS), ("normalize", c_int),
                ("out", vp), ("norms_out", vp)]


ONLINE_MAX_EXCL_SOURCES = 2


class ExclusionLists(ctypes.Structure):
    _fields_ = [("offsets", vp), ("items", vp), ("n_rows", c_i64), ("rows", vp)]


GRAD_FOLD_MAX = 8
DW_JOINT_MAX = 6


SIGNATURES = {
    "rt_abi_version": (c_int, []),
    "rt_status_string": (ctypes.c_char_p, [c_int]),
    "rt_last_error": (ctypes.c_char_p, []),
    "rt_gather_rows": (c_int, [vp, c_i64, c_i64, c_i64, vp, c_i64, vp, vp, vp]),
    "rt_scatter_add_rows_f32": (c_int, [vp, c_i64, c_int, vp, c_i64, vp, c_i64, vp]),
    "rt_scatter_rows": (c_int, [vp, c_i64, c_i64, vp, vp, c_i64, vp, vp]),
    "rt_rows_compact_workspace_bytes": (c_size, [c_i64]),
    "rt_rows_compact": (c_int, [vp, c_i64, c_i64, vp, c_i64, vp, c_i64, vp, vp, c_size, vp]),
    "rt_l2_renorm_f32": (c_int, [vp, c_i64, c_int, vp]),
    "rt_flatip_topk_workspace_bytes": (c_size, [c_i64, c_i64, c_int, c_int, c_int]),
    "rt_flatip_topk": (c_int, [vp, c_i64, vp, c_i64, c_int, c_int, c_int, vp, c_i64, c_i64, vp, vp, vp,
                               c_size, vp]),
    "rt_flatip_topk_online_workspace_bytes": (c_size, [c_i64, c_i64, c_int, c_int, c_int]),
    "rt_flatip_topk_online_plan": (c_int, [c_i64, c_i64, c_int, c_int, c_int, vp]),
    "rt_flatip_topk_online": (c_int, [vp, c_i64, vp, c_i64, c_int, c_int, c_int, vp, c_i64, c_i64, vp, vp, vp,
                                      c_size, vp]),
    "rt_flatip_topk_online_lists": (c_int, [vp, c_i64, vp, c_i64, c_int, c_int, c_int,
                                            ctypes.POINTER(ExclusionLists), c_int, c_i64, vp, vp, vp, c_size, vp]),
    "rt_ivf_topk_tuning": (c_int, [c_int]),
    "rt_ivf_topk_plan": (c_int, [c_i64, c_int, c_i64, vp]),
    "rt_ivf_topk_workspace_bytes": (c_size, [c_i64, c_int, c_i64, c_int]),
    "rt_ivf_topk": (c_int, [vp, c_i64, vp, c_i64, c_int, c_int, vp, c_i64, vp, vp, c_int, c_i64, c_int, vp, c_i64,
                            vp, vp, vp, c_size, vp]),
    "rt_segment_mean_f32": (c_int, [vp, c_i64, c_int, c_int, vp, c_i64, vp, c_int, vp, vp]),
    "rt_topk_merge": (c_int, [vp, vp, c_i64, c_int, c_int, c_int, vp, vp, vp]),
    "rt_flatip_topk_tuning": (c_int, [c_int, c_int, c_int]),
    "rt_flatip_topk_shard_workspace_bytes": (c_size, [c_i64, c_i64, c_int, c_int, c_int]),
    "rt_flatip_topk_shard_plan": (c_int, [c_i64, c_i64, c_int, c_int, c_int, c_int, vp]),
    "rt_flatip_topk_shard_sample": (c_int, [vp, c_i64, vp, c_i64, c_int, c_int, c_int, c_int, vp, vp, vp, c_size,
                                            vp]),
    "rt_topk_sample_rank": (c_int, [c_int, c_i64, c_i64, vp]),
    "rt_topk_sample_threshold": (c_int, [vp, c_int, c_i64, c_int, vp, vp]),
    "rt_flatip_topk_shard_search": (c_int, [vp, c_i64, vp, c_i64, c_int, c_int, c_int, vp, c_i64, vp, vp, vp,
                                            c_size, vp]),
    "rt_sample_negatives": (c_int, [vp, vp, c_i64, vp, c_i64, c_i64, c_int, c_u64, vp, vp, vp]),
    "rt_feeder_batch": (c_int, [vp, vp, vp, vp, c_i64, vp, vp, vp]),
    "rt_feeder_commit": (c_int, [vp, vp, c_i64, vp, vp]),
    "rt_linear_fwd_f32": (c_int, [ctypes.POINTER(LinearFwdArgs), vp]),
    "rt_linear_bwd_f32": (c_int, [ctypes.POINTER(LinearBwdArgs), vp]),
    "rt_linear_bwd_dz_f32": (c_int, [ctypes.POINTER(LinearBwdArgs), vp]),
    "rt_linear_bwd_dz_fused": (c_int, [ctypes.POINTER(LinearBwdArgs), c_int]),
    "rt_linear_bwd_dw_splits": (c_int, [ctypes.POINTER(LinearBwdArgs), c_int, ctypes.POINTER(c_i64)]),
    "rt_linear_bwd_dw_f32": (c_int, [ctypes.POINTER(LinearBwdArgs), vp]),
    "rt_linear_fwd_f32_multi": (c_int, [ctypes.POINTER(LinearFwdArgs), c_int, vp]),
    "rt_linear_bwd_dz_f32_multi": (c_int, [ctypes.POINTER(LinearBwdArgs), c_int, vp]),
    "rt_linear_bwd_dw_f32_multi": (c_int, [ctypes.POINTER(LinearBwdArgs), c_int, vp]),
    "rt_linear_bwd_dw_f32_joint": (c_int, [ctypes.POINTER(LinearBwdArgs), c_int, vp]),
    "rt_linear_bwd_dw_joint_splits": (c_int, [ctypes.POINTER(LinearBwdArgs), c_int, ctypes.POINTER(c_i64)]),
    "rt_tower_infer_f32": (c_int, [ctypes.POINTER(TowerInferArgs), vp]),
    "rt_twotower_loss_workspace_bytes": (c_size, [c_i64, c_int]),
    "rt_twotower_loss_fwd_bwd": (c_int, [vp, vp, vp, c_int, c_i64, c_int, c_int, c_f32, vp, vp, c_f32,
                                         c_f32, vp, vp, vp, vp, vp, vp, vp, c_size, vp]),
    "rt_twotower_loss_fwd": (c_int, [vp, vp, vp, c_int, c_i64, c_int, c_int, c_f32, vp, vp, c_f32, c_f32,
                                     vp, vp, c_size, vp]),
    "rt_inbatch_loss_workspace_bytes": (c_size, [c_i64, c_i64, c_int]),
    "rt_inbatch_loss_fwd_bwd": (c_int, [vp, vp, c_int, c_i64, c_i64, c_int, c_i64, c_f32, vp, vp, vp, vp, c_size, vp]),
    "rt_similarity_f32": (c_int, [vp, vp, c_i64, c_int, c_f32, vp, vp, vp, vp]),
    "rt_grad_sqnorm": (c_int, [vp, vp, c_int, vp, vp, vp, vp]),
    "rt_grad_sqnorm_fold": (c_int, [vp, vp, c_int, vp, vp, vp, ctypes.POINTER(GradFold), c_int, vp]),
    "rt_clip_adam_step": (c_int, [vp, vp, vp, vp, c_i64, vp, c_int, c_f32, c_f32, vp, c_f32, c_f32, c_f32,
                                  c_f32, c_int, vp, vp, c_i64, vp]),
    "rt_l2_augment_f32": (c_int, [vp, c_i64, c_int, vp, c_int, c_int, vp]),
    "rt_l2_finish_f32": (c_int, [vp, c_int, vp, c_int, c_int, c_i64, c_int, vp, vp, c_int, vp, vp, vp, c_i64, vp]),
    "rt_exclusion_bitmap": (c_int, [vp, vp, c_i64, vp, c_i64, c_i64, vp, c_i64, vp]),
    "rt_rank_metrics": (c_int, [vp, c_i64, c_int, vp, vp, vp, c_i64, vp, vp, vp, c_i64, vp, c_int, c_i64, vp, vp,
                                vp, vp]),
    "rt_rank_metrics_reduce": (c_int, [vp, vp, c_i64, c_int, vp, c_i64, vp, vp]),
    "rt_list_metrics": (c_int, [vp, c_i64, c_int, vp, c_int, c_i64, c_int, c_i64, vp, c_i64, ctypes.c_double, vp,
                                c_int, vp, vp, vp, vp, vp, vp]),
    "rt_list_metrics_reduce": (c_int, [vp, vp, vp, vp, c_i64, c_int, vp, vp]),
}

RT_METRICS_MAX_K = 16

_lib = None
_lock = threading.Lock()
_load_error: Optional[str] = None
MISSING: list = []


def lib():
    global _lib, _load_error
    if _lib is not None:
        return _lib
    with _lock:
        if _lib is not None:
            return _lib
        if not os.path.exists(LIB_PATH):
            _load_error = (f"{LIB_PATH} not found — build it with "
                           f"`make -C {PKG_DIR}` (or __graft_entry__.build())")
            raise NativeUnavailable(_load_error)
        try:
            handle = ctypes.CDLL(LIB_PATH)
        except OSError as e:
            _load_error = f"cannot load {LIB_PATH}: {e}"
            raise NativeUnavailable(_load_error) from e
        for name, (res, args) in SIGNATURES.items():
            if not hasattr(handle, name):
                MISSING.append(name)
                continue
            fn = getattr(handle, name)
            fn.restype = res
            fn.argtypes = args
        _lib = handle
        return _lib


def available() -> bool:
    try:
        lib()
        return True
    except NativeUnavailable:
        return False


def call(name: str, *args) -> int:
    fn = getattr(lib(), name)
    rc = fn(*args)
    if rc != 0:
        msg = lib().rt_status_string(rc).decode()
        last = lib().rt_last_error().decode()
        raise RTError(name, rc, msg + (f" [{last}]" if last else ""))
    return rc


def ptr(t: Optional[torch.Tensor]):
    return None if t is None else ctypes.c_void_p(t.data_ptr())


def stream_of(t: torch.Tensor):
    return ctypes.c_void_p(torch.cuda.current_stream(t.device).cuda_stream)


def require_device(*tensors: torch.Tensor, what: str = "rtrec kernel"):
    for t in tensors:
        if t is not None and t.device.type != "cuda":
            raise RuntimeError(f"{what}: expected a ROCm (cuda) device tensor, got {t.device}; "
                               "this MI355X build has no CPU fallback")
    lib()


def dtype_code(dt: torch.dtype) -> int:
    if dt == torch.float32:
        return RT_F32
    if dt == torch.float16:
        return RT_F16
    if dt == torch.bfloat16:
        return RT_BF16
    raise TypeError(f"unsupported dtype {dt}")
```

Measured before the change: 5.102 billion pairs/s.

## Pre-swizzle MLP weights into MFMA fragment order and stage loss fixed rows via LDS

The previous layer's forward kernel now also writes the next layer's weights, and the transposed weights, into a fragment-ordered image matching the MFMA lane layout. The forward and dz backward kernels can then fetch each weight fragment with contiguous float4 loads instead of strided per-row gathers. In the loss kernels, the fixed-side rows are loaded cooperatively by the whole block and read per wave from LDS, replacing redundant per-wave global loads. This costs extra LDS, extra global writes to build the images each step, added synchronisation, and new template variants.

```diff
diff --git a/include/rtrec_hip.h b/include/rtrec_hip.h
--- a/include/rtrec_hip.h
+++ b/include/rtrec_hip.h
@@ -172,9 +172,13 @@
     uint16_t* next_w_planes;
     int next_n;
     int next_k;
+    const float* w_frag;
+    float* next_w_frag;
+    float* wt_frag_out;
 } rt_linear_fwd_args;
 
 int rt_linear_fwd_f32(const rt_linear_fwd_args* args, void* stream);
+size_t rt_linear_w_frag_bytes(int n, int k, int transposed);
 
 typedef struct {
     int64_t m; int k; int n;
@@ -215,6 +219,7 @@
     int fold_splits;
     int fold_in;
     const uint16_t* wt_planes;
+    const float* wt_frag;
 } rt_linear_bwd_args;
 
 int rt_linear_bwd_f32(const rt_linear_bwd_args* args, void* stream);
diff --git a/real-time-recommendation-system-with-feature-store_amd/csrc/loss.hip b/real-time-recommendation-system-with-feature-store_amd/csrc/loss.hip
--- a/real-time-recommendation-system-with-feature-store_amd/csrc/loss.hip
+++ b/real-time-recommendation-system-with-feature-store_amd/csrc/loss.hip
@@ -93,6 +93,44 @@
         pf[kb] = split8(x);
     }
 }
+template <int DP, int NW>
+constexpr int fixed_per_thread() { return (32 * DP / 4 + 64 * NW - 1) / (64 * NW); }
+template <int DP, typename T, int NW>
+__device__ __forceinline__ void fixed_load(const T* __restrict__ F, int64_t f0, int64_t n, int D,
+                                           float4 (&v)[fixed_per_thread<DP, NW>()]) {
+    constexpr int TOT = 32 * DP / 4;
+    const int tid = threadIdx.x;
+#pragma unroll
+    for (int u = 0; u < fixed_per_thread<DP, NW>(); ++u) {
+        const int e = tid + 64 * NW * u;
+        const int row = e / (DP / 4), c = (e % (DP / 4)) * 4;
+        v[u] = make_float4(0.f, 0.f, 0.f, 0.f);
+        if (e < TOT && f0 + row < n && c < D) v[u] = load4<T>(F + (f0 + row) * D + c);
+    }
+}
+template <int DP, int NW>
+__device__ __forceinline__ void fixed_store(float* __restrict__ Fs, const float4 (&v)[fixed_per_thread<DP, NW>()]) {
+    constexpr int TOT = 32 * DP / 4;
+    const int tid = threadIdx.x;
+#pragma unroll
+    for (int u = 0; u < fixed_per_thread<DP, NW>(); ++u) {
+        const int e = tid + 64 * NW * u;
+        const int row = e / (DP / 4), c = (e % (DP / 4)) * 4;
+        if (e < TOT) *reinterpret_cast<float4*>(Fs + row * (DP + LDP) + c) = v[u];
+    }
+}
+template <int DP>
+__device__ __forceinline__ void fixed_from_lds(const float* __restrict__ Fs, Pieces (&pf)[DP / 16]) {
+    const int lane = threadIdx.x & 63, c = lane & 31, h = lane >> 5;
+    const float* ap = Fs + c * (DP + LDP) + 8 * h;
+#pragma unroll
+    for (int kb = 0; kb < DP / 16; ++kb) {
+        const float4 u = *reinterpret_cast<const float4*>(ap + 16 * kb);
+        const float4 v = *reinterpret_cast<const float4*>(ap + 16 * kb + 4);
+        const float x[8] = {u.x, u.y, u.z, u.w, v.x, v.y, v.z, v.w};
+        pf[kb] = split8(x);
+    }
+}
 template <int DP>
 __device__ __forceinline__ f32x16 s_tile3(const float* __restrict__ Ss, const Pieces (&pf)[DP / 16]) {
     const int lane = threadIdx.x & 63, c = lane & 31, h = lane >> 5;
@@ -118,6 +156,16 @@
     return DP <= 128 ? 8 : 4;
 #endif
 }
+template <int DP, int NW>
+constexpr bool bwd_fixed_own() {
+#ifdef RT_LOSS_FIXED_DIRECT
+    return false;
+#else
+    return inb_lds_bytes<DP>(NW + 1) + SPAN * sizeof(float) <= 160 * 1024;
+#endif
+}
+template <int DP, int NW>
+constexpr size_t bwd_lds_bytes() { return inb_lds_bytes<DP>(bwd_fixed_own<DP, NW>() ? NW + 1 : NW); }
 
 template <int DP, typename T>
 __global__ __launch_bounds__(256) void loss_fwd_kernel(Args a) {
@@ -137,10 +185,20 @@
     if (js < a.ib_blocks) {
         float* Ss = sm_f + w * 32 * (DP + LDP);
         Pieces pf[DP / 16];
-        load_fixed3<DP, T>(U, i0, a.b, D, pf);
         const int64_t t0 = static_cast<int64_t>(js) * SPAN + 32 * w, t1 = t0 + 128;
         float4 buf[DP / 8];
+#ifdef RT_LOSS_FIXED_DIRECT
+        load_fixed3<DP, T>(U, i0, a.b, D, pf);
         load_rows<DP, T>(P, t0, a.nx, D, buf);
+#else
+        float4 fx[fixed_per_thread<DP, 4>()];
+        fixed_load<DP, T, 4>(U, i0, a.b, D, fx);
+        load_rows<DP, T>(P, t0, a.nx, D, buf);
+        fixed_store<DP, 4>(sm_f, fx);
+        __syncthreads();
+        fixed_from_lds<DP>(sm_f, pf);
+        __syncthreads();
+#endif
         float om = -INFINITY, ol = 0.f;
 #pragma unroll 1
         for (int q = 0; q < 2; ++q) {
@@ -313,6 +371,12 @@
     const float scale = wb_eff / static_cast<float>(a.b);
     float lse_fixed = 0.f;
     const bool ib = wb_eff != 0.f;
+    const bool active = a.grad && ib && f0 < n_fixed && s0 < n_str;
+#ifndef RT_LOSS_FIXED_DIRECT
+    float* const Fs = bwd_fixed_own<DP, NW>() ? sm_b + NW * 32 * (DP + LDP) : sm_b;
+    float4 fx[fixed_per_thread<DP, NW>()];
+    if (active) fixed_load<DP, T, NW>(Fm, f0, n_fixed, D, fx);
+#endif
     if (row_pass) {
         const int64_t i = f0 + c;
         if (ib && i < a.b) lse_fixed = combine_lse(a.part, a.n_split, a.b, i);
@@ -345,15 +409,24 @@
             lse_s[x] = i < a.b ? combine_lse(a.part, a.n_split, a.b, i) : 0.f;
         }
     }
+#ifndef RT_LOSS_FIXED_DIRECT
+    if (active) fixed_store<DP, NW>(Fs, fx);
+#endif
     __syncthreads();
-    if (!a.grad || !ib || f0 >= n_fixed || s0 >= n_str) return;
+    if (!active) return;
 
     float* Ss = sm_b + w * 32 * (DP + LDP);
     Pieces pf[DP / 16];
-    load_fixed3<DP, T>(Fm, f0, n_fixed, D, pf);
     const int64_t t0 = s0 + 32 * w;
     float4 buf[DP / 8];
+#ifdef RT_LOSS_FIXED_DIRECT
+    load_fixed3<DP, T>(Fm, f0, n_fixed, D, pf);
     load_rows<DP, T>(Sm, t0, n_str, D, buf);
+#else
+    load_rows<DP, T>(Sm, t0, n_str, D, buf);
+    fixed_from_lds<DP>(Fs, pf);
+    if constexpr (!bwd_fixed_own<DP, NW>()) __syncthreads();
+#endif
     f32x16 acc[DT];
 #pragma unroll
     for (int x = 0; x < DT; ++x) acc[x] = f32x16{};
@@ -458,7 +531,7 @@
     const int rc = check_launch("loss_fwd_kernel");
     if (rc) return rc;
     constexpr int NW = loss::bwd_waves<DP>();
-    const size_t lds2 = loss::inb_lds_bytes<DP>(NW);
+    const size_t lds2 = loss::bwd_lds_bytes<DP, NW>();
     allow_lds<loss::loss_bwd_kernel<DP, T, NW>>(lds2);
     hipLaunchKernelGGL((loss::loss_bwd_kernel<DP, T, NW>), grid2, dim3(64 * NW), lds2, st, a, wb_eff, true);
     return check_launch("loss_bwd_kernel");
diff --git a/real-time-recommendation-system-with-feature-store_amd/csrc/mlp.hip b/real-time-recommendation-system-with-feature-store_amd/csrc/mlp.hip
--- a/real-time-recommendation-system-with-feature-store_amd/csrc/mlp.hip
+++ b/real-time-recommendation-system-with-feature-store_amd/csrc/mlp.hip
@@ -1,5 +1,6 @@
 #include "rt_common.h"
 #include "split3.h"
+#include "w_frag.h"
 
 namespace rt {
 namespace mlp {
@@ -236,9 +237,10 @@
     return !a.dsrc && a.g_prev && act_is_piecewise_linear(a.prev_act);
 }
 
-template <int TPW, bool KVEC, bool WPL>
+template <int TPW, bool KVEC, bool WPL, bool WF = false>
 __global__ __launch_bounds__(256) __attribute__((amdgpu_waves_per_eu(TPW == 1 ? 3 : 2))) void linear_fwd_kernel(FwdLaunch L) {
     static_assert(!WPL || (TPW == 1 && KVEC), "split-weight planes: one-tile waves, k % 4 == 0");
+    static_assert(!WF || (TPW <= 2 && KVEC && !WPL), "fragment image: one- or two-tile waves, k % 8 == 0");
     const bool g1 = blockIdx.x >= L.split;
     const rt_linear_fwd_args& a = g1 ? L.a1 : L.a0;
     const unsigned bid = blockIdx.x - (g1 ? L.split : 0u);
@@ -333,6 +335,35 @@
             }
         }
     }
+    if (a.next_w_frag || a.wt_frag_out) {
+        const int nblk = static_cast<int>(g1 ? gridDim.x - L.split : L.split);
+        const int64_t e0 = static_cast<int64_t>(bid) * 256 + tid, estep = static_cast<int64_t>(nblk) * 256;
+        if (a.next_w_frag) {
+            const int nn = a.next_n, nk = a.next_k;
+            const int64_t tot = wfrag::fwd_entries(nn, nk);
+            float4* dst = reinterpret_cast<float4*>(a.next_w_frag);
+            for (int64_t e = e0; e < tot; e += estep) {
+                int row, col;
+                wfrag::fwd_coords(nk, e, row, col);
+                float4 v = make_float4(0.f, 0.f, 0.f, 0.f);
+                if (row < nn && col < nk) v = *reinterpret_cast<const float4*>(a.next_w + static_cast<int64_t>(row) * nk + col);
+                dst[e] = v;
+            }
+        }
+        if (a.wt_frag_out) {
+            const int64_t tot = wfrag::dz_entries(n, k);
+            float4* dst = reinterpret_cast<float4*>(a.wt_frag_out);
+            for (int64_t e = e0; e < tot; e += estep) {
+                int trow, tcol;
+                wfrag::dz_coords(n, e, trow, tcol);
+                float x[4];
+#pragma unroll
+                for (int q = 0; q < 4; ++q)
+                    x[q] = (trow < k && tcol + q < n) ? a.w[static_cast<int64_t>(tcol + q) * k + trow] : 0.f;
+                dst[e] = make_float4(x[0], x[1], x[2], x[3]);
+            }
+        }
+    }
     const float* wrow[TPW];
     bool tile_on[TPW], row_ok[TPW];
 #pragma unroll
@@ -343,7 +374,21 @@
         wrow[i] = a.w + static_cast<int64_t>(row_ok[i] ? nn : 0) * k;
     }
     float4 wv[TPW][4], wn[TPW][4];
+    const float4* wfb[TPW];
+#pragma unroll
+    for (int i = 0; i < TPW; ++i)
+        wfb[i] = WF ? reinterpret_cast<const float4*>(a.w_frag) + wfrag::fwd_index(k, w + 4 * i, 0, 0, lane) : nullptr;
     auto load_w = [&](int s, float4 (&dst)[TPW][4]) {
+        if constexpr (WF) {
+#pragma unroll
+            for (int i = 0; i < TPW; ++i) {
+                const float4* p = wfb[i] + (s >> 5) * 256;
+#pragma unroll
+                for (int j = 0; j < 4; ++j)
+                    dst[i][j] = tile_on[i] ? p[j * 64] : make_float4(0.f, 0.f, 0.f, 0.f);
+            }
+            return;
+        }
 #pragma unroll
         for (int i = 0; i < TPW; ++i)
 #pragma unroll
@@ -707,8 +752,9 @@
     RT_PP_END(1)
 }
 
-template <int TPWK, bool WPL, bool KS, int FE>
+template <int TPWK, bool WPL, bool KS, int FE, bool WF = false>
 __global__ __launch_bounds__(256) __attribute__((amdgpu_waves_per_eu(3))) void linear_bwd_dz_kernel(BwdLaunch L) {
+    static_assert(!WF || (TPWK <= 2 && !WPL), "fragment image: one- or two-tile waves");
 #ifdef RT_FOLD_FIRST
     fold_side(L, 0);
 #endif
@@ -737,7 +783,23 @@
 #else
     const float* __restrict__ WtT = (a.wt && (n % 8) == 0) ? a.wt : nullptr;
 #endif
+    const float4* __restrict__ Wfr = WF ? reinterpret_cast<const float4*>(a.wt_frag) : nullptr;
     auto load_w = [&](int s, float (&dst)[TPWK][8]) {
+        if constexpr (WF) {
+#pragma unroll
+            for (int i = 0; i < TPWK; ++i) {
+                const int kt = tb + w + 4 * i;
+                float4 v0 = make_float4(0.f, 0.f, 0.f, 0.f), v1 = v0;
+                if (kt * 32 < k) {
+                    const float4* p = Wfr + wfrag::dz_index(n, kt, s >> 4, 0, lane);
+                    v0 = p[0];
+                    v1 = p[64];
+                }
+                dst[i][0] = v0.x; dst[i][1] = v0.y; dst[i][2] = v0.z; dst[i][3] = v0.w;
+                dst[i][4] = v1.x; dst[i][5] = v1.y; dst[i][6] = v1.z; dst[i][7] = v1.w;
+            }
+            return;
+        }
 #pragma unroll
         for (int i = 0; i < TPWK; ++i) {
             const int kk = (tb + w + 4 * i) * 32 + c32;
@@ -1573,11 +1635,30 @@
                             (reinterpret_cast<uintptr_t>(a.next_w) & 15) ||
                             (reinterpret_cast<uintptr_t>(a.next_w_planes) & 15)))
         return RT_ERR_INVALID;
+    if (a.w_frag && (rt_linear_w_frag_bytes(a.n, a.k, 0) == 0 || (reinterpret_cast<uintptr_t>(a.w_frag) & 15) ||
+                     (reinterpret_cast<uintptr_t>(a.w) & 15)))
+        return RT_ERR_INVALID;
+    if (a.next_w_frag && (!a.next_w || rt_linear_w_frag_bytes(a.next_n, a.next_k, 0) == 0 ||
+                          (reinterpret_cast<uintptr_t>(a.next_w) & 15) ||
+                          (reinterpret_cast<uintptr_t>(a.next_w_frag) & 15)))
+        return RT_ERR_INVALID;
+    if (a.wt_frag_out && (rt_linear_w_frag_bytes(a.n, a.k, 1) == 0 || (reinterpret_cast<uintptr_t>(a.wt_frag_out) & 15)))
+        return RT_ERR_INVALID;
     const int kp = mlp::pad8(a.k);
     const int tpw = a.n <= 128 ? 1 : a.n <= 256 ? 2 : 4;
     const size_t lds = (2 * kp + 3 * mlp::FM * kp / 2 + 4 * tpw * mlp::FM) * sizeof(float) + mlp::FM * sizeof(int64_t) + 16;
     if (lds > 160 * 1024) return RT_ERR_UNSUPPORTED;
     return RT_OK;
+}
+
+extern "C" size_t rt_linear_w_frag_bytes(int n, int k, int transposed) {
+    if (n <= 0 || k <= 0) return 0;
+    if (transposed) {
+        if ((n % 8) != 0 || k > 256) return 0;
+        return static_cast<size_t>(wfrag::dz_entries(n, k)) * sizeof(float4);
+    }
+    if ((k % 8) != 0 || n > 256) return 0;
+    return static_cast<size_t>(wfrag::fwd_entries(n, k)) * sizeof(float4);
 }
 
 extern "C" int rt_linear_fwd_f32_multi(const rt_linear_fwd_args* args, int n_args, void* stream) {
@@ -1589,12 +1670,14 @@
 #endif
     int tpw = 1, kp_max = 0;
     bool kvec = true, wpl = true;
+    bool wfr = true;
     unsigned blocks[2] = {0u, 0u};
     for (int g = 0; g < n_args; ++g) {
         const int v = validate_fwd(&args[g]);
         if (v) return v;
         const rt_linear_fwd_args& a = args[g];
         wpl = wpl && a.w_planes != nullptr;
+        wfr = wfr && a.w_frag != nullptr;
         const int t = a.n <= 128 ? 1 : a.n <= 256 ? 2 : 4;
         tpw = t > tpw ? t : tpw;
         kvec = kvec && (a.k % 4) == 0 && (reinterpret_cast<uintptr_t>(a.w) & 15) == 0;
@@ -1613,13 +1696,15 @@
     if (total == 0) return RT_OK;
     hipStream_t st = as_stream(stream);
     const dim3 grid(total);
-#define RT_FWD(T, V, P)                                                                           \
-    do {                                                                                          \
-        allow_lds<mlp::linear_fwd_kernel<T, V, P>>(lds);                                          \
-        hipLaunchKernelGGL((mlp::linear_fwd_kernel<T, V, P>), grid, dim3(256), lds, st, L);       \
+#define RT_FWD(T, V, P, ...)                                                                              \
+    do {                                                                                                  \
+        allow_lds<mlp::linear_fwd_kernel<T, V, P, ##__VA_ARGS__>>(lds);                                   \
+        hipLaunchKernelGGL((mlp::linear_fwd_kernel<T, V, P, ##__VA_ARGS__>), grid, dim3(256), lds, st, L); \
     } while (0)
     if (kvec && tpw == 1 && wpl) {
         RT_FWD(1, true, true);
+    } else if (kvec && wfr && tpw <= 2) {
+        if (tpw == 1) RT_FWD(1, true, false, true); else RT_FWD(2, true, false, true);
     } else if (kvec) {
         if (tpw == 1) RT_FWD(1, true, false); else if (tpw == 2) RT_FWD(2, true, false); else RT_FWD(4, true, false);
     } else {
@@ -1651,7 +1736,7 @@
 #if defined(RT_DZ_NO_FE) || defined(RT_NO_WT_ROWS)
     return 0;
 #endif
-    if (!a.wt || (a.n % 8) != 0) return 0;
+    if ((!a.wt && !a.wt_frag) || (a.n % 8) != 0) return 0;
     if ((a.m % mlp::FM) != 0 || !mlp::dz_da_fast(a)) return 0;
     if (a.grad_mode == 0) return mlp::dz_norm_fast(a.n) ? 1 : 0;
     return ((a.grad_mode == 1 || a.grad_mode == 2) && mlp::dz_bn_fast(a.n, a.act, a.grad_mode)) ? 2 : 0;
@@ -1678,6 +1763,8 @@
                        (reinterpret_cast<uintptr_t>(a.fold_src) & 15) || (reinterpret_cast<uintptr_t>(a.fold_dst) & 15)))
         return RT_ERR_INVALID;
     if (a.wt_planes && ((a.n % 8) != 0 || (reinterpret_cast<uintptr_t>(a.wt_planes) & 15))) return RT_ERR_INVALID;
+    if (a.wt_frag && (rt_linear_w_frag_bytes(a.n, a.k, 1) == 0 || (reinterpret_cast<uintptr_t>(a.wt_frag) & 15)))
+        return RT_ERR_INVALID;
     return RT_OK;
 }
 
@@ -1687,6 +1774,8 @@
     size_t lds = 0;
     unsigned blocks[2] = {0u, 0u};
     bool wpl = true;
+    bool wfr = true;
+    bool wt_all = true;
     int fe = -1;
     for (int g = 0; g < n_args; ++g) {
         const int v = validate_bwd(&args[g]);
@@ -1696,6 +1785,8 @@
         const int fc = dz_fast_class(a);
         fe = (fe < 0 || fe == fc) ? fc : 0;
         wpl = wpl && (!need_da || a.wt_planes != nullptr);
+        wfr = wfr && need_da && a.wt_frag != nullptr;
+        wt_all = wt_all && a.wt != nullptr;
         const int t = !need_da ? 1 : a.k <= 128 ? 1 : a.k <= 256 ? 2 : 4;
         tpwk = t > tpwk ? t : tpwk;
         const int np = mlp::pad8(a.n);
@@ -1725,13 +1816,22 @@
     if (ks == 2) tpwk = 1;
     const dim3 grid(total * ks);
     hipStream_t st = as_stream(stream);
-#define RT_DZ(T, P, K, F)                                                                        \
-    do {                                                                                         \
-        allow_lds<mlp::linear_bwd_dz_kernel<T, P, K, F>>(lds);                                   \
-        hipLaunchKernelGGL((mlp::linear_bwd_dz_kernel<T, P, K, F>), grid, dim3(256), lds, st, L); \
+#define RT_DZ(T, P, K, F, ...)                                                                               \
+    do {                                                                                                     \
+        allow_lds<mlp::linear_bwd_dz_kernel<T, P, K, F, ##__VA_ARGS__>>(lds);                                \
+        hipLaunchKernelGGL((mlp::linear_bwd_dz_kernel<T, P, K, F, ##__VA_ARGS__>), grid, dim3(256), lds, st, L); \
     } while (0)
+    if (!wfr && !wt_all) fe = 0;
     if (ks > 1) {
-        if (wpl) RT_DZ(1, true, true, 0); else RT_DZ(1, false, true, 0);
+        if (wpl) RT_DZ(1, true, true, 0); else if (wfr) RT_DZ(1, false, true, 0, true); else RT_DZ(1, false, true, 0);
+    } else if (wfr && !wpl && tpwk <= 2) {
+        if (tpwk == 1) {
+            if (fe == 1) RT_DZ(1, false, false, 1, true); else RT_DZ(1, false, false, 0, true);
+        } else {
+            if (fe == 1) RT_DZ(2, false, false, 1, true);
+            else if (fe == 2) RT_DZ(2, false, false, 2, true);
+            else RT_DZ(2, false, false, 0, true);
+        }
     } else {
         switch (tpwk) {
             case 1:
diff --git a/real-time-recommendation-system-with-feature-store_amd/csrc/w_frag.h b/real-time-recommendation-system-with-feature-store_amd/csrc/w_frag.h
--- /dev/null
+++ b/real-time-recommendation-system-with-feature-store_amd/csrc/w_frag.h
@@ -0,0 +1,52 @@
+#ifndef RTREC_W_FRAG_H
+#define RTREC_W_FRAG_H
+
+#include <stdint.h>
+
+#if defined(__HIPCC__) || defined(__CUDACC__)
+#define RT_WF_HD __host__ __device__ __forceinline__
+#else
+#define RT_WF_HD inline
+#endif
+
+namespace rt {
+namespace wfrag {
+
+RT_WF_HD int pad32(int x) { return (x + 31) / 32 * 32; }
+
+RT_WF_HD int fwd_tiles(int n) { return (n + 31) / 32; }
+RT_WF_HD int fwd_steps(int k) { return pad32(k) / 32; }
+RT_WF_HD int64_t fwd_entries(int n, int k) { return static_cast<int64_t>(fwd_tiles(n)) * fwd_steps(k) * 4 * 64; }
+RT_WF_HD int64_t fwd_index(int k, int t, int s, int j, int l) {
+    return ((static_cast<int64_t>(t) * fwd_steps(k) + s) * 4 + j) * 64 + l;
+}
+RT_WF_HD void fwd_coords(int k, int64_t e, int& row, int& col) {
+    const int l = static_cast<int>(e & 63), j = static_cast<int>((e >> 6) & 3);
+    const int64_t ts = e >> 8;
+    const int S = fwd_steps(k);
+    const int s = static_cast<int>(ts % S), t = static_cast<int>(ts / S);
+    const int c = l & 31, h = l >> 5;
+    row = 32 * t + c;
+    col = 32 * s + 16 * (j >> 1) + 8 * h + 4 * (j & 1);
+}
+
+RT_WF_HD int dz_tiles(int k) { return (k + 31) / 32; }
+RT_WF_HD int dz_steps(int n) { return pad32(n) / 16; }
+RT_WF_HD int64_t dz_entries(int n, int k) { return static_cast<int64_t>(dz_tiles(k)) * dz_steps(n) * 2 * 64; }
+RT_WF_HD int64_t dz_index(int n, int kt, int sb, int j, int l) {
+    return ((static_cast<int64_t>(kt) * dz_steps(n) + sb) * 2 + j) * 64 + l;
+}
+RT_WF_HD void dz_coords(int n, int64_t e, int& trow, int& tcol) {
+    const int l = static_cast<int>(e & 63), j = static_cast<int>((e >> 6) & 1);
+    const int64_t ks = e >> 7;
+    const int NS = dz_steps(n);
+    const int sb = static_cast<int>(ks % NS), kt = static_cast<int>(ks / NS);
+    const int c = l & 31, h = l >> 5;
+    trow = 32 * kt + c;
+    tcol = 16 * sb + 8 * h + 4 * j;
+}
+
+}
+}
+
+#endif
diff --git a/real-time-recommendation-system-with-feature-store_amd/rtrec_amd/models/fused.py b/real-time-recommendation-system-with-feature-store_amd/rtrec_amd/models/fused.py
--- a/real-time-recommendation-system-with-feature-store_amd/rtrec_amd/models/fused.py
+++ b/real-time-recommendation-system-with-feature-store_amd/rtrec_amd/models/fused.py
@@ -173,6 +173,8 @@
     wts: List[Optional[torch.Tensor]] = field(default_factory=list)
     w_planes: List[Optional[torch.Tensor]] = field(default_factory=list)
     wt_planes: List[Optional[torch.Tensor]] = field(default_factory=list)
+    wt_frags: List[Optional[torch.Tensor]] = field(default_factory=list)
+    w_frags: List[torch.Tensor] = field(default_factory=list)
     ains: List[Optional[torch.Tensor]] = field(default_factory=list)
 
 
@@ -187,6 +189,13 @@
 SPLIT_W_PLANES = _WPL in ("1", "fwd", "dz")
 SPLIT_W_PLANES_FWD = _WPL in ("1", "fwd")
 SPLIT_W_PLANES_DZ = _WPL in ("1", "dz")
+_WFR = os.environ.get("RTREC_W_FRAG", "1")
+W_FRAG_FWD = _WFR in ("1", "fwd")
+W_FRAG_DZ = _WFR in ("1", "dz")
+
+
+def _w_frag_floats(n: int, k: int, transposed: bool) -> int:
+    return int(native.lib().rt_linear_w_frag_bytes(n, k, 1 if transposed else 0)) // 4
 
 
 def stats_arena_size(blocks: List[Block], n_seg: int = 1) -> int:
@@ -323,16 +332,21 @@
                     prod.fin_eps, prod.fin_momentum = a.bn_eps, a.bn_momentum
                     a.prev_final = 1
         a.act = b.act
-        wt = wtp = None
+        wt = wtp = wtf = None
         if li > 0 and lin.training:
+            ftw = _w_frag_floats(lin.out_features, lin.in_features, True) if W_FRAG_DZ else 0
             if SPLIT_W_PLANES and SPLIT_W_PLANES_DZ and lin.out_features % 8 == 0:
                 wtp = torch.empty((3, lin.in_features, lin.out_features), dtype=torch.int16, device=dev)
                 a.wt_planes_out = wtp.data_ptr()
+            elif ftw:
+                wtf = torch.empty(ftw, dtype=torch.float32, device=dev)
+                a.wt_frag_out = wtf.data_ptr()
             else:
                 wt = torch.empty((lin.in_features, lin.out_features), dtype=torch.float32, device=dev)
                 a.wt_out = wt.data_ptr()
         ctx.wts.append(wt)
         ctx.wt_planes.append(wtp)
+        ctx.wt_frags.append(wtf)
         wp = None
         if SPLIT_W_PLANES and SPLIT_W_PLANES_FWD and li > 0 and lin.in_features % 8 == 0 and lin.out_features <= 128:
             wp = torch.empty((3, lin.out_features, lin.in_features), dtype=torch.int16, device=dev)
@@ -342,6 +356,16 @@
             prev.next_n, prev.next_k = lin.out_features, lin.in_features
             a.w_planes = wp.data_ptr()
         ctx.w_planes.append(wp)
+        if wp is None and W_FRAG_FWD and li > 0 and lin.training:
+            fw = _w_frag_floats(lin.out_features, lin.in_features, False)
+            if fw:
+                wf = torch.empty(fw, dtype=torch.float32, device=dev)
+                prev = layers[li - 1]
+                prev.next_w = lin.weight.data_ptr()
+                prev.next_w_frag = wf.data_ptr()
+                prev.next_n, prev.next_k = lin.out_features, lin.in_features
+                a.w_frag = wf.data_ptr()
+                ctx.w_frags.append(wf)
         ain = None
         if li > 0 and lin.training and lin.in_features % 4 == 0:
             ain = torch.empty((m, lin.in_features), dtype=torch.float32, device=dev)
@@ -618,6 +642,8 @@
                 a.wt = ctx.wts[li].data_ptr()
             if li < len(ctx.wt_planes) and ctx.wt_planes[li] is not None:
                 a.wt_planes = ctx.wt_planes[li].data_ptr()
+            if li < len(ctx.wt_frags) and ctx.wt_frags[li] is not None:
+                a.wt_frag = ctx.wt_frags[li].data_ptr()
             if li < len(ctx.ains) and ctx.ains[li] is not None:
                 a.a_in = ctx.ains[li].data_ptr()
         layers.append(a)
diff --git a/real-time-recommendation-system-with-feature-store_amd/rtrec_amd/native.py b/real-time-recommendation-system-with-feature-store_amd/rtrec_amd/native.py
--- a/real-time-recommendation-system-with-feature-store_amd/rtrec_amd/native.py
+++ b/real-time-recommendation-system-with-feature-store_amd/rtrec_amd/native.py
@@ -46,6 +46,7 @@
         ("fin_num_batches_tracked", vp), ("fin_eps", c_f32), ("fin_momentum", c_f32), ("prev_final", c_int),
         ("w_planes", vp), ("wt_planes_out", vp), ("next_w", vp), ("next_w_planes", vp), ("next_n", c_int),
         ("next_k", c_int),
+        ("w_frag", vp), ("next_w_frag", vp), ("wt_frag_out", vp),
     ]
 
 
@@ -61,7 +62,7 @@
         ("seed_offset", vp), ("g_prev", vp), ("g_prev_stats", vp), ("dsrc", vp), ("seg_split", c_i64),
         ("dbias_slots", vp), ("wt", vp), ("fuse_dz", c_int), ("a_in", vp), ("dw_part", vp),
         ("fold_src", vp), ("fold_dst", vp), ("fold_words", c_i64), ("fold_splits", c_int), ("fold_in", c_int),
-        ("wt_planes", vp),
+        ("wt_planes", vp), ("wt_frag", vp),
     ]
 
 
@@ -133,6 +134,7 @@
     "rt_feeder_batch": (c_int, [vp, vp, vp, vp, c_i64, vp, vp, vp]),
     "rt_feeder_commit": (c_int, [vp, vp, c_i64, vp, vp]),
     "rt_linear_fwd_f32": (c_int, [ctypes.POINTER(LinearFwdArgs), vp]),
+    "rt_linear_w_frag_bytes": (c_size, [c_int, c_int, c_int]),
     "rt_linear_bwd_f32": (c_int, [ctypes.POINTER(LinearBwdArgs), vp]),
     "rt_linear_bwd_dz_f32": (c_int, [ctypes.POINTER(LinearBwdArgs), vp]),
     "rt_linear_bwd_dz_fused": (c_int, [ctypes.POINTER(LinearBwdArgs), c_int]),
```

After: 5.359 billion pairs/s (median of 6 runs). 1.05x the previous value.
